# xxxupeng/stereo_toolbox

Hardware: AMD Instinct MI355X
Metric: stereo pairs/sec @ 540x960 D=192 (GwcNet_GC fwd+bwd) (higher is better)
Workload: dtype f32; 1 GPU; GwcNet_GC(maxdisp=192) train step: fwd+bwd+allreduce+Adam, 576x960 pairs (reference pad_to_2x shape), batch 1/GPU, fp32, synthetic randn inputs, deterministic filler weights; global_batch=1, parallelism=dp1, grad_sync=none (single rank: flat fp32 buffer packed, no collective), launch=eager, optimizer=torch.optim.Adam(fused=True)

## Files before the change

include/stx_hip.h:

```cpp
#ifndef STX_HIP_H
#define STX_HIP_H
#ifdef __cplusplus
extern "C" {
#endif

const char* stx_last_error(void);
const char* stx_build_info(void);
int stx_get_tuning(const char* name);
int stx_set_tuning(const char* name, int value);

int stx_cost_volume_fwd(const float* Lg, const float* Rg, int Cg, int G, const float* Lc, const float* Rc, int Cc,
                        const float* scale, float* vol, int B, int H, int W, int D, int mask_left, void* stream);
int stx_group_normalize_fwd(const float* x, float* y, int B, int C, int G, int HW, float out_scale, void* stream);
int stx_group_normalize_bwd(const float* x, const float* gy, float* gx, int B, int C, int G, int HW, float out_scale, void* stream);
int stx_cost_volume_bwd(const float* gvol, const float* Lg, const float* Rg, int Cg, int G, int Cc, float* gLg,
                        float* gRg, float* gLc, float* gRc, int B, int H, int W, int D, int mask_left, void* stream);

int stx_head_fwd(const float* cost, float* disp, float* stats, int B, int Dc, int Hc, int Wc, int D, int H, int W,
                 void* stream);
long long stx_head_bwd_workspace_floats(int B, int Dc, int H, int W);
int stx_head_bwd(const float* gdisp, const float* cost, const float* disp, const float* stats, float* gcost,
                 float* workspace, int B, int Dc, int Hc, int Wc, int D, int H, int W, void* stream);
int stx_head_fwd2(const float* cost, float* disp, float* stats, int B, int Dc, int Hc, int Wc, int D, int H, int W,
                  int align_corners, void* stream);
int stx_head_bwd2(const float* gdisp, const float* cost, const float* disp, const float* stats, float* gcost,
                  float* workspace, int B, int Dc, int Hc, int Wc, int D, int H, int W, int align_corners, void* stream);
int stx_softargmax_fwd(const float* x, float* out, int B, int D, int HW, void* stream);
int stx_argmax_fwd(const float* x, long long* out, int B, int D, int HW, void* stream);
int stx_unimodal_fwd(const float* x, float* out, int B, int D, int HW, void* stream);
int stx_dominant_modal_fwd(const float* x, float* out, int B, int D, int HW, void* stream);
int stx_modal_fwd(const float* x, float* out, float* aux, int B, int D, int HW, int kind, void* stream);
int stx_modal_bwd(const float* g, const float* out, const float* aux, float* gx, int B, int D, int HW, void* stream);
int stx_split_mode(const float* x, float* mode, unsigned char* mask, int B, int D, int HW, void* stream);
int stx_softmax_d_fwd(const float* x, float* y, int B, int D, int HW, void* stream);

long long stx_conv3d_packed_floats(int K, int N, int T);
int stx_conv3d_pack_weight(const float* w, float* wp, int A, int B, int T, int mode, void* stream);
int stx_conv3d_fwd_blocks(int Do, int Ho, int Wo);
long long stx_conv3d_fwd_stat_rows(int B, int Di, int Hi, int Wi, int Cin, int Cout, int ks, int stride);
int stx_conv3d_fwd(const float* x, const float* wp, float* out, const float* scale, const float* bias,
                   const float* residual, float* stats, int B, int Di, int Hi, int Wi, int Cin, int Cout, int ks,
                   int stride, int relu, void* stream);
int stx_deconv3d_fwd_blocks(int Di, int Hi, int Wi);
int stx_deconv3d_fwd(const float* x, const float* wp, float* out, const float* scale, const float* bias,
                     const float* residual, float* stats, int B, int Di, int Hi, int Wi, int Cin, int Cout, int Do,
                     int Ho, int Wo, int relu, void* stream);
long long stx_conv3d_wgrad_workspace_floats(int B, int Dc, int Hc, int Wc, int CF, int CC, int ks, int stride);
int stx_conv3d_wgrad(const float* fine, const float* coarse, float* dw, float* workspace, int B, int Df, int Hf, int Wf,
                     int CF, int Dc, int Hc, int Wc, int CC, int ks, int stride, void* stream);

int stx_conv3d_wgrad_bn_supported(int B, int D, int H, int W, int CF, int CC);
int stx_conv3d_wgrad_bn(const float* x, const float* gy, const float* z, const float* scale, const float* shift, const float* mean,
                        const float* invstd, const float* gamma, const float* sums, float inv_n, int act, float* dz, float* dw,
                        float* workspace, int B, int D, int H, int W, int CF, int CC, void* stream);

int stx_conv3d_axial_supported(int Cin, int Cout, int kd, int kh, int kw);
long long stx_conv3d_axial_packed_floats(int K, int N, int kd, int kh, int kw);
int stx_conv3d_axial_pack_weight(const float* w, float* wp, int A, int B, int kd, int kh, int kw, int mode, void* stream);
long long stx_conv3d_axial_fwd_stat_rows(int B, int D, int H, int W, int Cin, int Cout, int kd, int kh, int kw);
int stx_conv3d_axial_fwd(const float* x, const float* wp, float* out, const float* scale, const float* bias,
                         const float* residual, float* stats, int B, int D, int H, int W, int Cin, int Cout, int kd, int kh,
                         int kw, int act, void* stream);
long long stx_conv3d_axial_wgrad_workspace_floats(int B, int D, int H, int W, int CF, int CC, int kd, int kh, int kw);
int stx_conv3d_axial_wgrad(const float* x, const float* gz, float* dw, float* workspace, int B, int D, int H, int W, int CF,
                           int CC, int kd, int kh, int kw, void* stream);

int stx_convgru_supported(int hidden, int nx, int cx0, int cx1, int cx2, int ksize);
long long stx_convgru_packed_floats(int K, int N);
int stx_convgru_pack_weight(const float* w0, const float* w1, float* wp, int A, int Bd, int mode, void* stream);
int stx_convgru_gemm(const float* s0, int c0, int p0, const float* s1, int c1, int p1, const float* s2, int c2, int p2,
                     const float* s3, int c3, int p3, const float* wp, int N, int epi, int split, const float* bias0,
                     const float* bias1, const float* add0, int add0_pitch, const float* add1, int add1_pitch, const float* h,
                     int h_pitch, const float* z, float* out0, float* out1, float* out2, int out_pitch, int B, int H, int W,
                     void* stream);
int stx_convgru_gate_rows(long long P, int hidden);
int stx_convgru_gate_bwd(const float* g, int g_pitch, const float* z, const float* q, const float* h, int h_pitch, float* gq,
                         float* gz, float* rows, long long P, int hidden, void* stream);
int stx_convgru_reset_bwd(float* buf, int buf_pitch, const float* g, int g_pitch, const float* z, const float* r, const float* h,
                          int h_pitch, float* gr, float* rows, long long P, int hidden, void* stream);
int stx_convgru_row_sum(const float* rows, float* out, int nrows, int n, void* stream);
long long stx_convgru_wgrad_workspace_floats(int B, int H, int W, int K, int CC);
int stx_convgru_wgrad(const float* s0, int c0, int p0, const float* s1, int c1, int p1, const float* s2, int c2, int p2,
                      const float* s3, int c3, int p3, const float* g0, const float* g1, int CG, float* dw, float* workspace,
                      int B, int H, int W, void* stream);

int stx_conv2d_supported(int Cin, int Cout);
long long stx_conv2d_stat_rows(int groups);
int stx_conv2d_fwd(const float* x, const float* w, float* out, float* stats, int B, int H, int W, int Cin, int Cout, int dgrad,
                   int groups, void* stream);

int stx_conv3d_c1_fwd(const float* x, const float* w, const float* residual, float* out, int B, int D, int H, int W,
                      int Cin, void* stream);
long long stx_conv3d_c1_wgrad_workspace_floats(int Cin);
int stx_conv3d_c1_wgrad(const float* x, const float* gy, float* dw, float* workspace, int B, int D, int H, int W,
                        int Cin, void* stream);
int stx_conv3d_c1_dgrad(const float* gy, const float* w, float* gx, int B, int D, int H, int W, int Cin, void* stream);

int stx_mish_fwd(const float* x, float* y, long long n, void* stream);
int stx_mish_bwd(const float* gy, const float* x, float* gx, long long n, void* stream);
int stx_depth_to_space(const float* y, float* out, int B, int D, int H, int W, int C, int inverse, void* stream);
int stx_gate_fwd(const float* cv, const float* att, float* out, int B, int D, long long HW, int C, void* stream);
int stx_gate_bwd(const float* g, const float* cv, const float* att, float* gcv, float* gatt, int B, int D, long long HW,
                 int C, void* stream);

int stx_concat_channels(const float* in0, const float* in1, const float* in2, const float* in3, int C0, int C1, int C2, int C3,
                        float* out, long long nvox, void* stream);
int stx_split_channels(const float* in, float* out0, float* out1, float* out2, float* out3, int C0, int C1, int C2, int C3,
                       long long nvox, void* stream);
int stx_transpose(const float* in, float* out, int N, int rows, int cols, void* stream);

int stx_dwconv_hw_fwd(const float* x, const float* w, const int* dil, float* out, int B, int D, int H, int W, int C,
                      int flip, void* stream);
long long stx_dwconv_hw_wgrad_workspace_floats(int C);
int stx_dwconv_hw_wgrad(const float* x, const float* gy, const int* dil, float* dw, float* workspace, int B, int D,
                        int H, int W, int C, void* stream);
int stx_cost_volume_scale_bwd(const float* gvol, const float* Lc, const float* Rc, float* gscale, int B, int Cc, int H,
                              int W, int D, int mask_left, void* stream);
int stx_scale_channels(const float* x, const float* s, float* out, long long nvox, int C, void* stream);
int stx_ac_volume_bwd(const float* gvol, const float* Lc, const float* Rc, const float* prob, float* gL, float* gR,
                      float* gprob, int B, int Cc, int H, int W, int D, int mask_left, void* stream);

int stx_bn_reduce_blocks(void);
int stx_bn_stats_rows(long long nvox, int C);
int stx_bn_stats(const float* z, float* partials, long long nvox, int C, int groups, void* stream);
int stx_bn_finalize(const float* partials, int nrows, int C, double count, const float* gamma, const float* beta,
                    float* running_mean, float* running_var, float momentum, float eps, float* scale, float* shift,
                    float* mean, float* invstd, void* stream);
int stx_bn_finalize_groups(const float* partials, int nrows, int C, double count, const float* gamma, const float* beta,
                           float* running_mean, float* running_var, float momentum, float eps, float* out, int groups,
                           void* stream);
int stx_bn_apply(const float* z1, const float* scale1, const float* shift1, const float* z2, const float* scale2,
                 const float* shift2, float* out, long long nvox, int C, int relu, int groups, void* stream);
int stx_bn_bwd_reduce(const float* gy, const float* y, const float* z1, const float* mean1, const float* invstd1,
                      const float* z2, const float* mean2, const float* invstd2, float* partials, float* sums,
                      long long nvox, int C, int relu, void* stream);
int stx_bn_bwd_apply(const float* gy, const float* y, const float* z1, const float* mean1, const float* invstd1,
                     const float* gamma1, const float* z2, const float* mean2, const float* invstd2,
                     const float* gamma2, const float* sums, float* dz1, float* dz2, float* gout, long long nvox, int C,
                     int relu, void* stream);
int stx_bn_bwd_reduce2(const float* gy, const float* y, const float* z1, const float* mean1, const float* invstd1,
                       const float* z2, const float* mean2, const float* invstd2, const float* scale1,
                       const float* shift1, const float* scale2, const float* shift2, float* partials, float* sums,
                       long long nvox, int C, int relu, int groups, void* stream);
int stx_bn_bwd_apply2(const float* gy, const float* y, const float* z1, const float* mean1, const float* invstd1,
                      const float* gamma1, const float* z2, const float* mean2, const float* invstd2,
                      const float* gamma2, const float* scale1, const float* shift1, const float* scale2,
                      const float* shift2, const float* sums, float* dz1, float* dz2, float* gout, long long nvox,
                      int C, int relu, int groups, void* stream);

int stx_pad_normalize_u8(const unsigned char* img, float* out, int B, int H, int W, int Hp, int Wp, int top,
                         const float* mean3, const float* std3, void* stream);

int stx_sampled_volume_fwd(const float* Lg, const float* Rg, int Cg, int G, const float* Lc, const float* Rc, int Cc,
                           const float* samples, float* vol, int B, int H, int W, int S, int CTp, void* stream);
int stx_sampled_volume_bwd(const float* gvol, const float* Lg, const float* Rg, int Cg, int G, int Cc,
                           const float* samples, float* gLg, float* gRg, float* gLc, float* gRc, int B, int H, int W,
                           int S, int CTp, void* stream);

int stx_warp_fwd(const float* x, const float* disp, float* out, int B, int C, int H, int W, void* stream);
int stx_warp_bwd(const float* gout, const float* x, const float* disp, float* gx, float* gdisp, int B, int C, int H, int W,
                 void* stream);
int stx_corr_volume_fwd(const float* ref, const float* tgt, float* vol, int B, int C, int H, int W, int maxdisp, int groups,
                        void* stream);
int stx_corr_volume_bwd(const float* gvol, const float* ref, const float* tgt, float* gref, float* gtgt, int B, int C, int H,
                        int W, int maxdisp, int groups, void* stream);
int stx_disparity_variance_fwd(const float* x, const float* disp, const float* samples, float* out, int B, int D, int HW,
                               void* stream);
int stx_disparity_variance_bwd(const float* g, const float* x, const float* disp, const float* samples, float* gx, float* gdisp,
                               float* gsamples, int B, int D, int HW, void* stream);

long long stx_geo_pyramid_floats(long long rows, int len, int C, int levels);
int stx_geo_corr_fwd(const float* fmap1, const float* fmap2, float* cpyr, int B, int C, int H, int W1, int W2, int levels,
                     void* stream);
int stx_geo_corr_bwd(const float* gcpyr, const float* fmap1, const float* fmap2, float* gfmap1, float* gfmap2, int B, int C, int H,
                     int W1, int W2, int levels, void* stream);
int stx_geo_pyramid_fwd(const float* vol, float* gpyr, int B, int D, int H, int W, int C, int levels, void* stream);
int stx_geo_pyramid_bwd(const float* ggpyr, float* gvol, int B, int D, int H, int W, int C, int levels, void* stream);
int stx_geo_lookup_fwd(const float* gpyr, const float* cpyr, const float* disp, const float* coords, float* out, int B, int H,
                       int W, int D, int C, int W2, int levels, int radius, void* stream);
// ... 117 lines not shown
```

stereo_toolbox_amd/_capi.py:

```python
import ctypes
import os
import threading

import torch

_P = ctypes.c_void_p
_I = ctypes.c_int
_F = ctypes.c_float
_L = ctypes.c_longlong

SIGNATURES = {
    "stx_get_tuning": [ctypes.c_char_p],
    "stx_set_tuning": [ctypes.c_char_p, _I],
    "stx_cost_volume_fwd": [_P, _P, _I, _I, _P, _P, _I, _P, _P, _I, _I, _I, _I, _I, _P],
    "stx_cost_volume_bwd": [_P, _P, _P, _I, _I, _I, _P, _P, _P, _P, _I, _I, _I, _I, _I, _P],
    "stx_group_normalize_fwd": [_P, _P, _I, _I, _I, _I, _F, _P],
    "stx_group_normalize_bwd": [_P, _P, _P, _I, _I, _I, _I, _F, _P],
    "stx_head_fwd": [_P, _P, _P, _I, _I, _I, _I, _I, _I, _I, _P],
    "stx_head_bwd_workspace_floats": [_I, _I, _I, _I],
    "stx_head_bwd": [_P, _P, _P, _P, _P, _P, _I, _I, _I, _I, _I, _I, _I, _P],
    "stx_head_fwd2": [_P, _P, _P, _I, _I, _I, _I, _I, _I, _I, _I, _P],
    "stx_head_bwd2": [_P, _P, _P, _P, _P, _P, _I, _I, _I, _I, _I, _I, _I, _I, _P],
    "stx_softargmax_fwd": [_P, _P, _I, _I, _I, _P],
    "stx_argmax_fwd": [_P, _P, _I, _I, _I, _P],
    "stx_softmax_d_fwd": [_P, _P, _I, _I, _I, _P],
    "stx_unimodal_fwd": [_P, _P, _I, _I, _I, _P],
    "stx_dominant_modal_fwd": [_P, _P, _I, _I, _I, _P],
    "stx_modal_fwd": [_P, _P, _P, _I, _I, _I, _I, _P],
    "stx_modal_bwd": [_P, _P, _P, _P, _I, _I, _I, _P],
    "stx_split_mode": [_P, _P, _P, _I, _I, _I, _P],
    "stx_conv3d_packed_floats": [_I, _I, _I],
    "stx_conv3d_pack_weight": [_P, _P, _I, _I, _I, _I, _P],
    "stx_conv3d_fwd_blocks": [_I, _I, _I],
    "stx_conv3d_fwd_stat_rows": [_I, _I, _I, _I, _I, _I, _I, _I],
    "stx_deconv3d_fwd_blocks": [_I, _I, _I],
    "stx_conv3d_fwd": [_P, _P, _P, _P, _P, _P, _P, _I, _I, _I, _I, _I, _I, _I, _I, _I, _P],
    "stx_deconv3d_fwd": [_P, _P, _P, _P, _P, _P, _P, _I, _I, _I, _I, _I, _I, _I, _I, _I, _I, _P],
    "stx_conv3d_wgrad_workspace_floats": [_I, _I, _I, _I, _I, _I, _I, _I],
    "stx_conv3d_wgrad": [_P, _P, _P, _P, _I, _I, _I, _I, _I, _I, _I, _I, _I, _I, _I, _P],
    "stx_conv3d_wgrad_bn_supported": [_I, _I, _I, _I, _I, _I],
    "stx_conv3d_wgrad_bn": [_P] * 9 + [_F, _I, _P, _P, _P, _I, _I, _I, _I, _I, _I, _P],
    "stx_conv3d_axial_supported": [_I, _I, _I, _I, _I],
    "stx_conv3d_axial_packed_floats": [_I, _I, _I, _I, _I],
    "stx_conv3d_axial_pack_weight": [_P, _P, _I, _I, _I, _I, _I, _I, _P],
    "stx_conv3d_axial_fwd_stat_rows": [_I] * 9,
    "stx_conv3d_axial_fwd": [_P] * 7 + [_I] * 10 + [_P],
    "stx_conv3d_axial_wgrad_workspace_floats": [_I] * 9,
    "stx_conv3d_axial_wgrad": [_P, _P, _P, _P] + [_I] * 9 + [_P],
    "stx_convgru_supported": [_I] * 6,
    "stx_convgru_packed_floats": [_I, _I],
    "stx_convgru_pack_weight": [_P, _P, _P, _I, _I, _I, _P],
    "stx_convgru_gemm": [_P, _I, _I] * 4 + [_P, _I, _I, _I, _P, _P, _P, _I, _P, _I, _P, _I, _P, _P, _P, _P, _I, _I, _I, _I, _P],
    "stx_convgru_gate_rows": [_L, _I],
    "stx_convgru_gate_bwd": [_P, _I, _P, _P, _P, _I, _P, _P, _P, _L, _I, _P],
    "stx_convgru_reset_bwd": [_P, _I, _P, _I, _P, _P, _P, _I, _P, _P, _L, _I, _P],
    "stx_convgru_row_sum": [_P, _P, _I, _I, _P],
    "stx_convgru_wgrad_workspace_floats": [_I] * 5,
    "stx_convgru_wgrad": [_P, _I, _I] * 4 + [_P, _P, _I, _P, _P, _I, _I, _I, _P],
    "stx_conv2d_supported": [_I, _I],
    "stx_conv2d_stat_rows": [_I],
    "stx_conv2d_fwd": [_P, _P, _P, _P, _I, _I, _I, _I, _I, _I, _I, _P],
    "stx_conv3d_c1_fwd": [_P, _P, _P, _P, _I, _I, _I, _I, _I, _P],
    "stx_conv3d_c1_wgrad_workspace_floats": [_I],
    "stx_conv3d_c1_wgrad": [_P, _P, _P, _P, _I, _I, _I, _I, _I, _P],
    "stx_conv3d_c1_dgrad": [_P, _P, _P, _I, _I, _I, _I, _I, _P],
    "stx_mish_fwd": [_P, _P, _L, _P],
    "stx_mish_bwd": [_P, _P, _P, _L, _P],
    "stx_depth_to_space": [_P, _P, _I, _I, _I, _I, _I, _I, _P],
    "stx_gate_fwd": [_P, _P, _P, _I, _I, _L, _I, _P],
    "stx_gate_bwd": [_P, _P, _P, _P, _P, _I, _I, _L, _I, _P],
    "stx_concat_channels": [_P, _P, _P, _P, _I, _I, _I, _I, _P, _L, _P],
    "stx_split_channels": [_P, _P, _P, _P, _P, _I, _I, _I, _I, _L, _P],
    "stx_transpose": [_P, _P, _I, _I, _I, _P],
    "stx_dwconv_hw_fwd": [_P, _P, _P, _P, _I, _I, _I, _I, _I, _I, _P],
    "stx_dwconv_hw_wgrad_workspace_floats": [_I],
    "stx_dwconv_hw_wgrad": [_P, _P, _P, _P, _P, _I, _I, _I, _I, _I, _P],
    "stx_cost_volume_scale_bwd": [_P, _P, _P, _P, _I, _I, _I, _I, _I, _I, _P],
    "stx_scale_channels": [_P, _P, _P, _L, _I, _P],
    "stx_ac_volume_bwd": [_P, _P, _P, _P, _P, _P, _P, _I, _I, _I, _I, _I, _I, _P],
    "stx_pad_normalize_u8": [_P, _P, _I, _I, _I, _I, _I, _I, _P, _P, _P],
    "stx_warp_fwd": [_P, _P, _P, _I, _I, _I, _I, _P],
    "stx_warp_bwd": [_P, _P, _P, _P, _P, _I, _I, _I, _I, _P],
    "stx_corr_volume_fwd": [_P, _P, _P, _I, _I, _I, _I, _I, _I, _P],
    "stx_corr_volume_bwd": [_P, _P, _P, _P, _P, _I, _I, _I, _I, _I, _I, _P],
    "stx_disparity_variance_fwd": [_P, _P, _P, _P, _I, _I, _I, _P],
    "stx_disparity_variance_bwd": [_P, _P, _P, _P, _P, _P, _P, _I, _I, _I, _P],
    "stx_sampled_volume_fwd": [_P, _P, _I, _I, _P, _P, _I, _P, _P, _I, _I, _I, _I, _I, _P],
    "stx_sampled_volume_bwd": [_P, _P, _P, _I, _I, _I, _P, _P, _P, _P, _P, _I, _I, _I, _I, _I, _P],
    "stx_geo_pyramid_floats": [_L, _I, _I, _I],
    "stx_geo_corr_fwd": [_P, _P, _P, _I, _I, _I, _I, _I, _I, _P],
    "stx_geo_corr_bwd": [_P, _P, _P, _P, _P, _I, _I, _I, _I, _I, _I, _P],
    "stx_geo_pyramid_fwd": [_P, _P, _I, _I, _I, _I, _I, _I, _P],
    "stx_geo_pyramid_bwd": [_P, _P, _I, _I, _I, _I, _I, _I, _P],
    "stx_geo_lookup_fwd": [_P, _P, _P, _P, _P, _I, _I, _I, _I, _I, _I, _I, _I, _P],
    "stx_geo_lookup_bwd": [_P, _P, _P, _P, _P, _I, _I, _I, _I, _I, _I, _I, _I, _P],
    "stx_context_upsample_fwd": [_P, _P, _P, _I, _I, _I, _P],
    "stx_context_upsample_bwd": [_P, _P, _P, _P, _P, _I, _I, _I, _P],
    "stx_corr1d_pyramid_floats": [_L, _I, _I],
    "stx_corr1d_pyramid_fwd": [_P, _P, _P, _I, _I, _I, _I, _I, _I, _F, _P],
    "stx_corr1d_pyramid_bwd": [_P, _P, _P, _P, _P, _I, _I, _I, _I, _I, _I, _F, _P],
    "stx_corr1d_lookup_fwd": [_P, _P, _P, _P, _I, _P, _I, _I, _I, _I, _I, _P],
    "stx_corr1d_lookup_bwd": [_P, _P, _P, _P, _I, _P, _I, _I, _I, _I, _I, _P],
    "stx_allpairs_estimates_fwd": [_P, _I, _P, _P, _P, _P, _P, _I, _I, _I, _I, _P],
    "stx_allpairs_estimates_bwd": [_P, _P, _P, _P, _P, _P, _P, _I, _I, _I, _I, _P],
    "stx_corr1d_volume_pyramid_fwd": [_P, _P, _P, _F, _P, _I, _I, _I, _I, _I, _P],
    "stx_corr1d_volume_pyramid_bwd": [_P, _P, _P, _F, _P, _I, _I, _I, _I, _I, _P],
    "stx_truncate_mask_fwd": [_P, _P, _I, _F, _F, _P, _I, _I, _I, _P],
    "stx_generate_masks_fwd": [_P, _P, _I, _I, _I, _I, _P],
    "stx_masked_volume_fwd": [_P, _P, _P, _P, _I, _I, _I, _I, _I, _P],
    "stx_masked_volume_bwd": [_P, _P, _P, _P, _I, _I, _I, _I, _I, _P],
    "stx_softlrc_fwd": [_P, _P, _F, _P, _P, _I, _I, _I, _P],
    "stx_softlrc_bwd_workspace_floats": [_I, _I, _I],
    "stx_softlrc_bwd": [_P, _P, _P, _P, _F, _P, _P, _P, _I, _I, _I, _P],
    "stx_weighted_lsq_fwd": [_P, _P, _P, _F, _F, _P, _P, _P, _I, _L, _P],
    "stx_weighted_lsq_bwd": [_P, _P, _P, _P, _P, _P, _P, _P, _P, _I, _L, _P],
    "stx_mirror_detector_fwd": [_P, _P, _P, _P, _F, _F, _P, _L, _P],
    "stx_mirror_detector_bwd": [_P, _P, _P, _P, _P, _F, _F, _P, _P, _P, _P, _L, _P],
    "stx_photo_warp_fwd": [_P, _P, _P, _P, _I, _I, _I, _I, _P],
    "stx_photo_warp_bwd": [_P, _P, _P, _P, _I, _I, _I, _I, _P],
    "stx_ssim_fwd": [_P, _P, _P, _I, _I, _I, _I, _I, _P],
    "stx_ssim_bwd_workspace_floats": [_I, _I, _I, _I],
    "stx_ssim_bwd": [_P, _P, _P, _P, _P, _P, _I, _I, _I, _I, _I, _P],
    "stx_photometric_fwd": [_P, _P, _P, ctypes.c_double, _I, _P, _I, _I, _I, _I, _P],
    "stx_photometric_bwd_workspace_floats": [_I, _I, _I, _I],
# ... 105 lines not shown
```

stereo_toolbox_amd/aggregation.py:

```python
import os
import threading

import torch
import torch.nn as nn

from . import ops


def _is_transposed(conv):
    return isinstance(conv, nn.ConvTranspose3d)


def _conv_cfg(conv):
    ks = conv.kernel_size[0]
    stride = conv.stride[0]
    if _is_transposed(conv):
        k3 = ks == 3 and stride == 2 and conv.padding[0] == 1 and conv.output_padding[0] == 1
        k4 = ks == 4 and stride == 2 and conv.padding[0] == 1 and conv.output_padding[0] == 0
        if not (k3 or k4) or len(set(conv.kernel_size)) != 1 or len(set(conv.stride)) != 1:
            raise ops.StxError("only ConvTranspose3d(k=3, s=2, p=1, op=1) and ConvTranspose3d(k=4, s=2, p=1) are on the hot path")
    else:
        if not ((ks == 3 and conv.padding[0] == 1 and stride in (1, 2)) or (ks == 1 and conv.padding[0] == 0 and stride == 1)):
            raise ops.StxError(f"unsupported Conv3d k={ks} s={stride} p={conv.padding}")
    if conv.bias is not None or conv.groups != 1:
# ... 104 lines not shown
        momentum = 1.0 / float(bn.num_batches_tracked.item())
    else:
        momentum = 0.0
    return {"training": training, "partials": partials, "count": count, "running_mean": bn.running_mean,
            "running_var": bn.running_var, "momentum": momentum, "eps": bn.eps, "sync": sync}


def _raw_conv(x, conv, want):
    ks, stride = _conv_cfg(conv)
    if _is_transposed(conv) and ks == 4:
        return ops.deconv4_raw(x, conv.weight, want)
    return ops.ConvRawFn.apply(x, conv.weight, ks, stride, _is_transposed(conv), want)


@ops.fp32_region
def shared_input_convs(x, blocks):
    cfgs, ws = [], []
    for seq in blocks:
        conv, bn = seq[0], seq[1]
        if _is_transposed(conv) or not bn.training or conv.weight.shape[1] != x.shape[-1] or conv.weight.shape[1] % 8 \
                or conv.weight.shape[0] % 8:
            return None
        ks, stride = _conv_cfg(conv)
        cfgs.append((ks, stride, True))
        ws.append(conv.weight)
    if not _needs_grad(x, *[m for seq in blocks for m in (seq[0], seq[1])]):
        return None
    outs = ops.SharedInputConvsFn.apply(x, tuple(cfgs), *ws)
    return [(outs[2 * k], outs[2 * k + 1]) for k in range(len(blocks))]


@ops.fp32_region
def conv_block(x, conv, bn=None, relu=False, second=None, residual=None, mish=False, leaky=False, raw=None, second_raw=None):
    if (mish and relu) or (leaky and (relu or mish)):
        raise ops.StxError("conv_block: relu, mish and leaky are mutually exclusive")
    if second is not None and residual is not None:
        raise ops.StxError("conv_block: `second` and `residual` are mutually exclusive")
    mods = [conv, bn] + ([second[1], second[2]] if second is not None else [])
    grad = (raw is not None or second_raw is not None
            or _needs_grad(x, residual, *(m for m in mods if m is not None), *([second[0]] if second else [])))
    train_bn = (bn is not None and bn.training) or (second is not None and second[2].training)
    if mish and (grad or train_bn) and (bn is None or residual is not None):
        return ops.mish(conv_block(x, conv, bn, relu=False, second=second, residual=residual))
    if mish:
        relu = 2
    if leaky:
        relu = 3

    if not grad and not train_bn:
        if second is not None:
            s2, b2 = _fold(second[2])
            residual = _infer_conv(second[0], second[1], s2, b2, None, False)
        if bn is not None:
            s1, b1 = _fold(bn)
        else:
            s1 = b1 = None
        return _infer_conv(x, conv, s1, b1, residual, relu)

    want = bn is not None and bn.training
    z1, part1 = raw if raw is not None else _raw_conv(x, conv, want)
    if bn is None:
        y = z1
        if residual is not None:
            y = y + residual
        if relu == 3:
            return torch.nn.functional.leaky_relu(y, 0.01)
        return torch.relu(y) if relu else y
    count1 = z1.numel() // z1.shape[-1]
    st1 = _bn_state(bn, part1 if want else None, count1)
    if second is not None:
        x2, conv2, bn2 = second
        want2 = bn2.training
        z2, part2 = second_raw if second_raw is not None else _raw_conv(x2, conv2, want2)
        st2 = _bn_state(bn2, part2 if want2 else None, z2.numel() // z2.shape[-1])
        return ops.BnActFn.apply(z1, bn.weight, bn.bias, z2, bn2.weight, bn2.bias, None, relu, st1, st2)
    defer = (residual is None and want and relu in (0, 1, False, True) and not _is_transposed(conv) and _conv_cfg(conv) == (3, 1)
             and conv.weight.shape[0] % 32 == 0 and conv.weight.shape[1] % 32 == 0 and not st1.get("sync")
             and os.environ.get("STX_BN_BWD_IN_WGRAD", "1") != "0")
    if defer:
        ops.bn_defer_reset_if_stale()
    return ops.BnActFn.apply(z1, bn.weight, bn.bias, None, None, None, residual, relu, st1, None, 1, defer)


def _axial_cfg(conv):
    if not isinstance(conv, nn.Conv3d) or _is_transposed(conv):
        raise ops.StxError("axial_conv_block: expected an nn.Conv3d")
    kernel = ops._axial_kernel(conv.weight, "axial_conv_block")
    if tuple(conv.stride) != (1, 1, 1) or tuple(conv.dilation) != (1, 1, 1) or conv.groups != 1:
        raise ops.StxError(f"axial_conv_block: stride {tuple(conv.stride)} dilation {tuple(conv.dilation)} groups {conv.groups}: "
                           "only dense stride-1 convolutions are served")
    if tuple(conv.padding) != tuple(k // 2 for k in kernel) or conv.padding_mode != "zeros":
        raise ops.StxError(f"axial_conv_block: padding {conv.padding} ({conv.padding_mode}) is not the 'same' zero padding of kernel {kernel}")
    return kernel


def _fold_with_bias(conv, bn):
    scale, shift = _fold(bn)
    if conv.bias is None:
        return scale, shift
    hit = conv.__dict__.get("_stx_fold") if ops._CACHE_ENABLED else None
    key = (conv.bias._version, conv.bias.data_ptr())
    if hit is not None and hit[0] == key and hit[1] is shift:
        return scale, hit[2]
    with torch.no_grad():
        shift_b = torch.addcmul(shift, conv.bias, scale).contiguous()
    if ops._CACHE_ENABLED:
        conv.__dict__["_stx_fold"] = (key, shift, shift_b)
    return scale, shift_b


@ops.fp32_region
def axial_conv_block(x, conv, bn):
    kernel = _axial_cfg(conv)
    if not isinstance(bn, nn.modules.batchnorm._BatchNorm):
        raise ops.StxError(f"axial_conv_block: {type(bn).__name__} is not a BatchNorm")
    if not _needs_grad(x, conv, bn) and not bn.training:
        scale, shift = _fold_with_bias(conv, bn)
        xk, wk, _ = ops._axial_prepare(x, conv.weight.detach(), "axial_conv_block")
        wp = ops.pack_weight_axial(wk, 0, owner=conv.weight if wk.shape == conv.weight.shape else None)
        return ops.conv3d_axial_forward(xk, wp, conv.weight.shape[0], kernel, scale, shift, None, 1)[0]
    want = bn.training
    z, part = ops.AxialConvRawFn.apply(x, conv.weight, want)
    if conv.bias is not None:
        z = ops.ZeroGradBiasFn.apply(z, conv.bias) if want else z + conv.bias
    st = _bn_state(bn, part if want else None, z.numel() // z.shape[-1])
    y = ops.BnActFn.apply(z, bn.weight, bn.bias, None, None, None, None, 1, st, None)
    if want and conv.bias is not None and bn.track_running_stats and bn.running_mean is not None:
        with torch.no_grad():
            bn.running_mean.add_(conv.bias.detach(), alpha=float(st["momentum"]))
    return y


@ops.fp32_region
def convbn_block(x, seq, relu=False, second=None, residual=None, mish=False, raw=None, second_raw=None):
    sec = None
    if second is not None:
        sec = (second[0], second[1][0], second[1][1])
    return conv_block(x, seq[0], seq[1], relu=relu, second=sec, residual=residual, mish=mish, raw=raw, second_raw=second_raw)
```

stereo_toolbox_amd/csrc/conv3d.hip:

```cpp
#include "stx_common.h"
#include <stdlib.h>

namespace {

constexpr int CONV_THREADS = 256;

struct ConvArgs {
    const float* x;
    const float* wp;
    float* out;
    const float* scale;
    const float* bias;
    const float* residual;
    float* stats;
    int Di, Hi, Wi, Cin;
    int Do, Ho, Wo, Cout;
    int relu;
    int nDt, nHt, nWt;
};

__device__ __forceinline__ int xcd_remap(int bid, int nblk) {
    const int q = nblk >> 3, r = nblk & 7;
    const int xcd = bid & 7, k = bid >> 3;
    const int base = (xcd < r) ? xcd * (q + 1) : r * (q + 1) + (xcd - r) * q;
// ... 360 lines not shown
    };
    using HM = HaloMap<ED, EH, EW, NF4>;
    HM hm;
    hm.init(tid, a.Hi, a.Wi, a.Cin);
    auto load_item = [&](int t, int c0) {
        int b, od0, oh0, ow0;
        tile_origin(t, b, od0, oh0, ow0);
        const int id0 = od0 * S - PAD, ih0 = oh0 * S - PAD, iw0 = ow0 * S - PAD;
        unsigned vo[NST];
        hm.offsets(id0, ih0, iw0, a.Di, a.Hi, a.Wi, vo);
        const stx_bufrsrc xrs = HM::rsrc(a.x, b, id0, ih0, iw0, a.Di, a.Hi, a.Wi, a.Cin);
#pragma unroll
        for (int k = 0; k < NST; ++k) stg[k] = stx_buf_ld4(xrs, vo[k], (unsigned)c0 * 4u);
    };
    auto store_item = [&]() {
#pragma unroll
        for (int k = 0; k < NST; ++k) {
            const int e = tid + k * CONV_THREADS;
            const int v = e / NF4, f = e - v * NF4;
            const int wx = v % EW, hy = (v / EW) % EH, dz = v / (EW * EH);
            const int slot = (S == 2) ? (wx & 1) * EWH + (wx >> 1) : wx;
            if (e < NE) stx_st4(tile + ((dz * EH + hy) * EWS + slot) * VS + 4 * f, stg[k]);
        }
    };

    float s1[NTW], s2[NTW];
#pragma unroll
    for (int nt = 0; nt < NTW; ++nt) { s1[nt] = 0.f; s2[nt] = 0.f; }
    f32x16 acc[MT][NTW];
    float4 bring[3][NQC][NTW];
    static_assert(KS == 3, "the pipelined kernel serves 3x3x3 only");
    const float* wbase = a.wp + (size_t)lane * 4 + (size_t)wcol * NTW * 256;
    if (t_lo < t_hi) {
        load_item(t_lo, 0);
        conv_ring_prologue<NTW, NQC, NT>(wbase, NQ, bring);
    }
    for (int t = t_lo; t < t_hi; ++t) {
#pragma unroll
        for (int m = 0; m < MT; ++m)
#pragma unroll
            for (int nt = 0; nt < NTW; ++nt) acc[m][nt] = zero16();
        for (int ch = 0; ch < nchunk; ++ch) {
            __syncthreads();
            store_item();
            __syncthreads();
            {
                const int nch = ch + 1 < nchunk ? ch + 1 : 0;
                const int ntl = ch + 1 < nchunk ? t : t + 1;
                if (ntl < t_hi) load_item(ntl, nch * CK);
            }
            const float* wq = wbase + (size_t)(ch * (CK / 8)) * NT * 256;
            const float* wq_next = ch + 1 < nchunk ? wq + (size_t)NQC * NT * 256 : (t + 1 < t_hi ? wbase : nullptr);
            conv_chunk_taps27<S, MT, NTW, NQC, EH, EWS, EWH, VS, NT>(tile, abase, wq, wq_next, NQ, acc, bring);
        }
        int b, od0, oh0, ow0;
        tile_origin(t, b, od0, oh0, ow0);
#pragma unroll
        for (int m = 0; m < MT; ++m) {
            const int mtile = wrow * MT + m;
            const int od = od0 + mtile / TH, oh = oh0 + mtile % TH;
            int nrows = (od < a.Do && oh < a.Ho) ? (a.Wo - ow0) : 0;
            nrows = nrows > 32 ? 32 : nrows;
            const size_t vox0 = (((size_t)b * a.Do + od) * a.Ho + oh) * a.Wo + ow0;
#pragma unroll
            for (int nt = 0; nt < NTW; ++nt) {
                const int n = (wcol * NTW + nt) * 32 + i;
                const float sc = (a.scale && n < a.Cout) ? a.scale[n] : 1.f;
                const float bs = (a.bias && n < a.Cout) ? a.bias[n] : 0.f;
                conv_epilogue_block(a, acc[m][nt], vox0, 1, nrows, n, sc, bs, lane, s1[nt], s2[nt]);
            }
        }
    }
    if (a.stats) conv_write_stats<NT, WN>(a, s1, s2, tile, tid, (size_t)blockIdx.x);
}

struct MarchArgs {
    ConvArgs c;
    int ncols;
    int ablate;
    int xs, xo;
    int os, oo, ncout;
    int wq_total, wq_off, wnt_total, wnt_off;
    const float* acc_in;
};

constexpr int MW2_MW = 16, MW2_R = 2, MW2_TH = 8, MW2_EH = 10, MW2_EW = 18, MW2_VS = 36;
constexpr int MW2_SLOT = MW2_EH * MW2_EW * MW2_VS;
constexpr int MW2_NF4 = (MW2_EH * MW2_EW * 8 + 255) / 256;
constexpr int MW2_WFLOATS = 27 * 4 * 256;

template <int BS, int EPI = 1>
__global__ __launch_bounds__(256) void conv3d_marchw_kernel(MarchArgs ma) {
    const ConvArgs& a = ma.c;
    STX_DYN_SMEM(smem);
    float* wl = reinterpret_cast<float*>(smem);
    float* planes = wl + MW2_WFLOATS;
    const int tid = threadIdx.x, lane = tid & 63, wave = tid >> 6;
    const int i = lane & 31, half = lane >> 5;
    const int th = wave;
    auto n_lane = [&]() { return i; };

    for (int e = tid; e < MW2_WFLOATS / 4; e += 256) {
        const int tq = e >> 6, l4 = e & 63;
        const int tap = tq >> 2, q = tq & 3;
        const size_t src = (((size_t)tap * ma.wq_total + ma.wq_off + q) * ma.wnt_total + ma.wnt_off) * 256 + 4 * l4;
        stx_st4(wl + 4 * e, stx_ld4(a.wp + src));
    }

    int b = 0, oh0 = 0, ow0 = 0;
    const long long units = (long long)ma.ncols * a.Do;
    const long long wg = xcd_remap(blockIdx.x, gridDim.x);
    int u = __builtin_amdgcn_readfirstlane((int)(units * wg / gridDim.x));
    const int u_end = __builtin_amdgcn_readfirstlane((int)(units * (wg + 1) / gridDim.x));

    float4 stg[MW2_NF4];
    unsigned svoff[MW2_NF4], ovoff = 0, ovalid = 0;
    const unsigned xplane_bytes = (unsigned)a.Hi * (unsigned)a.Wi * (unsigned)ma.xs * 4u;
    const unsigned oplane_bytes = (unsigned)a.Ho * (unsigned)a.Wo * (unsigned)ma.os * 4u;
    auto column_offsets = [&]() {
#pragma unroll
        for (int k = 0; k < MW2_NF4; ++k) {
            const int idx = tid + k * 256;
            const int v = idx >> 3, f = idx & 7;
            const int wx = v % MW2_EW, hy = v / MW2_EW;
            const int gh = oh0 - 1 + hy, gw = ow0 - 1 + wx;
            const bool ok = v < MW2_EH * MW2_EW && gh >= 0 && gh < a.Hi && gw >= 0 && gw < a.Wi;
            svoff[k] = ok ? (unsigned)(((gh * a.Wi + gw) * ma.xs + ma.xo + 4 * f) * 4) : STX_BUF_OOB;
        }
        const int ohb = oh0 + th * MW2_R, owb = ow0 + 4 * half;
        ovoff = (unsigned)((((ohb * a.Wo + owb) * ma.os) + ma.oo + n_lane()) * 4);
        ovalid = 0;
#pragma unroll
        for (int r = 0; r < 16; ++r) {
            const int c = (r & 3) + 8 * ((r >> 2) & 1), dh = r >> 3;
            if (ohb + dh < a.Ho && owb + c < a.Wo && n_lane() < ma.ncout) ovalid |= 1u << r;
        }
    };
    auto load_plane = [&](int pd, bool on) {
        const bool in = on && pd >= 0 && pd < a.Di;
        const stx_bufrsrc rs = stx_make_rsrc(a.x + ((size_t)b * a.Di + (in ? pd : 0)) * a.Hi * a.Wi * ma.xs, in ? xplane_bytes : 0u);
#pragma unroll
        for (int k = 0; k < MW2_NF4; ++k) stg[k] = stx_buf_ld4(rs, svoff[k], 0u);
    };
    auto store_plane = [&](float* buf) {
#pragma unroll
        for (int k = 0; k < MW2_NF4; ++k) {
            const int idx = tid + k * 256;
            const int v = idx >> 3, f = idx & 7;
            if (v < MW2_EH * MW2_EW) stx_st4(buf + v * MW2_VS + 4 * f, stg[k]);
        }
    };

    float s1 = 0.f, s2 = 0.f;
    const int abase = ((th * MW2_R + i / MW2_MW) * MW2_EW + i % MW2_MW) * MW2_VS + 4 * half;
    const float* wlane = wl + lane * 4;
    const int n = i;
    const float sc = (a.scale && n < ma.ncout) ? a.scale[ma.oo + n] : 1.f;
    const float bs = (a.bias && n < ma.ncout) ? a.bias[ma.oo + n] : 0.f;

    auto emit_row = [&](const f32x16& done0, const f32x16& done1, const f32x16& done, int r, int dprev) {
        const int row = (r & 3) + 8 * (r >> 2) + 4 * half;
        const int oh = oh0 + th * MW2_R + row / MW2_MW, ow = ow0 + row % MW2_MW;
        if (oh < a.Ho && ow < a.Wo && n < ma.ncout && ma.ablate != 2) {
            const size_t idx = ((((size_t)b * a.Do + dprev) * a.Ho + oh) * a.Wo + ow) * ma.os + ma.oo + n;
            float v = BS ? (done0[r] + done1[r]) + done[r] : done[r];
            if (ma.acc_in) v += ma.acc_in[idx];
            s1 += v;
            s2 = fmaf(v, v, s2);
            v = fmaf(v, sc, bs);
            if (a.residual) v += a.residual[idx];
            v = stx_act(v, a.relu);
            a.out[idx] = v;
        }
    };
    const bool relu_on = a.relu == 1;
    float accp[16];
    auto load_partials = [&](unsigned vmask, const stx_bufrsrc& rs) {
#pragma unroll
        for (int r = 0; r < 16; ++r) {
            const int c = (r & 3) + 8 * ((r >> 2) & 1), dh = r >> 3;
            accp[r] = stx_buf_ld1(rs, ((vmask >> r) & 1u) ? ovoff : STX_BUF_OOB, (unsigned)((dh * a.Wo + c) * ma.os * 4));
        }
    };
    auto emit_row_plain = [&](const f32x16& done0, const f32x16& done1, const f32x16& done, int r, unsigned vmask,
                              const stx_bufrsrc& ors) {
        const int c = (r & 3) + 8 * ((r >> 2) & 1), dh = r >> 3;
        const bool ok = EPI == 5 ? vmask != 0u : (bool)((vmask >> r) & 1u);
        float v = BS ? (done0[r] + done1[r]) + done[r] : done[r];
        if (EPI == 2) v += accp[r];
        v = ok ? v : 0.f;
        s1 += v;
        s2 = fmaf(v, v, s2);
        if (EPI != 4 && EPI != 5) {
            v = fmaf(v, sc, bs);
            if (EPI == 3) v += accp[r];
            const float vr = fmaxf(v, 0.f);
            v = relu_on ? vr : v;
        }
        stx_buf_st1(ors, (EPI == 5 || ok) ? ovoff : STX_BUF_OOB, (unsigned)((dh * a.Wo + c) * ma.os * 4), v);
    };

    auto tap_plane = [&](const float* pbuf, int kd, f32x16& acc, bool fresh, bool with_epi, const f32x16& done0, const f32x16& done1,
                         const f32x16& done, int dprev, int epi0, unsigned vmask, const stx_bufrsrc& ors) {
        float4 av[2][4], bv[2][4];
        auto load_tap = [&](int t9, int buf) {
            const int kh = t9 / 3, kw = t9 % 3;
            const float* sl = pbuf + abase + (kh * MW2_EW + kw) * MW2_VS;
            const float* wt = wlane + (kd * 9 + t9) * 1024;
#pragma unroll
            for (int q = 0; q < 4; ++q) {
                av[buf][q] = stx_ld4(sl + 8 * q);
                bv[buf][q] = stx_ld4(wt + q * 256);
            }
        };
        load_tap(0, 0);
#pragma unroll
        for (int t9 = 0; t9 < 9; ++t9) {
            if (t9 + 1 < 9) load_tap(t9 + 1, (t9 + 1) & 1);
            const int cb = t9 & 1;
#pragma unroll
            for (int q = 0; q < 4; ++q) {
                acc = __builtin_amdgcn_mfma_f32_32x32x2f32(av[cb][q].x, bv[cb][q].x, (fresh && t9 == 0 && q == 0) ? zero16() : acc, 0, 0, 0);
                acc = __builtin_amdgcn_mfma_f32_32x32x2f32(av[cb][q].y, bv[cb][q].y, acc, 0, 0, 0);
                acc = __builtin_amdgcn_mfma_f32_32x32x2f32(av[cb][q].z, bv[cb][q].z, acc, 0, 0, 0);
                acc = __builtin_amdgcn_mfma_f32_32x32x2f32(av[cb][q].w, bv[cb][q].w, acc, 0, 0, 0);
            }
            const int r = epi0 + t9;
            if (EPI != 1) {
                if (epi0 >= 0 && r < 16) emit_row_plain(done0, done1, done, r, vmask, ors);
            }
            if (t9 + 1 < 9) {
// ... 442 lines not shown
    constexpr int ROWS = (KS == 1) ? NW : T;
    float* dst = a.slab + ((size_t)blockIdx.y * gridDim.x + blockIdx.x) * ROWS * 1024;
#pragma unroll
    for (int t = 0; t < NTAP; ++t) {
        const int row = (KS == 1) ? wave : t * NW + wave;
        if (KS == 1 ? (t == 0) : (row < T)) {
#pragma unroll
            for (int r = 0; r < 16; ++r) {
                const int cf = (r & 3) + 8 * (r >> 2) + 4 * half;
                dst[(size_t)row * 1024 + cf * 32 + i] = acc[t][r];
            }
        }
    }
}

__global__ __launch_bounds__(CONV_THREADS) void conv3d_wgrad_reduce4_kernel(const float* __restrict__ slab,
                                                                            float* __restrict__ dw, int CF, int CC,
                                                                            int T, int nchunks, int rows_per_chunk) {
    __shared__ float red[16][64];
    const int lane = threadIdx.x & 63, wave = threadIdx.x >> 6;
    const int part = wave * 4 + (lane >> 4), ql = lane & 15;
    const int idx0 = blockIdx.x * 64 + ql * 4;
    const int cc_l = idx0 & 31, cf_l = (idx0 >> 5) & 31;
    const int tap = (idx0 >> 10) % T, pair = (idx0 >> 10) / T;
    const float* p;
    size_t stride;
    int n;
    if (rows_per_chunk == T) {
        p = slab + ((size_t)pair * nchunks * T + tap) * 1024 + cf_l * 32 + cc_l;
        stride = (size_t)T * 1024; n = nchunks;
    } else {
        p = slab + ((size_t)pair * nchunks * rows_per_chunk) * 1024 + cf_l * 32 + cc_l;
        stride = 1024; n = nchunks * rows_per_chunk;
    }
    float4 s = make_float4(0.f, 0.f, 0.f, 0.f);
#pragma unroll 4
    for (int c = part; c < n; c += 16) {
        const float4 v = stx_ld4(p + (size_t)c * stride);
        s.x += v.x; s.y += v.y; s.z += v.z; s.w += v.w;
    }
    stx_st4(&red[part][ql * 4], s);
    __syncthreads();
    if (wave == 0) {
        float t = 0.f;
#pragma unroll
        for (int k = 0; k < 16; ++k) t += red[k][lane];
        const int idx = blockIdx.x * 64 + lane;
        const int cc = idx & 31, cf = (idx >> 5) & 31;
        const int ncf = CF / 32, cfb = pair % ncf, ccb = pair / ncf;
        dw[((size_t)(ccb * 32 + cc) * CF + cfb * 32 + cf) * T + tap] = t;
    }
}

template <typename K, typename... Args>
int launch_with_lds(K kernel, dim3 grid, size_t lds, hipStream_t st, Args... args) {
    if (int rc = stx_lds_require((const void*)kernel, lds, "conv3d")) return rc;
    static const bool report = getenv("STX_REPORT_OCCUPANCY") != nullptr;
    if (report) {
        int nb = -1;
        hipOccupancyMaxActiveBlocksPerMultiprocessor(&nb, (const void*)kernel, CONV_THREADS, lds);
        fprintf(stderr, "[stx] conv3d launch: grid %u x %u, %zu B LDS, %d workgroups per CU\n", grid.x, grid.y, lds, nb);
    }
    hipLaunchKernelGGL(kernel, grid, dim3(CONV_THREADS), lds, st, args...);
    return 0;
}

constexpr int CONV_TD = 2, CONV_TH = 2;

template <int KS, int S>
size_t conv_lds_bytes(int CK, int NT) {
    const int ED = (CONV_TD - 1) * S + KS, EH = (CONV_TH - 1) * S + KS, EW = 31 * S + KS;
    const int EWS = (S == 2) ? 2 * ((EW + 1) / 2) : EW;
    size_t t = (size_t)ED * EH * EWS * (CK + 4) * 4;
    size_t red = (size_t)4 * NT * 32 * 2 * 4;
    return t > red ? t : red;
}

template <int S>
void (*pgemm_kernel(int wn))(ConvArgs, int) {
    return wn == 4 ? conv3d_pgemm_kernel<3, S, CONV_TD, CONV_TH, 4, 8, 4>
         : wn == 2 ? conv3d_pgemm_kernel<3, S, CONV_TD, CONV_TH, 4, 8, 2> : conv3d_pgemm_kernel<3, S, CONV_TD, CONV_TH, 4, 8>;
}

void (*march_kernel(int bs, int epi))(MarchArgs) {
    switch (epi) {
    case 0: return bs ? conv3d_marchw_kernel<1, 0> : conv3d_marchw_kernel<0, 0>;
    case 2: return bs ? conv3d_marchw_kernel<1, 2> : conv3d_marchw_kernel<0, 2>;
    case 3: return bs ? conv3d_marchw_kernel<1, 3> : conv3d_marchw_kernel<0, 3>;
    case 4: return bs ? conv3d_marchw_kernel<1, 4> : conv3d_marchw_kernel<0, 4>;
    case 5: return bs ? conv3d_marchw_kernel<1, 5> : conv3d_marchw_kernel<0, 5>;
    default: return bs ? conv3d_marchw_kernel<1, 1> : conv3d_marchw_kernel<0, 1>;
    }
}

template <int KS, int S>
int conv_dispatch(const ConvArgs& a, int NT, int CK, dim3 grid, hipStream_t st) {
    const size_t lds = conv_lds_bytes<KS, S>(CK, NT);
#define CONV_CASE(NT_, CK_)                                                                                        \
    if (NT == NT_ && CK == CK_)                                                                                    \
        return launch_with_lds(conv3d_igemm_kernel<KS, S, CONV_TD, CONV_TH, NT_, CK_>, grid, lds, st, a);
    if constexpr (KS == 1) { CONV_CASE(1, 32) CONV_CASE(2, 32) CONV_CASE(4, 32) }
    if constexpr (KS == 3) {
        if (NT == 2 && CK == 8 && stx_tune(STX_TUNE_CONV_WN) >= 2)
            return launch_with_lds(conv3d_igemm_kernel<KS, S, CONV_TD, CONV_TH, 2, 8, 4, 2>, grid, lds, st, a);
    }
    CONV_CASE(1, 8) CONV_CASE(2, 8) CONV_CASE(4, 8)
#undef CONV_CASE
    return stx_set_error(STX_ERR_ARG, "conv3d: unsupported NT=%d CK=%d", NT, CK);
}

}

static int conv_pick_ck(int Cin, int ks) { return (ks == 1 && Cin % 32 == 0) ? 32 : 8; }
static int conv_nt(int N) { return N <= 32 ? 1 : (N <= 64 ? 2 : 4); }

extern "C" long long stx_conv3d_packed_floats(int K, int N, int T) {
    return (long long)T * (K / 8) * conv_nt(N) * 256;
}

extern "C" int stx_conv3d_pack_weight(const float* w, float* wp, int A, int Bd, int T, int mode, void* stream) {
    stx_begin();
    STX_REQUIRE(w && wp && A > 0 && Bd > 0 && (T == 1 || T == 27), "conv3d_pack_weight: bad args");
    STX_REQUIRE(mode >= 0 && mode <= 2, "conv3d_pack_weight: mode %d", mode);
    const int K = (mode == 0) ? Bd : A, N = (mode == 0) ? A : Bd;
    STX_REQUIRE(K % 8 == 0 && N <= 128, "conv3d_pack_weight: GEMM-K channels (%d) must be a multiple of 8, N (%d) <= 128", K, N);
    const int NT = conv_nt(N);
    const size_t total = (size_t)T * (K / 8) * NT * 256;
    hipLaunchKernelGGL(conv3d_pack_kernel, dim3((unsigned)((total + CONV_THREADS - 1) / CONV_THREADS)),
                       dim3(CONV_THREADS), 0, (hipStream_t)stream, w, wp, A, Bd, T, mode, K, N, NT, total);
    return stx_check_launch("conv3d_pack_weight");
}

static int march_wgs(long long units) {
    long long g = 256;
    if (g > units / 3) g = units / 3;
    return g < 1 ? 1 : (int)g;
}

extern "C" int stx_conv3d_fwd_blocks(int Do, int Ho, int Wo) {
    stx_begin();
    const int a = stx_cdiv(Do, CONV_TD) * stx_cdiv(Ho, CONV_TH) * stx_cdiv(Wo, 32);
    const int m = Do * stx_cdiv(Ho, 4) * stx_cdiv(Wo, 32);
    const int m16 = Do * stx_cdiv(Ho, 8) * stx_cdiv(Wo, 16);
    return a > m ? (a > m16 ? a : m16) : (m > m16 ? m : m16);
}
extern "C" int stx_deconv3d_fwd_blocks(int Di, int Hi, int Wi) {
    stx_begin(); return Di * stx_cdiv(Hi, 2) * stx_cdiv(Wi, 32); }

struct ConvPlan { int kind; int march_wgs; int pgrid; long long rows; };
static int persistent_grid(size_t lds, long long ntiles) {
    int per_cu = (int)(STX_LDS_MAX / (lds + 512));
    per_cu = per_cu < 1 ? 1 : (per_cu > 2 ? 2 : per_cu);
    const long long g = 256ll * per_cu;
    return (int)(g > ntiles ? ntiles : g);
}
static ConvPlan conv_plan(int B, int Di, int Hi, int Wi, int Cin, int Cout, int ks, int stride) {
    const int pad = ks / 2;
    const int Do = (Di + 2 * pad - ks) / stride + 1, Ho = (Hi + 2 * pad - ks) / stride + 1, Wo = (Wi + 2 * pad - ks) / stride + 1;
    ConvPlan p{2, 0, 0, 0};
    if (ks == 3 && stride == 1 && ((Cin == 32 && Cout <= 64) || (Cin == 64 && Cout <= 32) ||
                                   (Cin == 64 && Cout <= 64 && stx_tune(STX_TUNE_CONV_L1_MARCH)))) {
        const long long ncols = (long long)B * stx_cdiv(Ho, MW2_TH) * stx_cdiv(Wo, MW2_MW);
        if (ncols * Do < (1ll << 31) && (long long)Hi * Wi * Cin * 4 < (1ll << 31) && (long long)Ho * Wo * Cout * 4 < (1ll << 31)) {
            p.kind = 0; p.march_wgs = march_wgs(ncols * Do); p.rows = p.march_wgs;
            return p;
        }
    }
    const long long tiles = (long long)stx_cdiv(Do, CONV_TD) * stx_cdiv(Ho, CONV_TH) * stx_cdiv(Wo, 32);
    if (conv_nt(Cout) == 4 && ks == 3 && tiles * B < (1ll << 31)) {
        const size_t lds = stride == 1 ? conv_lds_bytes<3, 1>(8, 4) : conv_lds_bytes<3, 2>(8, 4);
        p.kind = 1; p.pgrid = persistent_grid(lds, tiles * B); p.rows = p.pgrid;
        return p;
    }
    p.rows = tiles * B;
    return p;
}

extern "C" long long stx_conv3d_fwd_stat_rows(int B, int Di, int Hi, int Wi, int Cin, int Cout, int ks, int stride) {
    stx_begin();
    if (B < 1 || Di < 1 || Hi < 1 || Wi < 1 || Cin < 1 || Cout < 1 || !((ks == 3 && (stride == 1 || stride == 2)) || (ks == 1 && stride == 1)))
        return 0;
    return conv_plan(B, Di, Hi, Wi, Cin, Cout, ks, stride).rows;
}

extern "C" int stx_conv3d_fwd(const float* x, const float* wp, float* out, const float* scale, const float* bias,
                              const float* residual, float* stats, int B, int Di, int Hi, int Wi, int Cin, int Cout,
                              int ks, int stride, int relu, void* stream) {
    stx_begin();
    STX_REQUIRE(x && wp && out && B > 0 && Di > 0 && Hi > 0 && Wi > 0, "conv3d_fwd: bad shape");
    STX_REQUIRE(Cin % 8 == 0 && Cout >= 1 && Cout <= 128, "conv3d_fwd: Cin=%d (need %%8) Cout=%d (need <=128)", Cin, Cout);
    STX_REQUIRE((ks == 3 && (stride == 1 || stride == 2)) || (ks == 1 && stride == 1),
                "conv3d_fwd: kernel %d stride %d unsupported", ks, stride);
    ConvArgs a;
    a.x = x; a.wp = wp; a.out = out; a.scale = scale; a.bias = bias; a.residual = residual; a.stats = stats;
    a.Di = Di; a.Hi = Hi; a.Wi = Wi; a.Cin = Cin; a.Cout = Cout; a.relu = relu;
    const int pad = ks / 2;
    a.Do = (Di + 2 * pad - ks) / stride + 1;
    a.Ho = (Hi + 2 * pad - ks) / stride + 1;
    a.Wo = (Wi + 2 * pad - ks) / stride + 1;
    a.nDt = stx_cdiv(a.Do, CONV_TD); a.nHt = stx_cdiv(a.Ho, CONV_TH); a.nWt = stx_cdiv(a.Wo, 32);
    const int NT = conv_nt(Cout);
    hipStream_t st = (hipStream_t)stream;
    const ConvPlan plan = conv_plan(B, Di, Hi, Wi, Cin, Cout, ks, stride);
    if (plan.kind == 0) {
        MarchArgs m2;
        m2.c = a;
        m2.c.nHt = stx_cdiv(a.Ho, MW2_TH);
        m2.c.nWt = stx_cdiv(a.Wo, MW2_MW);
        m2.ncols = B * m2.c.nHt * m2.c.nWt;
        m2.ablate = stx_tune(STX_TUNE_MARCH_ABLATE);
        {
            const int nb2 = plan.march_wgs;
            const size_t lds2 = ((size_t)MW2_WFLOATS + 2 * (size_t)MW2_SLOT) * 4;
            const int bs = stx_tune(STX_TUNE_MARCH_BS), epi_fast = stx_tune(STX_TUNE_MARCH_EPI);
            const bool whole = a.Ho % MW2_TH == 0 && a.Wo % MW2_MW == 0;
            m2.xs = Cin; m2.os = Cout; m2.wq_total = Cin / 8; m2.wnt_total = conv_nt(Cout);
            const int nk = Cin / 32, nn = stx_cdiv(Cout, 32);
            for (int ns = 0; ns < nn; ++ns)
                for (int kslice = 0; kslice < nk; ++kslice) {
                    MarchArgs m = m2;
                    m.xo = 32 * kslice; m.wq_off = 4 * kslice;
                    m.oo = 32 * ns; m.wnt_off = ns; m.ncout = Cout - 32 * ns < 32 ? Cout - 32 * ns : 32;
                    m.acc_in = kslice > 0 ? out : nullptr;
                    if (kslice + 1 < nk) {
                        m.c.scale = nullptr; m.c.bias = nullptr; m.c.residual = nullptr; m.c.stats = nullptr; m.c.relu = 0;
                    }
                    const bool plain = epi_fast && !(m.c.residual && m.acc_in) && m.c.relu < 2;
                    const bool raw = !m.acc_in && !m.c.residual && !m.c.scale && !m.c.bias && m.c.relu == 0;
                    const int epi = plain ? (raw ? (whole && m.ncout == 32 ? 5 : 4) : m.acc_in ? 2 : (m.c.residual ? 3 : 0)) : 1;
                    if (int rc = launch_with_lds(march_kernel(bs, epi), dim3(nb2), lds2, st, m)) return rc;
                }
            return stx_check_launch("conv3d_fwd(march)");
        }
    }
    STX_REQUIRE(halo_range_ok(Di, Hi, Wi, Cin), "conv3d_fwd: a batch item of %d x %d x %d x %d floats exceeds the 2 GiB "
                "buffer-descriptor range", Di, Hi, Wi, Cin);
    const int CK = (stride == 2) ? 8 : conv_pick_ck(Cin, ks);
    dim3 grid(a.nDt * a.nHt * a.nWt, B);
    int rc;
    if (plan.kind == 1) {
        const long long nt_all = (long long)grid.x * B;
        {
            const size_t lds = stride == 1 ? conv_lds_bytes<3, 1>(8, 4) : conv_lds_bytes<3, 2>(8, 4);
            const int wn = stx_tune(STX_TUNE_CONV_WN) == 4 ? 4 : (stx_tune(STX_TUNE_CONV_WN) == 3 ? 2 : 1);
            rc = launch_with_lds(stride == 1 ? pgemm_kernel<1>(wn) : pgemm_kernel<2>(wn), dim3(plan.pgrid), lds, st, a, (int)nt_all);
            if (rc) return rc;
            return stx_check_launch("conv3d_fwd(pipelined)");
        }
    }
    if (ks == 3 && stride == 1) rc = conv_dispatch<3, 1>(a, NT, CK, grid, st);
    else if (ks == 3 && NT == 2 && stx_tune(STX_TUNE_CONV_S2_DENSE)) {
        if (stx_tune(STX_TUNE_CONV_WN) >= 2)
            rc = launch_with_lds(conv3d_igemm_kernel<3, 2, CONV_TD, CONV_TH, 2, 8, 0, 2>, grid, (size_t)5 * 5 * 66 * 8 * 4, st, a);
        else
        rc = launch_with_lds(conv3d_igemm_kernel<3, 2, CONV_TD, CONV_TH, 2, 8, 0>, grid, (size_t)5 * 5 * 66 * 8 * 4, st, a);
    }
    else if (ks == 3) rc = conv_dispatch<3, 2>(a, NT, CK, grid, st);
    else rc = conv_dispatch<1, 1>(a, NT, CK, grid, st);
    if (rc) return rc;
    return stx_check_launch("conv3d_fwd");
}

extern "C" int stx_deconv3d_fwd(const float* x, const float* wp, float* out, const float* scale, const float* bias,
                                const float* residual, float* stats, int B, int Di, int Hi, int Wi, int Cin, int Cout,
                                int Do, int Ho, int Wo, int relu, void* stream) {
    stx_begin();
    STX_REQUIRE(x && wp && out && B > 0 && Di > 0 && Hi > 0 && Wi > 0, "deconv3d_fwd: bad shape");
    STX_REQUIRE(Cin % 32 == 0 && Cout >= 1 && Cout <= 64, "deconv3d_fwd: Cin=%d (need %%32) Cout=%d (need <=64)", Cin, Cout);
    STX_REQUIRE(Do <= 2 * Di && Do >= 2 * Di - 1 && Ho <= 2 * Hi && Ho >= 2 * Hi - 1 && Wo <= 2 * Wi && Wo >= 2 * Wi - 1,
                "deconv3d_fwd: output dims must be 2*in or 2*in-1");
    ConvArgs a;
    a.x = x; a.wp = wp; a.out = out; a.scale = scale; a.bias = bias; a.residual = residual; a.stats = stats;
    a.Di = Di; a.Hi = Hi; a.Wi = Wi; a.Cin = Cin; a.Cout = Cout; a.relu = relu;
    a.Do = Do; a.Ho = Ho; a.Wo = Wo;
    a.nDt = Di; a.nHt = stx_cdiv(Hi, 2); a.nWt = stx_cdiv(Wi, 32);
    STX_REQUIRE(halo_range_ok(Di, Hi, Wi, Cin), "deconv3d_fwd: a batch item of %d x %d x %d x %d floats exceeds the 2 GiB "
                "buffer-descriptor range", Di, Hi, Wi, Cin);
    dim3 grid(a.nDt * a.nHt * a.nWt, B);
    hipStream_t st = (hipStream_t)stream;
    const size_t lds = (size_t)2 * 3 * 33 * (8 + 4) * 4;
    int rc = conv_nt(Cout) == 1 ? launch_with_lds(deconv3d_igemm_kernel<1, 8>, grid, lds, st, a)
                                : launch_with_lds(deconv3d_igemm_kernel<2, 8>, grid, lds, st, a);
    if (rc) return rc;
    return stx_check_launch("deconv3d_fwd");
}

static bool wgrad_pipe(int ks, int stride, int npairs) { return ks == 3 && (stride == 2 || npairs <= 2); }
static void wgrad_tile(int ks, int stride, int Wc, bool pipe, int* TH, int* TW) {
    *TH = pipe ? 4 : 2; *TW = (stride == 2) ? 16 : 32;
    if (ks == 3 && stride == 1 && stx_cdiv(Wc, 16) * 16 < stx_cdiv(Wc, 32) * 32) { *TH = 4; *TW = 16; }
}
static int wgrad_chunks(int ntiles, int npairs, bool pipe) {
    int c = (pipe ? 256 : 512) / npairs;
    if (c < 1) c = 1;
    if (c > ntiles) c = ntiles;
    const int forced = stx_tune(STX_TUNE_WGRAD_GRID);
    if (forced > 0 && forced < c) c = forced;
    return c;
}

struct StxWgradBn {
    const float* z; float* dz;
    const float *scale, *shift, *mean, *invstd, *gamma, *sum_g, *sum_gx;
    float inv_n; int act;
};
int stx_wgrad_march_launch(const float* x, const float* gy, float* slab, int B, int D, int H, int W, int CF, int CC, int nchunks,
                           void* stream, const StxWgradBn* bn);
int stx_wgrad_march_chunks(int B, int D, int H, int W, int npairs);
int stx_wgrad_march_s2_launch(const float* f, const float* c, float* slab, int B, int Df, int Hf, int Wf, int CF, int Dc, int Hc,
                              int Wc, int CC, int nchunks, void* stream);

extern "C" long long stx_conv3d_wgrad_workspace_floats(int B, int Dc, int Hc, int Wc, int CF, int CC, int ks,
                                                       int stride) {
    const int npairs = (CF / 32) * (CC / 32);
    if (npairs < 1 || B < 1 || Dc < 1 || Hc < 1 || Wc < 1) return 0;
    const int rows = (ks == 1) ? 8 : 27;
    const bool pipe = wgrad_pipe(ks, stride, npairs);
    int TH, TW;
    wgrad_tile(ks, stride, Wc, pipe, &TH, &TW);
    int c = wgrad_chunks(B * Dc * stx_cdiv(Hc, TH) * stx_cdiv(Wc, TW), npairs, pipe);
    if (ks == 3) {
        const int cm = stx_wgrad_march_chunks(B, Dc, Hc, Wc, npairs);
        if (cm > c) c = cm;
    }
    return (long long)npairs * c * rows * 1024;
}

extern "C" int stx_conv3d_wgrad(const float* f, const float* c, float* dw, float* workspace, int B, int Df, int Hf,
                                int Wf, int CF, int Dc, int Hc, int Wc, int CC, int ks, int stride, void* stream) {
    stx_begin();
    STX_REQUIRE(f && c && dw && workspace && B > 0, "conv3d_wgrad: null operand");
    STX_REQUIRE(CF >= 32 && CC >= 32 && CF % 32 == 0 && CC % 32 == 0,
                "conv3d_wgrad: channel counts (%d, %d) must be positive multiples of 32", CF, CC);
    STX_REQUIRE(Dc > 0 && Hc > 0 && Wc > 0, "conv3d_wgrad: empty volume");
    STX_REQUIRE((ks == 3 && (stride == 1 || stride == 2)) || (ks == 1 && stride == 1), "conv3d_wgrad: ks/stride");
    STX_REQUIRE((long long)Hf * Wf * CF * 4 < (1ll << 31) && (long long)Hc * Wc * CC * 4 < (1ll << 31),
                "conv3d_wgrad: a plane of %d x %d voxels exceeds the 2 GiB buffer-descriptor range", Hf, Wf);
    WgradArgs a;
    a.f = f; a.c = c; a.slab = workspace;
    a.B = B; a.Df = Df; a.Hf = Hf; a.Wf = Wf; a.CF = CF; a.Dc = Dc; a.Hc = Hc; a.Wc = Wc; a.CC = CC;
    const int npairs = (CF / 32) * (CC / 32);
    const bool pipe = wgrad_pipe(ks, stride, npairs);
    a.ablate = stx_tune(STX_TUNE_WGRAD_ABLATE);
    int TH, TW;
    wgrad_tile(ks, stride, Wc, pipe, &TH, &TW);
    a.nHt = stx_cdiv(Hc, TH); a.nWt = stx_cdiv(Wc, TW);
    a.ntiles = B * Dc * a.nHt * a.nWt;
    int nchunks = wgrad_chunks(a.ntiles, npairs, pipe);
    hipStream_t st = (hipStream_t)stream;
    const int T = ks == 1 ? 1 : 27;
    if (ks == 3 && (stx_tune(STX_TUNE_WGRAD_MARCH) & (stride == 1 ? 1 : 2))) {
        int mc = stx_wgrad_march_chunks(B, Dc, Hc, Wc, npairs);
        const int forced = stx_tune(STX_TUNE_WGRAD_GRID);
        if (forced > 0 && forced < mc) mc = forced;
        const int rc = stride == 1 ? stx_wgrad_march_launch(f, c, workspace, B, Dc, Hc, Wc, CF, CC, mc, stream, nullptr)
                                   : stx_wgrad_march_s2_launch(f, c, workspace, B, Df, Hf, Wf, CF, Dc, Hc, Wc, CC, mc, stream);
        if (rc > 0) return rc;
        if (rc == 0) {
            const int total = npairs * T * 1024;
            hipLaunchKernelGGL(conv3d_wgrad_reduce4_kernel, dim3(total / 64), dim3(CONV_THREADS), 0, st, workspace, dw, CF, CC, T,
                               mc, 27);
            return stx_check_launch("conv3d_wgrad_reduce");
        }
    }
    dim3 grid(nchunks, npairs);
#define WG_LAUNCH(KS_, S_, TH_, TW_, NW_, PIPE_, LDS_)                                                           \
    {                                                                                                             \
        const size_t lds = (LDS_);                                                                                \
        void (*wk)(WgradArgs) = conv3d_wgrad_kernel<KS_, S_, TH_, TW_, NW_, PIPE_>;                               \
        if (int rc = stx_lds_require((const void*)wk, lds, "conv3d_wgrad")) return rc;                            \
        hipLaunchKernelGGL(wk, grid, dim3(NW_ * 64), lds, st, a);                                                 \
    }
    if (ks == 3 && stride == 1) {
        if (TW == 16 && pipe) WG_LAUNCH(3, 1, 4, 16, 8, true, ((size_t)3 * 6 * 18 + 64) * 32 * 4)
        else if (TW == 16) WG_LAUNCH(3, 1, 4, 16, 8, false, ((size_t)3 * 6 * 18 + 64) * 32 * 4)
        else if (pipe) WG_LAUNCH(3, 1, 4, 32, 8, true, ((size_t)3 * 6 * 34 + 128) * 32 * 4)
        else WG_LAUNCH(3, 1, 2, 32, 8, false, ((size_t)3 * 4 * 34 + 64) * 32 * 4)
    } else if (ks == 3) {
        WG_LAUNCH(3, 2, 4, 16, 8, true, ((size_t)3 * 9 * 34 + 64) * 32 * 4)
    } else {
        WG_LAUNCH(1, 1, 2, 32, 4, false, ((size_t)2 * 32 + 64) * 32 * 4)
    }
#undef WG_LAUNCH
    int rc = stx_check_launch("conv3d_wgrad");
    if (rc) return rc;
    const int total = npairs * T * 1024;
    hipLaunchKernelGGL(conv3d_wgrad_reduce4_kernel, dim3(total / 64), dim3(CONV_THREADS), 0, st, workspace, dw, CF, CC, T,
                       nchunks, ks == 1 ? 4 : 27);
    return stx_check_launch("conv3d_wgrad_reduce");
}

extern "C" int stx_conv3d_wgrad_bn_supported(int B, int D, int H, int W, int CF, int CC) {
    stx_begin();
    return (stx_tune(STX_TUNE_WGRAD_MARCH) & 1) && B > 0 && D > 0 && H > 0 && W > 0 && CF >= 32 && CC >= 32 && CF % 32 == 0 &&
           CC % 32 == 0 && (long long)H * W * CF * 4 < (1ll << 31) && (long long)H * W * CC * 4 < (1ll << 31) &&
           (long long)B * stx_cdiv(H, 4) * stx_cdiv(W, 16) < (1ll << 31);
}

extern "C" int stx_conv3d_wgrad_bn(const float* x, const float* gy, const float* z, const float* scale, const float* shift,
                                   const float* mean, const float* invstd, const float* gamma, const float* sums, float inv_n,
                                   int act, float* dz, float* dw, float* workspace, int B, int D, int H, int W, int CF, int CC,
                                   void* stream) {
    stx_begin();
    STX_REQUIRE(x && gy && z && scale && shift && mean && invstd && sums && dz && dw && workspace, "conv3d_wgrad_bn: null operand");
    STX_REQUIRE(act == 0 || act == 1, "conv3d_wgrad_bn: activation code %d (0 or 1)", act);
    STX_REQUIRE(stx_conv3d_wgrad_bn_supported(B, D, H, W, CF, CC), "conv3d_wgrad_bn: shape (%d x %d x %d x %d, %d -> %d channels) is "
                "not served by the march kernel (ask stx_conv3d_wgrad_bn_supported)", B, D, H, W, CF, CC);
    const int npairs = (CF / 32) * (CC / 32);
    int mc = stx_wgrad_march_chunks(B, D, H, W, npairs);
    const int forced = stx_tune(STX_TUNE_WGRAD_GRID);
    if (forced > 0 && forced < mc) mc = forced;
    StxWgradBn bn;
    bn.z = z; bn.dz = dz; bn.scale = scale; bn.shift = shift; bn.mean = mean; bn.invstd = invstd; bn.gamma = gamma;
    bn.sum_g = sums; bn.sum_gx = sums + CC; bn.inv_n = inv_n; bn.act = act;
    const int rc = stx_wgrad_march_launch(x, gy, workspace, B, D, H, W, CF, CC, mc, stream, &bn);
    if (rc > 0) return rc;
    STX_REQUIRE(rc == 0, "conv3d_wgrad_bn: the march kernel refused the shape");
    const int total = npairs * 27 * 1024;
    hipLaunchKernelGGL(conv3d_wgrad_reduce4_kernel, dim3(total / 64), dim3(CONV_THREADS), 0, (hipStream_t)stream, workspace, dw, CF,
                       CC, 27, mc, 27);
    return stx_check_launch("conv3d_wgrad_reduce");
}
```

stereo_toolbox_amd/csrc/conv_c1.hip:

```cpp
#include "stx_common.h"
#include <stdlib.h>

namespace {

constexpr int C1_THREADS = 256;
constexpr int C1_TD = 2, C1_TH = 4, C1_TW = 32;
constexpr int C1_ED = C1_TD + 2, C1_EH = C1_TH + 2, C1_EW = C1_TW + 2;
constexpr int C1_CK = 16, C1_VS = C1_CK + 4;

struct C1Args {
    const float* x;
    const float* w;
    const float* gy;
    const float* res;
    float* out;
    int B, D, H, W, Cin;
    int nDt, nHt, nWt, ntiles;
};

__device__ __forceinline__ void c1_stage(const C1Args& a, float* tile, int b, int d0, int h0, int w0, int c0, int tid) {
    for (int idx = tid; idx < C1_ED * C1_EH * C1_EW * (C1_CK / 4); idx += C1_THREADS) {
        const int v = idx / (C1_CK / 4), f = idx - v * (C1_CK / 4);
        const int wx = v % C1_EW, hy = (v / C1_EW) % C1_EH, dz = v / (C1_EW * C1_EH);
        const int gd = d0 - 1 + dz, gh = h0 - 1 + hy, gw = w0 - 1 + wx;
// ... 160 lines not shown
#pragma unroll
                for (int j = 0; j < 6; ++j) g6[j] = gp[j];
#pragma unroll
                for (int kw = 0; kw < 3; ++kw) {
                    const float4 wv = stx_ld4(ws + ((kd * 3 + kh) * 3 + kw) * Cin + 4 * q);
#pragma unroll
                    for (int j = 0; j < 4; ++j) {
                        const float g = g6[j + 2 - kw];
                        acc[j].x = fmaf(g, wv.x, acc[j].x);
                        acc[j].y = fmaf(g, wv.y, acc[j].y);
                        acc[j].z = fmaf(g, wv.z, acc[j].z);
                        acc[j].w = fmaf(g, wv.w, acc[j].w);
                    }
                }
            }
        const int oh = h0 + lh;
        if (oh < H) {
            float* o = gx + ((((size_t)b * D + d) * H + oh) * W + w0 + lw) * Cin + 4 * q;
#pragma unroll
            for (int j = 0; j < 4; ++j)
                if (w0 + lw + j < W) stx_st4(o + (size_t)j * Cin, acc[j]);
        }
    }
}


__global__ __launch_bounds__(C1_THREADS) void conv_c1_dgrad_mfma_kernel(const float* __restrict__ gy,
                                                                        const float* __restrict__ w, float* __restrict__ gx,
                                                                        int B, int D, int H, int W, int nHt, int nWt, int ntiles) {
    __shared__ float gys[3 * C1D_EH * C1D_EW];
    const int tid = threadIdx.x, lane = tid & 63, wave = tid >> 6;
    const int i = lane & 31, half = lane >> 5;
    float wreg[14];
    int aoff[14];
#pragma unroll
    for (int j = 0; j < 14; ++j) {
        const int tap = 2 * j + half;
        const int tp = tap < 27 ? tap : 26;
        const int kd = tp / 9, kh = (tp / 3) % 3, kw = tp % 3;
        wreg[j] = tap < 27 ? w[(size_t)i * 27 + tap] : 0.f;
        aoff[j] = ((2 - kd) * C1D_EH + (wave + 2 - kh)) * C1D_EW + i + 2 - kw;
    }
    const unsigned plane_bytes = (unsigned)H * (unsigned)W * 128u;
    for (int tile = blockIdx.x; tile < ntiles; tile += gridDim.x) {
        int r_ = tile;
        const int wt = r_ % nWt; r_ /= nWt;
        const int ht = r_ % nHt; r_ /= nHt;
        const int d = r_ % D;
        const int b = r_ / D;
        const int h0 = ht * C1D_TH, w0 = wt * C1D_TW;
        __syncthreads();
        for (int idx = tid; idx < 3 * C1D_EH * C1D_EW; idx += C1_THREADS) {
            const int wx = idx % C1D_EW, hy = (idx / C1D_EW) % C1D_EH, dz = idx / (C1D_EW * C1D_EH);
            const int gd = d - 1 + dz, gh = h0 - 1 + hy, gw = w0 - 1 + wx;
            gys[idx] = (gd >= 0 && gd < D && gh >= 0 && gh < H && gw >= 0 && gw < W)
                           ? gy[(((size_t)b * D + gd) * H + gh) * W + gw] : 0.f;
        }
        __syncthreads();
        f32x16 acc;
#pragma unroll
        for (int r = 0; r < 16; ++r) acc[r] = 0.f;
        float av[14];
#pragma unroll
        for (int j = 0; j < 14; ++j) av[j] = gys[aoff[j]];
#pragma unroll
        for (int j = 0; j < 14; ++j) acc = __builtin_amdgcn_mfma_f32_32x32x2f32(av[j], wreg[j], acc, 0, 0, 0);
        const int oh = h0 + wave;
        const stx_bufrsrc ors = stx_make_rsrc(gx + ((size_t)b * D + d) * H * W * 32, plane_bytes);
        const unsigned vbase = (unsigned)((((oh < H ? oh : 0) * W + w0 + 4 * half) * 32 + i) * 4);
#pragma unroll
        for (int r = 0; r < 16; ++r) {
            const int m = (r & 3) + 8 * (r >> 2);
            const bool ok = oh < H && w0 + 4 * half + m < W;
            stx_buf_st1(ors, ok ? vbase : STX_BUF_OOB, (unsigned)(m * 128), acc[r]);
        }
    }
}


constexpr int C1M_TD = 2, C1M_TH = 8, C1M_TW = 32;
constexpr int C1M_ED = C1M_TD + 2, C1M_EH = C1M_TH + 2, C1M_EW = C1M_TW + 2;
constexpr int C1M_BLOCKS = 1024;

__global__ __launch_bounds__(C1_THREADS) void conv_c1_wgrad_mfma_kernel(const float* __restrict__ x,
                                                                        const float* __restrict__ gy,
                                                                        float* __restrict__ slab, int B, int D, int H,
                                                                        int W, int Cin, int nDt, int nHt, int nWt,
                                                                        int ntiles) {
    __shared__ float gys[C1M_ED * C1M_EH * C1M_EW];
    __shared__ float red[4][1024];
    const int tid = threadIdx.x, lane = tid & 63, wave = tid >> 6;
    const int i = lane & 31, half = lane >> 5;
    const int cb = blockIdx.y;
    const int kd = i / 9, kh = (i / 3) % 3, kw = i % 3;
    const int toff = (i < 27) ? ((2 - kd) * C1M_EH + (2 - kh)) * C1M_EW + (2 - kw) + half : half;
    f32x16 acc;
#pragma unroll
    for (int r = 0; r < 16; ++r) acc[r] = 0.f;
    for (int t = blockIdx.x; t < ntiles; t += gridDim.x) {
        int r = t;
        const int wt = r % nWt; r /= nWt;
        const int ht = r % nHt; r /= nHt;
        const int dt = r % nDt;
        const int b = r / nDt;
        const int d0 = dt * C1M_TD, h0 = ht * C1M_TH, w0 = wt * C1M_TW;
        __syncthreads();
        for (int idx = tid; idx < C1M_ED * C1M_EH * C1M_EW; idx += C1_THREADS) {
            const int wx = idx % C1M_EW, hy = (idx / C1M_EW) % C1M_EH, dz = idx / (C1M_EW * C1M_EH);
            const int gd = d0 - 1 + dz, gh = h0 - 1 + hy, gw = w0 - 1 + wx;
            gys[idx] = (gd >= 0 && gd < D && gh >= 0 && gh < H && gw >= 0 && gw < W)
                           ? gy[(((size_t)b * D + gd) * H + gh) * W + gw] : 0.f;
        }
        __syncthreads();
#pragma unroll 1
        for (int k = 0; k < 4; ++k) {
            const int row = wave * 4 + k;
            const int ld = row / C1M_TH, lh = row % C1M_TH;
            const int gd = d0 + ld, gh = h0 + lh;
            const bool rowok = gd < D && gh < H;
            const float* xr = x + ((((size_t)b * D + gd) * H + gh) * W + w0 + half) * Cin + cb * 32 + i;
            float av[16];
#pragma unroll
            for (int p = 0; p < 16; ++p)
                av[p] = (rowok && w0 + 2 * p + half < W) ? xr[(size_t)(2 * p) * Cin] : 0.f;
            const float* gp = gys + (ld * C1M_EH + lh) * C1M_EW + toff;
#pragma unroll
            for (int p = 0; p < 16; ++p) {
                float bv = gp[2 * p];
                bv = (i < 27) ? bv : 0.f;
                acc = __builtin_amdgcn_mfma_f32_32x32x2f32(av[p], bv, acc, 0, 0, 0);
            }
        }
    }
#pragma unroll
    for (int r = 0; r < 16; ++r) red[wave][((r & 3) + 8 * (r >> 2) + 4 * half) * 32 + i] = acc[r];
    __syncthreads();
    float* dst = slab + ((size_t)cb * gridDim.x + blockIdx.x) * 1024;
    for (int idx = tid; idx < 1024; idx += C1_THREADS)
        dst[idx] = (red[0][idx] + red[1][idx]) + (red[2][idx] + red[3][idx]);
}

__global__ __launch_bounds__(C1_THREADS) void c1m_reduce_kernel(const float* __restrict__ slab, int nrows,
                                                                float* __restrict__ dw) {
    __shared__ double red[C1_THREADS];
    const int m = blockIdx.x, tid = threadIdx.x;
    const int tap = m % 27, cfull = m / 27, cb = cfull >> 5, c = cfull & 31;
    const float* p = slab + (size_t)cb * nrows * 1024 + c * 32 + tap;
    double s = 0.0;
    for (int r = tid; r < nrows; r += C1_THREADS) s += (double)p[(size_t)r * 1024];
    red[tid] = s;
    __syncthreads();
    for (int k = C1_THREADS / 2; k > 0; k >>= 1) {
        if (tid < k) red[tid] += red[tid + k];
        __syncthreads();
    }
    if (tid == 0) dw[m] = (float)red[0];
}


constexpr int C1F_TH = 8, C1F_TW = 32;
constexpr int C1F_EH = C1F_TH + 2, C1F_EW = C1F_TW + 2, C1F_NV = C1F_EH * C1F_EW;
constexpr int C1F_MT = (C1F_NV + 31) / 32;
constexpr int C1F_WGS = 512;

__global__ __launch_bounds__(C1_THREADS) void conv_c1_fwd_mfma_kernel(const float* __restrict__ x,
                                                                      const float* __restrict__ w,
                                                                      const float* __restrict__ res,
                                                                      float* __restrict__ out, int B, int D, int H, int W,
                                                                      int nHt, int nWt, int ncols) {
    STX_DYN_SMEM(smem);
    float* Ps = reinterpret_cast<float*>(smem);
    const int tid = threadIdx.x, lane = tid & 63, wave = __builtin_amdgcn_readfirstlane(tid >> 6);
    const int i = lane & 31, half = lane >> 5;
    float wreg[16];
#pragma unroll
    for (int s_ = 0; s_ < 16; ++s_) wreg[s_] = (i < 27) ? w[(size_t)(16 * half + s_) * 27 + i] : 0.f;
    const int lh = tid / C1F_TW, lw = tid % C1F_TW;

    constexpr int MTW = (C1F_MT + 3) / 4;
    const long long units = (long long)ncols * D;
    int u = __builtin_amdgcn_readfirstlane((int)(units * blockIdx.x / gridDim.x));
    const int u_end = __builtin_amdgcn_readfirstlane((int)(units * (blockIdx.x + 1) / gridDim.x));
    const unsigned plane_bytes = (unsigned)H * (unsigned)W * 32u * 4u;
    while (u < u_end) {
        const int col = u / D;
        const int d_lo = u - col * D;
        const int left = u_end - u;
        const int d_hi = (D - d_lo < left) ? D : d_lo + left;
        u += d_hi - d_lo;
        const int wt = col % nWt, ht = (col / nWt) % nHt, b = col / (nWt * nHt);
        const int h0 = ht * C1F_TH, w0 = wt * C1F_TW;
        const int oh = h0 + lh, ow = w0 + lw;
        const bool ook = oh < H && ow < W;
        unsigned voff[MTW];
#pragma unroll
        for (int t = 0; t < MTW; ++t) {
            const int hv = (wave + 4 * t) * 32 + i;
            const int hy = hv / C1F_EW, wx = hv - hy * C1F_EW;
            const int gh = h0 - 1 + hy, gw = w0 - 1 + wx;
            const bool ok = wave + 4 * t < C1F_MT && hv < C1F_NV && gh >= 0 && gh < H && gw >= 0 && gw < W;
            voff[t] = ok ? (unsigned)(((gh * W + gw) * 32 + 16 * half) * 4) : STX_BUF_OOB;
        }
        float4 nxt[MTW][4];
        auto load_plane = [&](int p) {
            const bool in = p >= 0 && p < D && p <= d_hi;
            const stx_bufrsrc rs = stx_make_rsrc(x + ((size_t)b * D + (in ? p : 0)) * H * W * 32, in ? plane_bytes : 0u);
#pragma unroll
            for (int t = 0; t < MTW; ++t)
#pragma unroll
                for (int q = 0; q < 4; ++q) nxt[t][q] = stx_buf_ld4(rs, voff[t], 16u * q);
        };
        float accA = 0.f, accB = 0.f;
        load_plane(d_lo - 1);
        __syncthreads();
        for (int p = d_lo - 1; p <= d_hi; ++p) {
            float* Pb = Ps + ((p + 2) & 1) * (C1F_NV * 27);
            const bool pin = p >= 0 && p < D;
            float4 cur[MTW][4];
#pragma unroll
            for (int t = 0; t < MTW; ++t)
#pragma unroll
                for (int q = 0; q < 4; ++q) cur[t][q] = nxt[t][q];
            load_plane(p + 1);
            if (pin) {
#pragma unroll
                for (int t = 0; t < MTW; ++t) {
                    const int m = wave + 4 * t;
                    if (m < C1F_MT) {
                        f32x16 acc;
#pragma unroll
                        for (int r = 0; r < 16; ++r) acc[r] = 0.f;
#pragma unroll
                        for (int q = 0; q < 4; ++q) {
                            acc = __builtin_amdgcn_mfma_f32_32x32x2f32(cur[t][q].x, wreg[4 * q + 0], acc, 0, 0, 0);
                            acc = __builtin_amdgcn_mfma_f32_32x32x2f32(cur[t][q].y, wreg[4 * q + 1], acc, 0, 0, 0);
                            acc = __builtin_amdgcn_mfma_f32_32x32x2f32(cur[t][q].z, wreg[4 * q + 2], acc, 0, 0, 0);
                            acc = __builtin_amdgcn_mfma_f32_32x32x2f32(cur[t][q].w, wreg[4 * q + 3], acc, 0, 0, 0);
                        }
                        if (i < 27) {
#pragma unroll
                            for (int r = 0; r < 16; ++r) {
                                const int v = m * 32 + (r & 3) + 8 * (r >> 2) + 4 * half;
                                if (v < C1F_NV) Pb[v * 27 + i] = acc[r];
                            }
                        }
                    }
                }
            }
            __syncthreads();
            float s0 = 0.f, s1 = 0.f, s2 = 0.f;
            if (pin) {
#pragma unroll
                for (int kh = 0; kh < 3; ++kh)
#pragma unroll
                    for (int kw = 0; kw < 3; ++kw) {
                        const float* pp = Pb + ((lh + kh) * C1F_EW + lw + kw) * 27 + kh * 3 + kw;
                        s0 += pp[0];
                        s1 += pp[9];
                        s2 += pp[18];
                    }
            }
            const float done = accA + s2;
            const int od = p - 1;
            if (od >= d_lo && od < d_hi && ook) {
                const size_t o = (((size_t)b * D + od) * H + oh) * W + ow;
                out[o] = res ? done + res[o] : done;
            }
            accA = accB + s1;
            accB = s0;
        }
    }
}

}

extern "C" int stx_conv3d_c1_fwd(const float* x, const float* w, const float* residual, float* out, int B, int D,
                                 int H, int W, int Cin, void* stream) {
    stx_begin();
    STX_REQUIRE(x && w && out && B > 0 && D > 0 && H > 0 && W > 0, "conv3d_c1_fwd: bad shape");
    STX_REQUIRE(Cin % C1_CK == 0, "conv3d_c1_fwd: Cin=%d must be a multiple of %d", Cin, C1_CK);
    if (Cin == 32 && (long long)H * W * 128 < (1ll << 31)) {
        const int nHt = stx_cdiv(H, C1F_TH), nWt = stx_cdiv(W, C1F_TW);
        const long long ncols = (long long)B * nHt * nWt, units = ncols * D;
        STX_REQUIRE(units < (1ll << 31), "conv3d_c1_fwd: volume too large");
        long long g = C1F_WGS;
        if (g > units / 4) g = units / 4 > 0 ? units / 4 : 1;
        const size_t lds = (size_t)2 * C1F_NV * 27 * 4;
        if (int rc = stx_lds_require((const void*)conv_c1_fwd_mfma_kernel, lds, "conv3d_c1_fwd(mfma)")) return rc;
        hipLaunchKernelGGL(conv_c1_fwd_mfma_kernel, dim3((unsigned)g), dim3(C1_THREADS), lds, (hipStream_t)stream, x, w,
                           residual, out, B, D, H, W, nHt, nWt, (int)ncols);
        return stx_check_launch("conv3d_c1_fwd(mfma)");
    }
    C1Args a;
    a.x = x; a.w = w; a.gy = nullptr; a.res = residual; a.out = out;
    a.B = B; a.D = D; a.H = H; a.W = W; a.Cin = Cin;
    a.nDt = stx_cdiv(D, C1_TD); a.nHt = stx_cdiv(H, C1_TH); a.nWt = stx_cdiv(W, C1_TW);
    a.ntiles = B * a.nDt * a.nHt * a.nWt;
    if (int rc = stx_lds_require((const void*)conv_c1_fwd_kernel, C1_TILE_BYTES, "conv3d_c1_fwd")) return rc;
    hipLaunchKernelGGL(conv_c1_fwd_kernel, dim3(a.ntiles), dim3(C1_THREADS), C1_TILE_BYTES, (hipStream_t)stream, a);
    return stx_check_launch("conv3d_c1_fwd");
}

extern "C" long long stx_conv3d_c1_wgrad_workspace_floats(int Cin) {
    const long long valu = (long long)C1_WGRAD_BLOCKS * Cin * 27;
    const long long mfma = (long long)C1M_BLOCKS * 1024 * ((Cin + 31) / 32);
    return valu > mfma ? valu : mfma;
}

extern "C" int stx_conv3d_c1_wgrad(const float* x, const float* gy, float* dw, float* workspace, int B, int D, int H,
                                   int W, int Cin, void* stream) {
    stx_begin();
    STX_REQUIRE(x && gy && dw && workspace && B > 0, "conv3d_c1_wgrad: null operand");
    STX_REQUIRE(Cin % C1_CK == 0 && Cin <= 4 * C1_CK, "conv3d_c1_wgrad: Cin=%d must be 16..64 in steps of 16", Cin);
    if (Cin % 32 == 0) {
        const int nDt = stx_cdiv(D, C1M_TD), nHt = stx_cdiv(H, C1M_TH), nWt = stx_cdiv(W, C1M_TW);
        const long long nt = (long long)B * nDt * nHt * nWt;
        STX_REQUIRE(nt < (1ll << 31), "conv3d_c1_wgrad: volume too large");
        const int nblk = nt < C1M_BLOCKS ? (int)nt : C1M_BLOCKS;
        hipStream_t st = (hipStream_t)stream;
        hipLaunchKernelGGL(conv_c1_wgrad_mfma_kernel, dim3(nblk, Cin / 32), dim3(C1_THREADS), 0, st, x, gy, workspace, B,
                           D, H, W, Cin, nDt, nHt, nWt, (int)nt);
        int rc = stx_check_launch("conv3d_c1_wgrad(mfma)");
        if (rc) return rc;
        hipLaunchKernelGGL(c1m_reduce_kernel, dim3(Cin * 27), dim3(C1_THREADS), 0, st, workspace, nblk, dw);
        return stx_check_launch("conv3d_c1_wgrad(reduce)");
    }
    C1Args a;
    a.x = x; a.w = nullptr; a.gy = gy; a.res = nullptr; a.out = workspace;
    a.B = B; a.D = D; a.H = H; a.W = W; a.Cin = Cin;
    a.nDt = stx_cdiv(D, C1_TD); a.nHt = stx_cdiv(H, C1_TH); a.nWt = stx_cdiv(W, C1_TW);
    a.ntiles = B * a.nDt * a.nHt * a.nWt;
    const int nblk = a.ntiles < C1_WGRAD_BLOCKS ? a.ntiles : C1_WGRAD_BLOCKS;
    const size_t lds = C1_TILE_BYTES + 256 * 4;
    hipStream_t st = (hipStream_t)stream;
    if (int rc = stx_lds_require((const void*)conv_c1_wgrad_kernel, lds, "conv3d_c1_wgrad")) return rc;
    hipLaunchKernelGGL(conv_c1_wgrad_kernel, dim3(nblk), dim3(C1_THREADS), lds, st, a);
    if (int rc = stx_check_launch("conv3d_c1_wgrad")) return rc;
    hipLaunchKernelGGL(c1_colsum_kernel, dim3(Cin * 27), dim3(C1_THREADS), 0, st, workspace, nblk, Cin * 27, dw);
    return stx_check_launch("conv3d_c1_colsum");
}

extern "C" int stx_conv3d_c1_dgrad(const float* gy, const float* w, float* gx, int B, int D, int H, int W, int Cin,
                                   void* stream) {
    stx_begin();
    STX_REQUIRE(gy && w && gx && B > 0 && D > 0 && H > 0 && W > 0, "conv3d_c1_dgrad: bad shape");
    STX_REQUIRE(Cin % 4 == 0 && Cin <= 64, "conv3d_c1_dgrad: Cin=%d must be a multiple of 4, <= 64", Cin);
    const int nHt = stx_cdiv(H, C1D_TH), nWt = stx_cdiv(W, C1D_TW);
    const long long nt = (long long)B * D * nHt * nWt;
    if (Cin == 32 && (long long)H * W * 128 < (1ll << 31) && nt < (1ll << 31)) {
        const long long g = nt < 256 * 8 ? nt : 256 * 8;
        hipLaunchKernelGGL(conv_c1_dgrad_mfma_kernel, dim3((unsigned)g), dim3(C1_THREADS), 0, (hipStream_t)stream, gy, w, gx, B, D,
                           H, W, nHt, nWt, (int)nt);
        return stx_check_launch("conv3d_c1_dgrad(mfma)");
    }
    hipLaunchKernelGGL(conv_c1_dgrad_kernel, dim3((unsigned)((size_t)B * D * nHt * nWt)), dim3(C1_THREADS), 0,
                       (hipStream_t)stream, gy, w, gx, B, D, H, W, Cin, nHt, nWt);
    return stx_check_launch("conv3d_c1_dgrad");
}
```

stereo_toolbox_amd/csrc/stx_common.h:

```cpp
#pragma once
#ifdef STX_HIPEMU
#include "hipemu.h"
#define STX_DYN_SMEM(name) char* name = hipemu::dyn_smem()
#define stx_exp(x) expf(x)
#define stx_fdiv(a, b) ((a) / (b))
#define STX_SCHED_BARRIER() ((void)0)
#define STX_SCHED_GROUP(mask, n) ((void)0)
#define STX_OPAQUE_VGPR(x) ((void)0)
#define STX_TIE3(a, b, c) ((void)0)
#define STX_BARRIER_LDS() __syncthreads()
#define STX_GLDS4(base, off, ldsptr) ((void)(((float*)(ldsptr))[threadIdx.x & 63u] = (base)[(off)]))
#define STX_GLDS_WAIT() ((void)0)
#else
#include <hip/hip_runtime.h>
#define STX_DYN_SMEM(name) extern __shared__ __attribute__((aligned(16))) char name[]
#ifdef STX_PRECISE_MATH
#define stx_exp(x) expf(x)
#define stx_fdiv(a, b) ((a) / (b))
#else
#define stx_exp(x) __expf(x)
#define stx_fdiv(a, b) __fdividef((a), (b))
#endif
#define STX_SCHED_BARRIER() __builtin_amdgcn_sched_barrier(0)
#define STX_SCHED_GROUP(mask, n) __builtin_amdgcn_sched_group_barrier(mask, n, 0)
// ... 35 lines not shown
}
static inline void stx_buf_st4(stx_bufrsrc r, unsigned voff, unsigned soff, float4 v) {
    if (voff >= STX_BUF_OOB || voff >= r.bytes) return;
    const unsigned long long off = (unsigned long long)voff + soff;
    if (off + 16 > r.bytes) abort();
    *reinterpret_cast<float4*>(const_cast<char*>(r.base) + off) = v;
}
#else
typedef __amdgpu_buffer_rsrc_t stx_bufrsrc;
typedef unsigned int stx_u32x4 __attribute__((ext_vector_type(4)));
__device__ __forceinline__ stx_bufrsrc stx_make_rsrc(const void* p, unsigned bytes) {
    return __builtin_amdgcn_make_buffer_rsrc(const_cast<void*>(p), 0, (int)bytes, 0x00020000);
}
__device__ __forceinline__ float4 stx_buf_ld4(stx_bufrsrc r, unsigned voff, unsigned soff) {
    const stx_u32x4 v = __builtin_amdgcn_raw_buffer_load_b128(r, (int)voff, (int)soff, 0);
    return make_float4(__uint_as_float(v[0]), __uint_as_float(v[1]), __uint_as_float(v[2]), __uint_as_float(v[3]));
}
__device__ __forceinline__ float stx_buf_ld1(stx_bufrsrc r, unsigned voff, unsigned soff) {
    return __uint_as_float(__builtin_amdgcn_raw_buffer_load_b32(r, (int)voff, (int)soff, 0));
}
__device__ __forceinline__ void stx_buf_st1(stx_bufrsrc r, unsigned voff, unsigned soff, float v) {
    __builtin_amdgcn_raw_buffer_store_b32(__float_as_uint(v), r, (int)voff, (int)soff, 0);
}
__device__ __forceinline__ void stx_buf_st4(stx_bufrsrc r, unsigned voff, unsigned soff, float4 v) {
    const stx_u32x4 u = {__float_as_uint(v.x), __float_as_uint(v.y), __float_as_uint(v.z), __float_as_uint(v.w)};
    __builtin_amdgcn_raw_buffer_store_b128(u, r, (int)voff, (int)soff, 0);
}
#endif
template <typename T>
__device__ __forceinline__ T* stx_uniform_ptr(T* p) {
    const unsigned long long v = (unsigned long long)p;
    const unsigned lo = (unsigned)__builtin_amdgcn_readfirstlane((int)(unsigned)v);
    const unsigned hi = (unsigned)__builtin_amdgcn_readfirstlane((int)(unsigned)(v >> 32));
    return (T*)(((unsigned long long)hi << 32) | lo);
}
#include <stdint.h>

typedef float f32x4 __attribute__((ext_vector_type(4)));
typedef float f32x16 __attribute__((ext_vector_type(16)));

#define STX_OK 0
#define STX_ERR_ARG 1
#define STX_ERR_LAUNCH 2

int stx_set_error(int code, const char* fmt, ...);
int stx_check_launch(const char* what);
static inline void stx_begin() { (void)hipGetLastError(); }

#define STX_REQUIRE(cond, ...)                                   \
    do {                                                         \
        if (!(cond)) return stx_set_error(STX_ERR_ARG, __VA_ARGS__); \
    } while (0)

static inline int stx_cdiv(int a, int b) { return (a + b - 1) / b; }

constexpr size_t STX_LDS_DEFAULT = 64 * 1024;
constexpr size_t STX_LDS_MAX = 160 * 1024;
bool stx_lds_try(const void* kern, size_t bytes);
int stx_lds_require(const void* kern, size_t bytes, const char* what);

enum StxTune {
    STX_TUNE_MARCH_BS,
    STX_TUNE_MARCH_EPI,
    STX_TUNE_MARCH_ABLATE,
    STX_TUNE_WGRAD_ABLATE,
    STX_TUNE_WGRAD_MARCH,
    STX_TUNE_WGRAD_GRID,
    STX_TUNE_CONV_L1_MARCH,
    STX_TUNE_CONV_S2_DENSE,
    STX_TUNE_CONV_WN,
    STX_TUNE_CV_OLD,
    STX_TUNE_CV_GRID,
    STX_TUNE_CV_PF,
    STX_TUNE_CV_UNITS,
    STX_TUNE_CV_WIN,
    STX_TUNE_CVB_OLD,
    STX_TUNE_CVB_TEAM,
    STX_TUNE_CVB_GRID,
    STX_TUNE_CVB_NSET,
    STX_TUNE_SV_BWD_V1,
    STX_TUNE_DWCONV_ROLL,
    STX_TUNE_C2_PAD,
    STX_TUNE_C2_ABLATE,
    STX_TUNE_COUNT
};
int stx_tune(StxTune id);

__device__ __forceinline__ float stx_mish_tanh_sp(float x, float& w) {
    w = stx_exp(x < 20.f ? x : 20.f);
    const float n = w * (w + 2.f);
    return x > 20.f ? 1.f : stx_fdiv(n, n + 2.f);
}
__device__ __forceinline__ float stx_mish(float x) {
    float w;
    return x * stx_mish_tanh_sp(x, w);
}
__device__ __forceinline__ float stx_mish_grad(float x) {
    float w;
    const float t = stx_mish_tanh_sp(x, w);
    const float ds = x > 20.f ? 1.f : stx_fdiv(w, 1.f + w);
    return t + x * (1.f - t * t) * ds;
}
#define STX_LEAKY_SLOPE 0.01f
__device__ __forceinline__ float stx_act(float v, int code) {
    return code == 1 ? (v > 0.f ? v : 0.f) : (code == 2 ? stx_mish(v) : (code == 3 ? (v > 0.f ? v : STX_LEAKY_SLOPE * v) : v));
}
__device__ __forceinline__ float stx_act_bwd(float g, float t, int code) {
    return code == 2 ? g * stx_mish_grad(t) : (code == 3 ? (t > 0.f ? g : STX_LEAKY_SLOPE * g) : (t > 0.f ? g : 0.f));
}

__device__ __forceinline__ float4 stx_ld4(const float* p) { return *reinterpret_cast<const float4*>(p); }
__device__ __forceinline__ void stx_st4(float* p, float4 v) { *reinterpret_cast<float4*>(p) = v; }
__device__ __forceinline__ void stx_st4_nt(float* p, float4 v) {
#ifdef STX_HIPEMU
    *reinterpret_cast<float4*>(p) = v;
#else
    f32x4 t;
    t[0] = v.x; t[1] = v.y; t[2] = v.z; t[3] = v.w;
    __builtin_nontemporal_store(t, reinterpret_cast<f32x4*>(p));
#endif
}
```

stereo_toolbox_amd/csrc/stx_runtime.hip:

```cpp
#include "stx_common.h"
#include <stdarg.h>
#include <stdio.h>

static thread_local char g_err[512] = "";

int stx_set_error(int code, const char* fmt, ...) {
    va_list ap;
    va_start(ap, fmt);
    vsnprintf(g_err, sizeof(g_err), fmt, ap);
    va_end(ap);
    return code;
}

int stx_check_launch(const char* what) {
    hipError_t e = hipGetLastError();
    if (e != hipSuccess) return stx_set_error(STX_ERR_LAUNCH, "%s: launch failed: %s", what, hipGetErrorString(e));
    return STX_OK;
}

bool stx_lds_try(const void* kern, size_t bytes) {
    if (bytes <= STX_LDS_DEFAULT) return true;
    if (bytes > STX_LDS_MAX) return false;
    if (hipFuncSetAttribute(kern, hipFuncAttributeMaxDynamicSharedMemorySize, (int)bytes) == hipSuccess) return true;
    (void)hipGetLastError();
    return false;
}

int stx_lds_require(const void* kern, size_t bytes, const char* what) {
    if (bytes > STX_LDS_MAX) return stx_set_error(STX_ERR_ARG, "%s: %zu B of LDS exceed the %zu B of a CU", what, bytes, STX_LDS_MAX);
    if (!stx_lds_try(kern, bytes)) return stx_set_error(STX_ERR_LAUNCH, "%s: %zu B of LDS refused by this device", what, bytes);
    return STX_OK;
}

extern "C" const char* stx_last_error(void) { return g_err; }

extern "C" const char* stx_build_info(void) {
#ifdef STX_HIPEMU
    return "stx-hipemu (host SIMT emulator build: tests only)";
#else
    return "stx-gfx950 (hipcc --offload-arch=gfx950)";
#endif
}

#include <stdlib.h>
#include <string.h>
namespace {
struct TuneEntry { const char* name; int value; };
constexpr int TUNE_N = STX_TUNE_COUNT + 1;
TuneEntry g_tune[TUNE_N] = {
    {"STX_MARCH_BS", 1}, {"STX_MARCH_EPI", 1}, {"STX_MARCH_ABLATE", 0}, {"STX_WGRAD_ABLATE", 0}, {"STX_WGRAD_MARCH", 3}, {"STX_WGRAD_GRID", 0}, {"STX_CONV_L1_MARCH", 0}, {"STX_CONV_S2_DENSE", 1}, {"STX_CONV_WN", 2},
    {"STX_CV_OLD", 0}, {"STX_CV_GRID", 0}, {"STX_CV_PF", 0}, {"STX_CV_UNITS", 1}, {"STX_CV_WIN", 0}, {"STX_CVB_OLD", 0}, {"STX_CVB_TEAM", 0}, {"STX_CVB_GRID", 0}, {"STX_CVB_NSET", 3},
    {"STX_SV_BWD_V1", 0}, {"STX_DWCONV_ROLL", 1}, {"STX_C2_PAD", 8}, {"STX_C2_ABLATE", 0}, {"STX_DA_GRID", 0},
};
struct TuneInit {
    TuneInit() {
        for (int i = 0; i < TUNE_N; ++i)
            if (const char* e = getenv(g_tune[i].name)) g_tune[i].value = atoi(e);
    }
} g_tune_init;
}

int stx_tune(StxTune id) { return g_tune[id].value; }

extern "C" int stx_get_tuning(const char* name) {
    for (int i = 0; i < TUNE_N; ++i)
        if (name && !strcmp(name, g_tune[i].name)) return g_tune[i].value;
    return -1;
}

extern "C" int stx_set_tuning(const char* name, int value) {
    for (int i = 0; i < TUNE_N; ++i)
        if (name && !strcmp(name, g_tune[i].name)) { g_tune[i].value = value; return STX_OK; }
    return stx_set_error(STX_ERR_ARG, "stx_set_tuning: unknown switch %s", name ? name : "(null)");
}
```

stereo_toolbox_amd/csrc/wgrad_march.hip:

```cpp
#include "stx_common.h"

namespace {

constexpr int WM_TH = 4, WM_TW = 16;
constexpr int WM_NW = 8, WM_THR = WM_NW * 64;
constexpr int WM_EH = WM_TH + 2, WM_EW = WM_TW + 2;
constexpr int WM_EWP = 20;
constexpr int WM_CHP = 132;
constexpr int WM_XPLANE = 32 * WM_CHP;
constexpr int WM_GP = 68;
constexpr int WM_GPLANE = 32 * WM_GP;
constexpr int WM_NXB = 4, WM_NGB = 2;
constexpr int WM_NPX = (WM_EH * WM_EW * 8 + WM_THR - 1) / WM_THR;
static_assert(WM_TH * WM_TW * 8 == WM_THR, "one gy float4 per lane");
constexpr size_t WM_LDS_BYTES = (size_t)(WM_NXB * WM_XPLANE + WM_NGB * WM_GPLANE) * 4;

struct WmArgs {
    const float* x;
    const float* gy;
    float* slab;
    int B, D, H, W, CF, CC;
    int nHt, nWt, ncols;
    long long nsteps;
    const float* z;
    float* dz;
    const float *bn_scale, *bn_shift, *bn_mean, *bn_invstd, *bn_gamma, *bn_sum_g, *bn_sum_gx;
    float bn_inv_n;
    int bn_act;
};

__device__ __forceinline__ f32x16 wm_zero16() {
    f32x16 z;
#pragma unroll
    for (int i = 0; i < 16; ++i) z[i] = 0.f;
    return z;
}

template <bool BN>
__global__ __launch_bounds__(WM_THR) void conv3d_wgrad_march_kernel(WmArgs a) {
    STX_DYN_SMEM(smem);
    float* xl = reinterpret_cast<float*>(smem);
    float* gl = xl + WM_NXB * WM_XPLANE;
    const int tid = threadIdx.x, lane = tid & 63;
    const int wave = __builtin_amdgcn_readfirstlane(tid >> 6);
    const int i = lane & 31, half = lane >> 5;
    const int ncf = a.CF / 32;
    const int cfb = blockIdx.y % ncf, ccb = blockIdx.y / ncf;
    const int kdw = wave / 3, khw = wave % 3;

    f32x16 acc[3], acc8[3];
#pragma unroll
    for (int t = 0; t < 3; ++t) { acc[t] = wm_zero16(); acc8[t] = wm_zero16(); }

    unsigned xoff[WM_NPX];
    int xhw[WM_NPX], xpos[WM_NPX];
#pragma unroll
    for (int k = 0; k < WM_NPX; ++k) {
        const int e = tid + k * WM_THR, v = e >> 3, f = e & 7;
        const int hy = v / WM_EW, wx = v % WM_EW;
        xhw[k] = e < WM_EH * WM_EW * 8 ? (hy << 16 | wx) : -1;
        xoff[k] = (unsigned)(((hy * a.W + wx) * a.CF + cfb * 32 + 4 * f) * 4);
        xpos[k] = (4 * f) * WM_CHP + hy * WM_EWP + wx;
    }
    const int gv = tid >> 3, gf = tid & 7;
    const int glh = gv / WM_TW, glw = gv % WM_TW;
    const unsigned goff = (unsigned)(((glh * a.W + glw) * a.CC + ccb * 32 + 4 * gf) * 4);
    const int gpos = (4 * gf) * WM_GP + glh * WM_TW + glw;
    const long long plane = (long long)a.H * a.W;
    float4 bsc, bsh, bmu, bis, bgm, bsg, bsx;
    if constexpr (BN) {
        const int c4 = ccb * 32 + 4 * gf;
        bsc = stx_ld4(a.bn_scale + c4); bsh = stx_ld4(a.bn_shift + c4); bmu = stx_ld4(a.bn_mean + c4);
        bis = stx_ld4(a.bn_invstd + c4); bsg = stx_ld4(a.bn_sum_g + c4); bsx = stx_ld4(a.bn_sum_gx + c4);
        bgm = a.bn_gamma ? stx_ld4(a.bn_gamma + c4) : make_float4(1.f, 1.f, 1.f, 1.f);
    }

    const int grp8 = (wave >> 1) * WM_EWP + 8 * (wave & 1);
    const int grp8g = (wave >> 1) * WM_TW + 8 * (wave & 1);
    const int xlane = i * WM_CHP + 4 * half, glane = i * WM_GP + 4 * half;

    const long long s0 = a.nsteps * blockIdx.x / gridDim.x, s1 = a.nsteps * (blockIdx.x + 1) / gridDim.x;
    long long s = s0;
    while (s < s1) {
        const int col = (int)(s / a.D), ob = (int)(s - (long long)col * a.D);
        const int oe = (int)((long long)a.D - ob < s1 - s ? a.D : ob + (s1 - s));
        int r = col;
        const int wt = r % a.nWt; r /= a.nWt;
        const int ht = r % a.nHt;
        const int b = r / a.nHt;
        const int oh0 = ht * WM_TH, ow0 = wt * WM_TW;
        unsigned xvo[WM_NPX];
#pragma unroll
        for (int k = 0; k < WM_NPX; ++k) {
            const int gh = oh0 - 1 + (xhw[k] >> 16), gw = ow0 - 1 + (xhw[k] & 0xffff);
            xvo[k] = (xhw[k] >= 0 && gh >= 0 && gh < a.H && gw >= 0 && gw < a.W) ? xoff[k] : STX_BUF_OOB;
        }
        const unsigned gvo = (oh0 + glh < a.H && ow0 + glw < a.W) ? goff : STX_BUF_OOB;
        const long long xorg = (long long)(oh0 - 1) * a.W + (ow0 - 1), gorg = (long long)oh0 * a.W + ow0;

        float4 sx[WM_NPX], sg, sz;
        auto load_x = [&](int p) {
            const bool in = p >= 0 && p < a.D;
            const stx_bufrsrc rs = stx_make_rsrc(a.x + (((long long)b * a.D + (in ? p : 0)) * plane + xorg) * a.CF,
                                                 in ? (unsigned)((plane - xorg) * a.CF * 4) : 0u);
#pragma unroll
            for (int k = 0; k < WM_NPX; ++k) sx[k] = stx_buf_ld4(rs, xvo[k], 0u);
        };
        auto load_g = [&](int p) {
            const bool in = p >= 0 && p < a.D;
            const stx_bufrsrc rs = stx_make_rsrc(a.gy + (((long long)b * a.D + (in ? p : 0)) * plane + gorg) * a.CC,
                                                 in ? (unsigned)((plane - gorg) * a.CC * 4) : 0u);
            sg = stx_buf_ld4(rs, gvo, 0u);
            if constexpr (BN) {
                const stx_bufrsrc rz = stx_make_rsrc(a.z + (((long long)b * a.D + (in ? p : 0)) * plane + gorg) * a.CC,
                                                     in ? (unsigned)((plane - gorg) * a.CC * 4) : 0u);
                sz = stx_buf_ld4(rz, gvo, 0u);
            }
        };
        auto bn_apply_staged = [&](int p) {
            float4 g = sg;
            if (a.bn_act) {
                g.x = stx_act_bwd(g.x, fmaf(sz.x, bsc.x, bsh.x), a.bn_act); g.y = stx_act_bwd(g.y, fmaf(sz.y, bsc.y, bsh.y), a.bn_act);
                g.z = stx_act_bwd(g.z, fmaf(sz.z, bsc.z, bsh.z), a.bn_act); g.w = stx_act_bwd(g.w, fmaf(sz.w, bsc.w, bsh.w), a.bn_act);
            }
            const float n1 = a.bn_inv_n;
            float4 d;
            d.x = bgm.x * bis.x * (g.x - bsg.x * n1 - (sz.x - bmu.x) * bis.x * bsx.x * n1);
            d.y = bgm.y * bis.y * (g.y - bsg.y * n1 - (sz.y - bmu.y) * bis.y * bsx.y * n1);
            d.z = bgm.z * bis.z * (g.z - bsg.z * n1 - (sz.z - bmu.z) * bis.z * bsx.z * n1);
            d.w = bgm.w * bis.w * (g.w - bsg.w * n1 - (sz.w - bmu.w) * bis.w * bsx.w * n1);
            if (gvo == STX_BUF_OOB) d = make_float4(0.f, 0.f, 0.f, 0.f);
            else if (cfb == 0) stx_st4(a.dz + (((long long)b * a.D + p) * plane + gorg) * a.CC + (goff >> 2), d);
            sg = d;
        };
        auto store_x = [&](int p) {
            float* dst = xl + (p & 3) * WM_XPLANE;
#pragma unroll
            for (int k = 0; k < WM_NPX; ++k)
                if (xhw[k] >= 0) {
                    float* q = dst + xpos[k];
                    q[0] = sx[k].x; q[WM_CHP] = sx[k].y; q[2 * WM_CHP] = sx[k].z; q[3 * WM_CHP] = sx[k].w;
                }
        };
        auto store_g = [&](int p) {
            if constexpr (BN) bn_apply_staged(p);
            float* q = gl + (p & 1) * WM_GPLANE + gpos;
            q[0] = sg.x; q[WM_GP] = sg.y; q[2 * WM_GP] = sg.z; q[3 * WM_GP] = sg.w;
        };

        for (int p = ob - 1; p <= ob + 1; ++p) { load_x(p); store_x(p); }
        load_g(ob);
        store_g(ob);
        __syncthreads();

        for (int o = ob; o < oe; ++o) {
            const bool more = o + 1 < oe;
            {
                const bool in = more && o + 2 < a.D;
                const stx_bufrsrc rs = stx_make_rsrc(a.x + (((long long)b * a.D + (in ? o + 2 : 0)) * plane + xorg) * a.CF,
                                                     in ? (unsigned)((plane - xorg) * a.CF * 4) : 0u);
#pragma unroll
                for (int k = 0; k < WM_NPX; ++k) sx[k] = stx_buf_ld4(rs, xvo[k], 0u);
                const stx_bufrsrc rg = stx_make_rsrc(a.gy + (((long long)b * a.D + (more ? o + 1 : 0)) * plane + gorg) * a.CC,
                                                     more ? (unsigned)((plane - gorg) * a.CC * 4) : 0u);
                sg = stx_buf_ld4(rg, gvo, 0u);
                if constexpr (BN) {
                    const stx_bufrsrc rz = stx_make_rsrc(a.z + (((long long)b * a.D + (more ? o + 1 : 0)) * plane + gorg) * a.CC,
                                                         more ? (unsigned)((plane - gorg) * a.CC * 4) : 0u);
                    sz = stx_buf_ld4(rz, gvo, 0u);
                }
            }
            const float* xa = xl + ((o + kdw - 1) & 3) * WM_XPLANE + khw * WM_EWP + xlane;
            const float* x8 = xl + ((o + 1) & 3) * WM_XPLANE + 2 * WM_EWP + grp8 + xlane;
            const float* gb = gl + (o & 1) * WM_GPLANE + glane;
            float4 A0[2], A1[2], Bv[2];
            A0[0] = stx_ld4(xa); A1[0] = stx_ld4(xa + 4); Bv[0] = stx_ld4(gb);
#pragma unroll
            for (int q = 0; q < 8; ++q) {
                const int cb = q & 1, nb = cb ^ 1;
                if (q < 7) {
                    const int h = (q + 1) >> 1, w8 = (q + 1) & 1;
                    A0[nb] = stx_ld4(xa + h * WM_EWP + 8 * w8);
                    A1[nb] = stx_ld4(xa + h * WM_EWP + 8 * w8 + 4);
                    Bv[nb] = stx_ld4(gb + h * WM_TW + 8 * w8);
                } else {
                    A0[nb] = stx_ld4(x8);
                    A1[nb] = stx_ld4(x8 + 4);
                    Bv[nb] = stx_ld4(gb + grp8g);
                }
                STX_SCHED_BARRIER();
                const float av[6] = {A0[cb].x, A0[cb].y, A0[cb].z, A0[cb].w, A1[cb].x, A1[cb].y};
                const float bv[4] = {Bv[cb].x, Bv[cb].y, Bv[cb].z, Bv[cb].w};
#pragma unroll
                for (int j = 0; j < 4; ++j)
#pragma unroll
                    for (int kw = 0; kw < 3; ++kw)
                        acc[kw] = __builtin_amdgcn_mfma_f32_32x32x2f32(av[j + kw], bv[j], acc[kw], 0, 0, 0);
                STX_SCHED_BARRIER();
                if (q == 4) {
                    if (more) { store_x(o + 2); store_g(o + 1); }
                    STX_SCHED_BARRIER();
                }
            }
            {
                const float av[6] = {A0[0].x, A0[0].y, A0[0].z, A0[0].w, A1[0].x, A1[0].y};
                const float bv[4] = {Bv[0].x, Bv[0].y, Bv[0].z, Bv[0].w};
#pragma unroll
                for (int j = 0; j < 4; ++j)
#pragma unroll
                    for (int kw = 0; kw < 3; ++kw)
                        acc8[kw] = __builtin_amdgcn_mfma_f32_32x32x2f32(av[j + kw], bv[j], acc8[kw], 0, 0, 0);
            }
            __syncthreads();
        }
        s += oe - ob;
    }

    float* dst = a.slab + ((size_t)blockIdx.y * gridDim.x + blockIdx.x) * 27 * 1024;
#pragma unroll
// ... 170 lines not shown
            float4 E0[2], O0[2], Bv[2];
            float E1[2];
            E0[0] = stx_ld4(xa); E1[0] = xa[4]; O0[0] = stx_ld4(xa + 20); Bv[0] = stx_ld4(gb);
#pragma unroll
            for (int q = 0; q < 8; ++q) {
                const int cb = q & 1, nb = cb ^ 1;
                if (q < 7) {
                    const int h = (q + 1) >> 1, w8 = (q + 1) & 1;
                    const float* p = xa + (2 * h) * W2_RP + 8 * w8;
                    E0[nb] = stx_ld4(p); E1[nb] = p[4]; O0[nb] = stx_ld4(p + 20);
                    Bv[nb] = stx_ld4(gb + h * WM_TW + 8 * w8);
                } else {
                    E0[nb] = stx_ld4(x8); E1[nb] = x8[4]; O0[nb] = stx_ld4(x8 + 20);
                    Bv[nb] = stx_ld4(gb + grp8g);
                }
                if (ablate != 1) { if (q < W2_NPART) load_part(q); else if (q == W2_NPART) load_g(o + 1, more); }
                STX_SCHED_BARRIER();
                const float ev[5] = {E0[cb].x, E0[cb].y, E0[cb].z, E0[cb].w, E1[cb]};
                const float od[4] = {O0[cb].x, O0[cb].y, O0[cb].z, O0[cb].w};
                const float bv[4] = {Bv[cb].x, Bv[cb].y, Bv[cb].z, Bv[cb].w};
                if (ablate != 2) {
#pragma unroll
                for (int j = 0; j < 4; ++j) {
                    acc[0] = __builtin_amdgcn_mfma_f32_32x32x2f32(ev[j], bv[j], acc[0], 0, 0, 0);
                    acc[1] = __builtin_amdgcn_mfma_f32_32x32x2f32(od[j], bv[j], acc[1], 0, 0, 0);
                    acc[2] = __builtin_amdgcn_mfma_f32_32x32x2f32(ev[j + 1], bv[j], acc[2], 0, 0, 0);
                }
                }
                STX_SCHED_BARRIER();
            }
            {
                const float ev[5] = {E0[0].x, E0[0].y, E0[0].z, E0[0].w, E1[0]};
                const float od[4] = {O0[0].x, O0[0].y, O0[0].z, O0[0].w};
                const float bv[4] = {Bv[0].x, Bv[0].y, Bv[0].z, Bv[0].w};
#pragma unroll
                for (int j = 0; j < 4; ++j) {
                    acc8[0] = __builtin_amdgcn_mfma_f32_32x32x2f32(ev[j], bv[j], acc8[0], 0, 0, 0);
                    acc8[1] = __builtin_amdgcn_mfma_f32_32x32x2f32(od[j], bv[j], acc8[1], 0, 0, 0);
                    acc8[2] = __builtin_amdgcn_mfma_f32_32x32x2f32(ev[j + 1], bv[j], acc8[2], 0, 0, 0);
                }
            }
            __syncthreads();
            if (more && ablate != 3) { store_planes(2 * o + 2, 2 * o + 3, true); store_g(o + 1); }
            __syncthreads();
        }
        s += oe - ob;
    }

    float* dst = a.slab + ((size_t)blockIdx.y * gridDim.x + blockIdx.x) * 27 * 1024;
#pragma unroll
    for (int kw = 0; kw < 3; ++kw)
#pragma unroll
        for (int r = 0; r < 16; ++r) {
            const int cf = (r & 3) + 8 * (r >> 2) + 4 * half;
            dst[(size_t)(wave * 3 + kw) * 1024 + cf * 32 + i] = acc[kw][r];
        }
    float* red = reinterpret_cast<float*>(smem);
#pragma unroll
    for (int kw = 0; kw < 3; ++kw) {
        __syncthreads();
#pragma unroll
        for (int r = 0; r < 16; ++r) {
            const int cf = (r & 3) + 8 * (r >> 2) + 4 * half;
            red[wave * 1024 + cf * 32 + i] = acc8[kw][r];
        }
        __syncthreads();
        for (int e = tid; e < 1024; e += WM_THR) {
            float t = red[e];
#pragma unroll
            for (int w = 1; w < WM_NW; ++w) t += red[w * 1024 + e];
            dst[(size_t)(24 + kw) * 1024 + e] = t;
        }
    }
}

}

struct StxWgradBn {
    const float* z; float* dz;
    const float *scale, *shift, *mean, *invstd, *gamma, *sum_g, *sum_gx;
    float inv_n; int act;
};

int stx_wgrad_march_launch(const float* x, const float* gy, float* slab, int B, int D, int H, int W, int CF, int CC,
                           int nchunks, void* stream, const StxWgradBn* bn) {
    if (CF % 32 || CC % 32 || B < 1 || D < 1 || H < 1 || W < 1) return -1;
    if ((long long)H * W * CF * 4 >= (1ll << 31) || (long long)H * W * CC * 4 >= (1ll << 31)) return -1;
    WmArgs a;
    a.x = x; a.gy = gy; a.slab = slab; a.B = B; a.D = D; a.H = H; a.W = W; a.CF = CF; a.CC = CC;
    a.z = nullptr; a.dz = nullptr;
    a.bn_scale = a.bn_shift = a.bn_mean = a.bn_invstd = a.bn_gamma = a.bn_sum_g = a.bn_sum_gx = nullptr;
    a.bn_inv_n = 0.f; a.bn_act = 0;
    if (bn) {
        a.z = bn->z; a.dz = bn->dz; a.bn_scale = bn->scale; a.bn_shift = bn->shift; a.bn_mean = bn->mean; a.bn_invstd = bn->invstd;
        a.bn_gamma = bn->gamma; a.bn_sum_g = bn->sum_g; a.bn_sum_gx = bn->sum_gx; a.bn_inv_n = bn->inv_n; a.bn_act = bn->act;
    }
    a.nHt = stx_cdiv(H, WM_TH); a.nWt = stx_cdiv(W, WM_TW);
    const long long ncols = (long long)B * a.nHt * a.nWt;
    if (ncols >= (1ll << 31)) return -1;
    a.ncols = (int)ncols;
    a.nsteps = ncols * D;
    const int npairs = (CF / 32) * (CC / 32);
    void (*kern)(WmArgs) = bn ? conv3d_wgrad_march_kernel<true> : conv3d_wgrad_march_kernel<false>;
    if (int rc = stx_lds_require((const void*)kern, WM_LDS_BYTES, "conv3d_wgrad(march)")) return rc;
    hipLaunchKernelGGL(kern, dim3(nchunks, npairs), dim3(WM_THR), WM_LDS_BYTES, (hipStream_t)stream, a);
    return stx_check_launch("conv3d_wgrad(march)");
}

int stx_wgrad_march_s2_launch(const float* f, const float* c, float* slab, int B, int Df, int Hf, int Wf, int CF, int Dc, int Hc,
                              int Wc, int CC, int nchunks, void* stream) {
    if (CF % 32 || CC % 32 || B < 1 || Dc < 1 || Hc < 1 || Wc < 1) return -1;
    if ((long long)Df * Hf * Wf * CF * 4 >= (1ll << 32) || (long long)Hc * Wc * CC * 4 >= (1ll << 31)) return -1;
    WmArgs a = {};
    a.x = f; a.gy = c; a.slab = slab; a.B = B; a.D = Dc; a.H = Hc; a.W = Wc; a.CF = CF; a.CC = CC;
    a.nHt = stx_cdiv(Hc, WM_TH); a.nWt = stx_cdiv(Wc, WM_TW);
    const long long ncols = (long long)B * a.nHt * a.nWt;
    if (ncols >= (1ll << 31)) return -1;
    a.ncols = (int)ncols;
    a.nsteps = ncols * Dc;
    const int npairs = (CF / 32) * (CC / 32);
    if (int rc = stx_lds_require((const void*)conv3d_wgrad_march_s2_kernel, W2_LDS_BYTES, "conv3d_wgrad(march s2)")) return rc;
    hipLaunchKernelGGL(conv3d_wgrad_march_s2_kernel, dim3(nchunks, npairs), dim3(WM_THR), W2_LDS_BYTES, (hipStream_t)stream, a,
                       Df, Hf, Wf, stx_tune(STX_TUNE_WGRAD_ABLATE));
    return stx_check_launch("conv3d_wgrad(march s2)");
}

int stx_wgrad_march_chunks(int B, int D, int H, int W, int npairs) {
    const long long nsteps = (long long)B * stx_cdiv(H, WM_TH) * stx_cdiv(W, WM_TW) * D;
    long long c = 256 / npairs;
    if (c < 1) c = 1;
    if (c > nsteps) c = nsteps;
    return (int)c;
}
```

stereo_toolbox_amd/models/GwcNet/gwcnet.py:

```python
import torch
import torch.nn as nn

from ... import ops
from ...aggregation import conv_block, convbn_block, deferred_bn_counters, shared_input_convs
from ..features2d import ResTrunk, cat_features, channels_last_weights_, convbn, init_reference_style, run_head2d, run_pair
from .submodule import convbn_3d


class feature_extraction(ResTrunk):
    fused_everywhere = True

    def __init__(self, concat_feature=False, concat_feature_channel=12):
        super().__init__()
        self.concat_feature = concat_feature
        if concat_feature:
            self.lastconv = nn.Sequential(convbn(320, 128, 3, 1, 1, 1), nn.ReLU(inplace=True),
                                          nn.Conv2d(128, concat_feature_channel, 1, bias=False))

    def forward(self, x):
        gwc = cat_features(self.trunk(x))
        if not self.concat_feature:
            return {"gwc_feature": gwc}
        return {"gwc_feature": gwc, "concat_feature": run_head2d(self.lastconv, gwc)}


class hourglass(nn.Module):

    def __init__(self, c):
        super().__init__()
        self.conv1 = nn.Sequential(convbn_3d(c, c * 2, 3, 2, 1), nn.ReLU(inplace=True))
        self.conv2 = nn.Sequential(convbn_3d(c * 2, c * 2, 3, 1, 1), nn.ReLU(inplace=True))
        self.conv3 = nn.Sequential(convbn_3d(c * 2, c * 4, 3, 2, 1), nn.ReLU(inplace=True))
        self.conv4 = nn.Sequential(convbn_3d(c * 4, c * 4, 3, 1, 1), nn.ReLU(inplace=True))
        self.conv5 = nn.Sequential(nn.ConvTranspose3d(c * 4, c * 2, 3, padding=1, output_padding=1, stride=2, bias=False),
                                   nn.BatchNorm3d(c * 2))
        self.conv6 = nn.Sequential(nn.ConvTranspose3d(c * 2, c, 3, padding=1, output_padding=1, stride=2, bias=False),
                                   nn.BatchNorm3d(c))
        self.redir1 = convbn_3d(c, c, kernel_size=1, stride=1, pad=0)
        self.redir2 = convbn_3d(c * 2, c * 2, kernel_size=1, stride=1, pad=0)

    def forward(self, x, mid=None, also=None):
        rx = shared_input_convs(x, [self.conv1[0], self.redir1] + ([also] if also is not None else []))
        rx = rx or [None, None, None]
        c1 = convbn_block(x, self.conv1[0], relu=True, raw=rx[0])
        c2 = convbn_block(c1, self.conv2[0], relu=True)
        r2 = shared_input_convs(c2, [self.conv3[0], self.redir2]) or [None, None]
        c3 = convbn_block(c2, self.conv3[0], relu=True, raw=r2[0])
        c4 = convbn_block(c3, self.conv4[0], relu=True)
        if mid is not None:
            c4 = mid(c4)
        c5 = convbn_block(c4, self.conv5, relu=True, second=(c2, self.redir2), second_raw=r2[1])
        out = convbn_block(c5, self.conv6, relu=True, second=(x, self.redir1), second_raw=rx[1])
        return (out, rx[2]) if also is not None else out


def classifier(c):
    return nn.Sequential(convbn_3d(c, c, 3, 1, 1), nn.ReLU(inplace=True),
                         nn.Conv3d(c, 1, kernel_size=3, padding=1, stride=1, bias=False))


def run_classifier(seq, x, add=None, raw=None):
    h = convbn_block(x, seq[0], relu=True, raw=raw)
    cost = conv_block(h, seq[2], residual=None if add is None else add.unsqueeze(-1))
    return cost.squeeze(-1)


class GwcNet(nn.Module):
    def __init__(self, maxdisp, use_concat_volume=False):
        super().__init__()
        self.maxdisp = maxdisp
        self.use_concat_volume = use_concat_volume
        self.num_groups = 40
        if use_concat_volume:
            self.concat_channels = 12
            self.feature_extraction = feature_extraction(True, self.concat_channels)
        else:
            self.concat_channels = 0
            self.feature_extraction = feature_extraction(False)
        self.dres0 = nn.Sequential(convbn_3d(self.num_groups + self.concat_channels * 2, 32, 3, 1, 1),
                                   nn.ReLU(inplace=True), convbn_3d(32, 32, 3, 1, 1), nn.ReLU(inplace=True))
        self.dres1 = nn.Sequential(convbn_3d(32, 32, 3, 1, 1), nn.ReLU(inplace=True), convbn_3d(32, 32, 3, 1, 1))
        self.dres2 = hourglass(32)
        self.dres3 = hourglass(32)
        self.dres4 = hourglass(32)
        self.classif0 = classifier(32)
        self.classif1 = classifier(32)
        self.classif2 = classifier(32)
        self.classif3 = classifier(32)
        init_reference_style(self)
        channels_last_weights_(self.feature_extraction)

    def forward(self, left, right):
        with deferred_bn_counters():
            fl, fr = run_pair(self.feature_extraction, left, right, self.training)
            return self.aggregate(fl, fr, left.shape[2], left.shape[3])

    @ops.fp32_region
    def aggregate(self, fl, fr, H, W):
        vol = ops.cost_volume(fl["gwc_feature"], fr["gwc_feature"], fl.get("concat_feature"),
                              fr.get("concat_feature"), self.maxdisp // 4, self.num_groups, mask_left=True)
        cost0 = convbn_block(vol, self.dres0[0], relu=True)
        cost0 = convbn_block(cost0, self.dres0[2], relu=True)
        t = convbn_block(cost0, self.dres1[0], relu=True)
        cost0 = convbn_block(t, self.dres1[2], relu=False, residual=cost0)
        if self.training:
            out1, r0 = self.dres2(cost0, also=self.classif0[0])
            out2, r1 = self.dres3(out1, also=self.classif1[0])
            out3, r2 = self.dres4(out2, also=self.classif2[0])
            return [ops.regression_head(run_classifier(c, o, raw=r), self.maxdisp, H, W)
                    for c, o, r in ((self.classif0, cost0, r0), (self.classif1, out1, r1), (self.classif2, out2, r2),
                                    (self.classif3, out3, None))]
        out1 = self.dres2(cost0)
        out2 = self.dres3(out1)
        out3 = self.dres4(out2)
        return ops.regression_head(run_classifier(self.classif3, out3), self.maxdisp, H, W)


def GwcNet_G(d=192):
    return GwcNet(d, use_concat_volume=False)


def GwcNet_GC(d=192):
    return GwcNet(d, use_concat_volume=True)
```

stereo_toolbox_amd/ops.py:

```python
import ctypes

import torch

from ._capi import StxError, get_lib

_P = ctypes.c_void_p


class _DevPtr(ctypes.c_void_p):
    """A device pointer that remembers the device of the tensor it came from: _call() reads the launch device off its
    own arguments, so nothing survives between launches (an exception between building the arguments and the launch
    cannot leak state into the next one)."""


def _stream(dev=None):
    return _P(torch.cuda.current_stream(dev).cuda_stream)


def _p(t):
    if t is None:
        return None
    p = _DevPtr(t.data_ptr())
    p.dev = t.device
    return p
# ... 210 lines not shown
    n = get_lib().raw("stx_conv3d_wgrad_workspace_floats")(B, D, H, W, CF, CC, 3, 1)
    ws = _WS.get("wgrad", n, x.device)
    dw = torch.empty(CC, CF, 27, dtype=torch.float32, device=x.device)
    dz = torch.empty_like(gy)
    _call("stx_conv3d_wgrad_bn", _p(x), _p(gy), _p(pend.z), _p(pend.scale), _p(pend.shift), _p(pend.mean), _p(pend.invstd),
          _p(pend.gamma), _p(pend.sums), float(pend.inv_n), int(pend.act), _p(dz), _p(dw), _p(ws), B, D, H, W, CF, CC)
    return dw, dz


class _PendingBn:
    __slots__ = ("g", "z", "scale", "shift", "mean", "invstd", "gamma", "sums", "inv_n", "act")

    def materialize(self):
        C = self.z.shape[-1]
        nvox = self.z.numel() // C
        dz = torch.empty_like(self.z)
        _call("stx_bn_bwd_apply2", _p(self.g), None, _p(self.z), _p(self.mean), _p(self.invstd), _p(self.gamma), None, None,
              None, None, _p(self.scale), _p(self.shift), None, None, _p(self.sums), _p(dz), None, None, nvox, C, int(self.act), 1)
        return dz


_BN_DEFER = {"outstanding": 0, "armed": False}


def _bn_defer_check():
    n, _BN_DEFER["outstanding"], _BN_DEFER["armed"] = _BN_DEFER["outstanding"], 0, False
    if n:
        raise StxError(f"{n} deferred BatchNorm-backward record(s) were not consumed by their convolution's backward node: "
                       "the gradients of this backward pass are wrong (set STX_BN_BWD_IN_WGRAD=0 and report)")


def _defer_pending_bn(g, pend):
    g._stx_pending_bn = pend
    _BN_DEFER["outstanding"] += 1
    if not _BN_DEFER["armed"]:
        _BN_DEFER["armed"] = True
        torch.autograd.Variable._execution_engine.queue_callback(_bn_defer_check)


def bn_defer_reset_if_stale():
    if not _BN_DEFER["armed"]:
        return
    task_id = getattr(torch._C, "_current_graph_task_id", None)
    if task_id is None or task_id() == -1:
        _BN_DEFER["outstanding"], _BN_DEFER["armed"] = 0, False


def _take_pending_bn(g):
    pend = getattr(g, "_stx_pending_bn", None) if g is not None else None
    if pend is not None:
        del g._stx_pending_bn
        _BN_DEFER["outstanding"] -= 1
        if pend.g is not g:
            raise StxError("deferred BatchNorm backward: record attached to a different gradient tensor")
    return pend


def _is_c1(w, ks, stride, transposed):
    return (not transposed) and ks == 3 and stride == 1 and w.shape[0] == 1 and w.shape[1] % 16 == 0 and w.shape[1] <= 64


def conv3d_c1_forward(x, w, residual=None):
    _chk(x, "x", 5)
    _chk(w, "weight", 5)
    B, D, H, W, Cin = x.shape
    out = torch.empty(B, D, H, W, 1, dtype=torch.float32, device=x.device)
    _call("stx_conv3d_c1_fwd", _p(x), _p(w), _p(residual), _p(out), B, D, H, W, Cin)
    return out


def conv3d_c1_wgrad(x, gy):
    B, D, H, W, Cin = x.shape
    ws = _WS.get("c1wgrad", get_lib().raw("stx_conv3d_c1_wgrad_workspace_floats")(Cin), x.device)
    dw = torch.empty(1, Cin, 3, 3, 3, dtype=torch.float32, device=x.device)
    _call("stx_conv3d_c1_wgrad", _p(x), _p(gy), _p(dw), _p(ws), B, D, H, W, Cin)
    return dw


def conv3d_c1_dgrad(gy, w, Cin):
    B, D, H, W, _ = gy.shape
    gx = torch.empty(B, D, H, W, Cin, dtype=torch.float32, device=gy.device)
    _call("stx_conv3d_c1_dgrad", _p(gy), _p(w), _p(gx), B, D, H, W, Cin)
    return gx


class ConvRawFn(torch.autograd.Function):

    @staticmethod
    def forward(ctx, x, w, ks, stride, transposed, want_stats):
        _chk(x, "x", 5)
        ctx.cin_true = None
        ctx.x_prepadded = False
        if not transposed and x.shape[-1] != w.shape[1]:
            if x.shape[-1] != (w.shape[1] + 7) // 8 * 8:
                raise StxError(f"conv: input has {x.shape[-1]} channels, weight expects {w.shape[1]}")
            ctx.cin_true, ctx.x_prepadded = w.shape[1], True
            w = pad_weight_channels(w, x.shape[-1])
        elif not transposed and x.shape[-1] % 8 != 0:
            ctx.cin_true = x.shape[-1]
            x, w = pad_input_channels(x, w)
        if _is_c1(w, ks, stride, transposed) and not want_stats:
            z, stats = conv3d_c1_forward(x, w.contiguous()), None
        elif transposed:
            Cout = w.shape[1]
            z, stats = deconv3d_forward(x, pack_weight(w, 2), Cout, want_stats=want_stats)
        else:
            Cout = w.shape[0]
            z, stats = conv3d_forward(x, pack_weight(w, 0), Cout, ks, stride, want_stats=want_stats)
        ctx.save_for_backward(x, w)
        ctx.cfg = (ks, stride, transposed)
        if stats is None:
            stats = x.new_empty(0)
        ctx.mark_non_differentiable(stats)
        return z, stats

    @staticmethod
    def backward(ctx, gz, _gstats):
        x, w = ctx.saved_tensors
        ks, stride, transposed = ctx.cfg
        pend = _take_pending_bn(gz)
        gx = gw = None
        B, D, H, W, Cin = x.shape
        if pend is not None:
            if (ctx.needs_input_grad[1] and not transposed and ks == 3 and stride == 1 and ctx.cin_true is None
                    and get_lib().raw("stx_conv3d_wgrad_bn_supported")(B, D, H, W, Cin, w.shape[0])):
                gw_pre, gz = conv3d_wgrad_bn(x, gz, pend)
                gw_pre = gw_pre.reshape(w.shape)
            else:
                gw_pre, gz = None, pend.materialize()
        else:
            gw_pre = None
        gz = gz.contiguous()
        if transposed:
            Ci, Co = w.shape[0], w.shape[1]
            if ctx.needs_input_grad[0]:
                gx, _ = conv3d_forward(gz, pack_weight(w, 0), Ci, 3, 2)
            if ctx.needs_input_grad[1]:
                gz_w = gz if Co % 32 == 0 else _pad_channels(gz, (Co + 31) // 32 * 32)
                x_w = x if Ci % 32 == 0 else _pad_channels(x, (Ci + 31) // 32 * 32)
                gw = conv3d_wgrad(gz_w, x_w, 3, 2)[:Ci, :Co].reshape(w.shape)
        else:
            Co, Ci = w.shape[0], w.shape[1]
            c1 = _is_c1(w, ks, stride, transposed)
            gz_k, w_k = gz, w
            if Co % 8 != 0 and not c1:
                Cp = (Co + 7) // 8 * 8
                gz_k = _pad_channels(gz, Cp)
                w_k = w.new_zeros(Cp, *w.shape[1:])
                w_k[:Co] = w
            if ctx.needs_input_grad[0]:
                if c1:
                    gx = conv3d_c1_dgrad(gz, w.contiguous(), Ci)
                elif stride == 1 and Ci > 128:
                    parts = []
                    for lo in range(0, Ci, 128):
                        hi = min(Ci, lo + 128)
                        g, _ = conv3d_forward(gz_k, pack_weight(w_k[:, lo:hi].contiguous(), 1), hi - lo, ks, 1)
                        parts.append(g)
                    gx = torch.cat(parts, -1)
                elif stride == 1:
                    gx, _ = conv3d_forward(gz_k, pack_weight(w_k, 1), Ci, ks, 1)
                else:
                    if Co % 32:
                        Cp = (Co + 31) // 32 * 32
                        gz_k = _pad_channels(gz, Cp)
                        w_k = w.new_zeros(Cp, *w.shape[1:])
# ... 2762 lines not shown
```

Baseline: 0.1785 pairs/s.

## Fuse BatchNorm+ReLU application into the consuming 3D conv's input load (fwd and wgrad)

Adds 'on-load' variants of the march 3D conv forward, the 1-channel classifier conv, and the weight-gradient kernels. These apply the previous layer's BatchNorm scale/shift and ReLU while loading input tiles, so the normalized activation tensor is never materialized. GwcNet's dres0/dres1 chains and classifiers are routed through a new BnActConvFn autograd function. This is meant to remove a full read-write pass over large 4D cost volumes in both forward and backward. In exchange it recomputes the affine+ReLU in every consumer kernel, adds template variants, and falls back to the old path when a shape is unsupported.

```diff
diff --git a/include/stx_hip.h b/include/stx_hip.h
--- a/include/stx_hip.h
+++ b/include/stx_hip.h
@@ -53,6 +53,18 @@
 int stx_conv3d_wgrad_bn(const float* x, const float* gy, const float* z, const float* scale, const float* shift, const float* mean,
                         const float* invstd, const float* gamma, const float* sums, float inv_n, int act, float* dz, float* dw,
                         float* workspace, int B, int D, int H, int W, int CF, int CC, void* stream);
+
+int stx_conv3d_fwd_onload_supported(int B, int Di, int Hi, int Wi, int Cin, int Cout);
+int stx_conv3d_fwd_onload(const float* x, const float* in_scale, const float* in_shift, int in_act, const float* wp, float* out,
+                          const float* scale, const float* bias, const float* residual, float* stats, int B, int Di, int Hi,
+                          int Wi, int Cin, int Cout, int relu, void* stream);
+int stx_conv3d_wgrad_onload_supported(int B, int D, int H, int W, int CF, int CC);
+int stx_conv3d_wgrad_onload(const float* x, const float* x_scale, const float* x_shift, int x_act, const float* gy, float* dw,
+                            float* workspace, int B, int D, int H, int W, int CF, int CC, void* stream);
+int stx_conv3d_wgrad_bn_onload(const float* x, const float* x_scale, const float* x_shift, int x_act, const float* gy,
+                               const float* z, const float* scale, const float* shift, const float* mean, const float* invstd,
+                               const float* gamma, const float* sums, float inv_n, int act, float* dz, float* dw,
+                               float* workspace, int B, int D, int H, int W, int CF, int CC, void* stream);
 
 int stx_conv3d_axial_supported(int Cin, int Cout, int kd, int kh, int kw);
 long long stx_conv3d_axial_packed_floats(int K, int N, int kd, int kh, int kw);
@@ -95,6 +107,11 @@
 int stx_conv3d_c1_wgrad(const float* x, const float* gy, float* dw, float* workspace, int B, int D, int H, int W,
                         int Cin, void* stream);
 int stx_conv3d_c1_dgrad(const float* gy, const float* w, float* gx, int B, int D, int H, int W, int Cin, void* stream);
+int stx_conv3d_c1_onload_supported(int B, int D, int H, int W, int Cin);
+int stx_conv3d_c1_fwd_onload(const float* x, const float* in_scale, const float* in_shift, int in_act, const float* w,
+                             const float* residual, float* out, int B, int D, int H, int W, int Cin, void* stream);
+int stx_conv3d_c1_wgrad_onload(const float* x, const float* in_scale, const float* in_shift, int in_act, const float* gy,
+                               float* dw, float* workspace, int B, int D, int H, int W, int Cin, void* stream);
 
 int stx_mish_fwd(const float* x, float* y, long long n, void* stream);
 int stx_mish_bwd(const float* gy, const float* x, float* gx, long long n, void* stream);
diff --git a/stereo_toolbox_amd/_capi.py b/stereo_toolbox_amd/_capi.py
--- a/stereo_toolbox_amd/_capi.py
+++ b/stereo_toolbox_amd/_capi.py
@@ -40,6 +40,14 @@
     "stx_conv3d_wgrad": [_P, _P, _P, _P, _I, _I, _I, _I, _I, _I, _I, _I, _I, _I, _I, _P],
     "stx_conv3d_wgrad_bn_supported": [_I, _I, _I, _I, _I, _I],
     "stx_conv3d_wgrad_bn": [_P] * 9 + [_F, _I, _P, _P, _P, _I, _I, _I, _I, _I, _I, _P],
+    "stx_conv3d_fwd_onload_supported": [_I, _I, _I, _I, _I, _I],
+    "stx_conv3d_fwd_onload": [_P, _P, _P, _I, _P, _P, _P, _P, _P, _P, _I, _I, _I, _I, _I, _I, _I, _P],
+    "stx_conv3d_wgrad_onload_supported": [_I, _I, _I, _I, _I, _I],
+    "stx_conv3d_wgrad_onload": [_P, _P, _P, _I, _P, _P, _P, _I, _I, _I, _I, _I, _I, _P],
+    "stx_conv3d_wgrad_bn_onload": [_P, _P, _P, _I] + [_P] * 8 + [_F, _I, _P, _P, _P, _I, _I, _I, _I, _I, _I, _P],
+    "stx_conv3d_c1_onload_supported": [_I, _I, _I, _I, _I],
+    "stx_conv3d_c1_fwd_onload": [_P, _P, _P, _I, _P, _P, _P, _I, _I, _I, _I, _I, _P],
+    "stx_conv3d_c1_wgrad_onload": [_P, _P, _P, _I, _P, _P, _P, _I, _I, _I, _I, _I, _P],
     "stx_conv3d_axial_supported": [_I, _I, _I, _I, _I],
     "stx_conv3d_axial_packed_floats": [_I, _I, _I, _I, _I],
     "stx_conv3d_axial_pack_weight": [_P, _P, _I, _I, _I, _I, _I, _I, _P],
diff --git a/stereo_toolbox_amd/aggregation.py b/stereo_toolbox_amd/aggregation.py
--- a/stereo_toolbox_amd/aggregation.py
+++ b/stereo_toolbox_amd/aggregation.py
@@ -210,6 +210,37 @@
     return ops.BnActFn.apply(z1, bn.weight, bn.bias, None, None, None, residual, relu, st1, None, 1, defer)
 
 
+def _plain_conv3(conv):
+    return (isinstance(conv, nn.Conv3d) and not _is_transposed(conv) and tuple(conv.kernel_size) == (3, 3, 3)
+            and tuple(conv.stride) == (1, 1, 1) and tuple(conv.padding) == (1, 1, 1) and tuple(conv.dilation) == (1, 1, 1)
+            and conv.groups == 1 and conv.bias is None)
+
+
+@ops.fp32_region
+def bn_act_conv(x, seq, consumer, relu=True, raw=None, want_stats=False):
+    conv, bn = seq[0], seq[1]
+    if not torch.is_grad_enabled() or not isinstance(bn, nn.BatchNorm3d) or isinstance(bn, nn.SyncBatchNorm) or not bn.training:
+        return None
+    if not (_plain_conv3(conv) and _plain_conv3(consumer)) or bn.weight is None or bn.bias is None:
+        return None
+    if not all(p.requires_grad for p in (conv.weight, bn.weight, bn.bias, consumer.weight)):
+        return None
+    src = raw[0] if raw is not None else x
+    C = conv.weight.shape[0]
+    if src.dim() != 5 or src.dtype != torch.float32 or C != 32 or consumer.weight.shape[1] != C \
+            or src.shape[-1] != (C if raw is not None else conv.weight.shape[1]) or src.shape[-1] % 8:
+        return None
+    if not ops.bn_on_load_enabled() or not ops.bn_on_load_supported((*src.shape[:4], C), consumer.weight):
+        return None
+    z, part = raw if raw is not None else _raw_conv(x, conv, True)
+    st = _bn_state(bn, part, z.numel() // C)
+    defer = conv.weight.shape[1] % 32 == 0 and os.environ.get("STX_BN_BWD_IN_WGRAD", "1") != "0"
+    if defer:
+        ops.bn_defer_reset_if_stale()
+    out, stats = ops.BnActConvFn.apply(z, bn.weight, bn.bias, consumer.weight, 1 if relu else 0, st, bool(want_stats), defer)
+    return out, (stats if want_stats else None)
+
+
 def _axial_cfg(conv):
     if not isinstance(conv, nn.Conv3d) or _is_transposed(conv):
         raise ops.StxError("axial_conv_block: expected an nn.Conv3d")
diff --git a/stereo_toolbox_amd/csrc/conv3d.hip b/stereo_toolbox_amd/csrc/conv3d.hip
--- a/stereo_toolbox_amd/csrc/conv3d.hip
+++ b/stereo_toolbox_amd/csrc/conv3d.hip
@@ -466,6 +466,8 @@
     int os, oo, ncout;
     int wq_total, wq_off, wnt_total, wnt_off;
     const float* acc_in;
+    const float *in_scale, *in_shift;
+    int in_act;
 };
 
 constexpr int MW2_MW = 16, MW2_R = 2, MW2_TH = 8, MW2_EH = 10, MW2_EW = 18, MW2_VS = 36;
@@ -473,7 +475,7 @@
 constexpr int MW2_NF4 = (MW2_EH * MW2_EW * 8 + 255) / 256;
 constexpr int MW2_WFLOATS = 27 * 4 * 256;
 
-template <int BS, int EPI = 1>
+template <int BS, int EPI = 1, bool XBN = false>
 __global__ __launch_bounds__(256) void conv3d_marchw_kernel(MarchArgs ma) {
     const ConvArgs& a = ma.c;
     STX_DYN_SMEM(smem);
@@ -520,8 +522,12 @@
             if (ohb + dh < a.Ho && owb + c < a.Wo && n_lane() < ma.ncout) ovalid |= 1u << r;
         }
     };
+    float4 xsc = make_float4(1.f, 1.f, 1.f, 1.f), xsh = make_float4(0.f, 0.f, 0.f, 0.f);
+    if constexpr (XBN) { xsc = stx_ld4(ma.in_scale + ma.xo + 4 * (tid & 7)); xsh = stx_ld4(ma.in_shift + ma.xo + 4 * (tid & 7)); }
+    bool stg_in = false;
     auto load_plane = [&](int pd, bool on) {
         const bool in = on && pd >= 0 && pd < a.Di;
+        stg_in = in;
         const stx_bufrsrc rs = stx_make_rsrc(a.x + ((size_t)b * a.Di + (in ? pd : 0)) * a.Hi * a.Wi * ma.xs, in ? xplane_bytes : 0u);
 #pragma unroll
         for (int k = 0; k < MW2_NF4; ++k) stg[k] = stx_buf_ld4(rs, svoff[k], 0u);
@@ -531,6 +537,7 @@
         for (int k = 0; k < MW2_NF4; ++k) {
             const int idx = tid + k * 256;
             const int v = idx >> 3, f = idx & 7;
+            if constexpr (XBN) stg[k] = stx_bn_onload4(stg[k], xsc, xsh, ma.in_act, stg_in && svoff[k] != STX_BUF_OOB);
             if (v < MW2_EH * MW2_EW) stx_st4(buf + v * MW2_VS + 4 * f, stg[k]);
         }
     };
@@ -1139,7 +1146,14 @@
          : wn == 2 ? conv3d_pgemm_kernel<3, S, CONV_TD, CONV_TH, 4, 8, 2> : conv3d_pgemm_kernel<3, S, CONV_TD, CONV_TH, 4, 8>;
 }
 
-void (*march_kernel(int bs, int epi))(MarchArgs) {
+void (*march_kernel(int bs, int epi, bool xbn = false))(MarchArgs) {
+    if (xbn) {
+        switch (epi) {
+        case 4: return bs ? conv3d_marchw_kernel<1, 4, true> : conv3d_marchw_kernel<0, 4, true>;
+        case 5: return bs ? conv3d_marchw_kernel<1, 5, true> : conv3d_marchw_kernel<0, 5, true>;
+        default: return bs ? conv3d_marchw_kernel<1, 1, true> : conv3d_marchw_kernel<0, 1, true>;
+        }
+    }
     switch (epi) {
     case 0: return bs ? conv3d_marchw_kernel<1, 0> : conv3d_marchw_kernel<0, 0>;
     case 2: return bs ? conv3d_marchw_kernel<1, 2> : conv3d_marchw_kernel<0, 2>;
@@ -1240,10 +1254,15 @@
     return conv_plan(B, Di, Hi, Wi, Cin, Cout, ks, stride).rows;
 }
 
-extern "C" int stx_conv3d_fwd(const float* x, const float* wp, float* out, const float* scale, const float* bias,
-                              const float* residual, float* stats, int B, int Di, int Hi, int Wi, int Cin, int Cout,
-                              int ks, int stride, int relu, void* stream) {
+extern "C" int stx_conv3d_fwd_onload_supported(int B, int Di, int Hi, int Wi, int Cin, int Cout) {
     stx_begin();
+    return B > 0 && Di > 0 && Hi > 0 && Wi > 0 && Cin == 32 && Cout >= 1 && Cout <= 64 &&
+           conv_plan(B, Di, Hi, Wi, Cin, Cout, 3, 1).kind == 0;
+}
+
+static int conv3d_fwd_impl(const float* x, const float* in_scale, const float* in_shift, int in_act, const float* wp, float* out,
+                           const float* scale, const float* bias, const float* residual, float* stats, int B, int Di, int Hi,
+                           int Wi, int Cin, int Cout, int ks, int stride, int relu, void* stream) {
     STX_REQUIRE(x && wp && out && B > 0 && Di > 0 && Hi > 0 && Wi > 0, "conv3d_fwd: bad shape");
     STX_REQUIRE(Cin % 8 == 0 && Cout >= 1 && Cout <= 128, "conv3d_fwd: Cin=%d (need %%8) Cout=%d (need <=128)", Cin, Cout);
     STX_REQUIRE((ks == 3 && (stride == 1 || stride == 2)) || (ks == 1 && stride == 1),
@@ -1266,6 +1285,8 @@
         m2.c.nWt = stx_cdiv(a.Wo, MW2_MW);
         m2.ncols = B * m2.c.nHt * m2.c.nWt;
         m2.ablate = stx_tune(STX_TUNE_MARCH_ABLATE);
+        m2.in_scale = in_scale; m2.in_shift = in_shift; m2.in_act = in_act;
+        const bool xbn = in_scale != nullptr;
         {
             const int nb2 = plan.march_wgs;
             const size_t lds2 = ((size_t)MW2_WFLOATS + 2 * (size_t)MW2_SLOT) * 4;
@@ -1284,12 +1305,14 @@
                     }
                     const bool plain = epi_fast && !(m.c.residual && m.acc_in) && m.c.relu < 2;
                     const bool raw = !m.acc_in && !m.c.residual && !m.c.scale && !m.c.bias && m.c.relu == 0;
-                    const int epi = plain ? (raw ? (whole && m.ncout == 32 ? 5 : 4) : m.acc_in ? 2 : (m.c.residual ? 3 : 0)) : 1;
-                    if (int rc = launch_with_lds(march_kernel(bs, epi), dim3(nb2), lds2, st, m)) return rc;
+                    int epi = plain ? (raw ? (whole && m.ncout == 32 ? 5 : 4) : m.acc_in ? 2 : (m.c.residual ? 3 : 0)) : 1;
+                    if (xbn && epi != 4 && epi != 5) epi = 1;
+                    if (int rc = launch_with_lds(march_kernel(bs, epi, xbn), dim3(nb2), lds2, st, m)) return rc;
                 }
             return stx_check_launch("conv3d_fwd(march)");
         }
     }
+    STX_REQUIRE(!in_scale, "conv3d_fwd_onload: shape not served (ask stx_conv3d_fwd_onload_supported)");
     STX_REQUIRE(halo_range_ok(Di, Hi, Wi, Cin), "conv3d_fwd: a batch item of %d x %d x %d x %d floats exceeds the 2 GiB "
                 "buffer-descriptor range", Di, Hi, Wi, Cin);
     const int CK = (stride == 2) ? 8 : conv_pick_ck(Cin, ks);
@@ -1316,6 +1339,25 @@
     else rc = conv_dispatch<1, 1>(a, NT, CK, grid, st);
     if (rc) return rc;
     return stx_check_launch("conv3d_fwd");
+}
+
+extern "C" int stx_conv3d_fwd(const float* x, const float* wp, float* out, const float* scale, const float* bias,
+                              const float* residual, float* stats, int B, int Di, int Hi, int Wi, int Cin, int Cout,
+                              int ks, int stride, int relu, void* stream) {
+    stx_begin();
+    return conv3d_fwd_impl(x, nullptr, nullptr, 0, wp, out, scale, bias, residual, stats, B, Di, Hi, Wi, Cin, Cout, ks, stride, relu,
+                           stream);
+}
+
+extern "C" int stx_conv3d_fwd_onload(const float* x, const float* in_scale, const float* in_shift, int in_act, const float* wp,
+                                     float* out, const float* scale, const float* bias, const float* residual, float* stats, int B,
+                                     int Di, int Hi, int Wi, int Cin, int Cout, int relu, void* stream) {
+    stx_begin();
+    STX_REQUIRE(in_scale && in_shift && (in_act == 0 || in_act == 1), "conv3d_fwd_onload: scale / shift / activation code %d", in_act);
+    STX_REQUIRE(stx_conv3d_fwd_onload_supported(B, Di, Hi, Wi, Cin, Cout), "conv3d_fwd_onload: shape (%d x %d x %d x %d, %d -> %d "
+                "channels) not served", B, Di, Hi, Wi, Cin, Cout);
+    return conv3d_fwd_impl(x, in_scale, in_shift, in_act, wp, out, scale, bias, residual, stats, B, Di, Hi, Wi, Cin, Cout, 3, 1, relu,
+                           stream);
 }
 
 extern "C" int stx_deconv3d_fwd(const float* x, const float* wp, float* out, const float* scale, const float* bias,
@@ -1361,8 +1403,11 @@
     const float *scale, *shift, *mean, *invstd, *gamma, *sum_g, *sum_gx;
     float inv_n; int act;
 };
+struct StxWgradXbn {
+    const float *scale, *shift; int act;
+};
 int stx_wgrad_march_launch(const float* x, const float* gy, float* slab, int B, int D, int H, int W, int CF, int CC, int nchunks,
-                           void* stream, const StxWgradBn* bn);
+                           void* stream, const StxWgradBn* bn, const StxWgradXbn* xbn);
 int stx_wgrad_march_chunks(int B, int D, int H, int W, int npairs);
 int stx_wgrad_march_s2_launch(const float* f, const float* c, float* slab, int B, int Df, int Hf, int Wf, int CF, int Dc, int Hc,
                               int Wc, int CC, int nchunks, void* stream);
@@ -1410,7 +1455,7 @@
         int mc = stx_wgrad_march_chunks(B, Dc, Hc, Wc, npairs);
         const int forced = stx_tune(STX_TUNE_WGRAD_GRID);
         if (forced > 0 && forced < mc) mc = forced;
-        const int rc = stride == 1 ? stx_wgrad_march_launch(f, c, workspace, B, Dc, Hc, Wc, CF, CC, mc, stream, nullptr)
+        const int rc = stride == 1 ? stx_wgrad_march_launch(f, c, workspace, B, Dc, Hc, Wc, CF, CC, mc, stream, nullptr, nullptr)
                                    : stx_wgrad_march_s2_launch(f, c, workspace, B, Df, Hf, Wf, CF, Dc, Hc, Wc, CC, mc, stream);
         if (rc > 0) return rc;
         if (rc == 0) {
@@ -1454,6 +1499,23 @@
            (long long)B * stx_cdiv(H, 4) * stx_cdiv(W, 16) < (1ll << 31);
 }
 
+static int wgrad_march_forms(const char* who, const float* x, const float* gy, float* dw, float* workspace, int B, int D, int H, int W,
+                             int CF, int CC, void* stream, const StxWgradBn* bn, const StxWgradXbn* xbn) {
+    STX_REQUIRE(stx_conv3d_wgrad_bn_supported(B, D, H, W, CF, CC), "%s: shape (%d x %d x %d x %d, %d -> %d channels) is "
+                "not served by the march kernel (ask stx_conv3d_wgrad_bn_supported)", who, B, D, H, W, CF, CC);
+    const int npairs = (CF / 32) * (CC / 32);
+    int mc = stx_wgrad_march_chunks(B, D, H, W, npairs);
+    const int forced = stx_tune(STX_TUNE_WGRAD_GRID);
+    if (forced > 0 && forced < mc) mc = forced;
+    const int rc = stx_wgrad_march_launch(x, gy, workspace, B, D, H, W, CF, CC, mc, stream, bn, xbn);
+    if (rc > 0) return rc;
+    STX_REQUIRE(rc == 0, "%s: the march kernel refused the shape", who);
+    const int total = npairs * 27 * 1024;
+    hipLaunchKernelGGL(conv3d_wgrad_reduce4_kernel, dim3(total / 64), dim3(CONV_THREADS), 0, (hipStream_t)stream, workspace, dw, CF,
+                       CC, 27, mc, 27);
+    return stx_check_launch("conv3d_wgrad_reduce");
+}
+
 extern "C" int stx_conv3d_wgrad_bn(const float* x, const float* gy, const float* z, const float* scale, const float* shift,
                                    const float* mean, const float* invstd, const float* gamma, const float* sums, float inv_n,
                                    int act, float* dz, float* dw, float* workspace, int B, int D, int H, int W, int CF, int CC,
@@ -1461,20 +1523,39 @@
     stx_begin();
     STX_REQUIRE(x && gy && z && scale && shift && mean && invstd && sums && dz && dw && workspace, "conv3d_wgrad_bn: null operand");
     STX_REQUIRE(act == 0 || act == 1, "conv3d_wgrad_bn: activation code %d (0 or 1)", act);
-    STX_REQUIRE(stx_conv3d_wgrad_bn_supported(B, D, H, W, CF, CC), "conv3d_wgrad_bn: shape (%d x %d x %d x %d, %d -> %d channels) is "
-                "not served by the march kernel (ask stx_conv3d_wgrad_bn_supported)", B, D, H, W, CF, CC);
-    const int npairs = (CF / 32) * (CC / 32);
-    int mc = stx_wgrad_march_chunks(B, D, H, W, npairs);
-    const int forced = stx_tune(STX_TUNE_WGRAD_GRID);
-    if (forced > 0 && forced < mc) mc = forced;
     StxWgradBn bn;
     bn.z = z; bn.dz = dz; bn.scale = scale; bn.shift = shift; bn.mean = mean; bn.invstd = invstd; bn.gamma = gamma;
     bn.sum_g = sums; bn.sum_gx = sums + CC; bn.inv_n = inv_n; bn.act = act;
-    const int rc = stx_wgrad_march_launch(x, gy, workspace, B, D, H, W, CF, CC, mc, stream, &bn);
-    if (rc > 0) return rc;
-    STX_REQUIRE(rc == 0, "conv3d_wgrad_bn: the march kernel refused the shape");
-    const int total = npairs * 27 * 1024;
-    hipLaunchKernelGGL(conv3d_wgrad_reduce4_kernel, dim3(total / 64), dim3(CONV_THREADS), 0, (hipStream_t)stream, workspace, dw, CF,
-                       CC, 27, mc, 27);
-    return stx_check_launch("conv3d_wgrad_reduce");
-}
+    return wgrad_march_forms("conv3d_wgrad_bn", x, gy, dw, workspace, B, D, H, W, CF, CC, stream, &bn, nullptr);
+}
+
+extern "C" int stx_conv3d_wgrad_onload_supported(int B, int D, int H, int W, int CF, int CC) {
+    return CF == 32 && stx_conv3d_wgrad_bn_supported(B, D, H, W, CF, CC);
+}
+
+extern "C" int stx_conv3d_wgrad_onload(const float* x, const float* x_scale, const float* x_shift, int x_act, const float* gy,
+                                       float* dw, float* workspace, int B, int D, int H, int W, int CF, int CC, void* stream) {
+    stx_begin();
+    STX_REQUIRE(x && x_scale && x_shift && gy && dw && workspace, "conv3d_wgrad_onload: null operand");
+    STX_REQUIRE(x_act == 0 || x_act == 1, "conv3d_wgrad_onload: activation code %d (0 or 1)", x_act);
+    STX_REQUIRE(CF == 32, "conv3d_wgrad_onload: %d fine channels (32 are served)", CF);
+    const StxWgradXbn xbn = {x_scale, x_shift, x_act};
+    return wgrad_march_forms("conv3d_wgrad_onload", x, gy, dw, workspace, B, D, H, W, CF, CC, stream, nullptr, &xbn);
+}
+
+extern "C" int stx_conv3d_wgrad_bn_onload(const float* x, const float* x_scale, const float* x_shift, int x_act, const float* gy,
+                                          const float* z, const float* scale, const float* shift, const float* mean,
+                                          const float* invstd, const float* gamma, const float* sums, float inv_n, int act, float* dz,
+                                          float* dw, float* workspace, int B, int D, int H, int W, int CF, int CC, void* stream) {
+    stx_begin();
+    STX_REQUIRE(x && x_scale && x_shift && gy && z && scale && shift && mean && invstd && sums && dz && dw && workspace,
+                "conv3d_wgrad_bn_onload: null operand");
+    STX_REQUIRE((act == 0 || act == 1) && (x_act == 0 || x_act == 1), "conv3d_wgrad_bn_onload: activation codes %d, %d (0 or 1)", act,
+                x_act);
+    STX_REQUIRE(CF == 32, "conv3d_wgrad_bn_onload: %d fine channels (32 are served)", CF);
+    StxWgradBn bn;
+    bn.z = z; bn.dz = dz; bn.scale = scale; bn.shift = shift; bn.mean = mean; bn.invstd = invstd; bn.gamma = gamma;
+    bn.sum_g = sums; bn.sum_gx = sums + CC; bn.inv_n = inv_n; bn.act = act;
+    const StxWgradXbn xbn = {x_scale, x_shift, x_act};
+    return wgrad_march_forms("conv3d_wgrad_bn_onload", x, gy, dw, workspace, B, D, H, W, CF, CC, stream, &bn, &xbn);
+}
diff --git a/stereo_toolbox_amd/csrc/conv_c1.hip b/stereo_toolbox_amd/csrc/conv_c1.hip
--- a/stereo_toolbox_amd/csrc/conv_c1.hip
+++ b/stereo_toolbox_amd/csrc/conv_c1.hip
@@ -266,11 +266,13 @@
 constexpr int C1M_ED = C1M_TD + 2, C1M_EH = C1M_TH + 2, C1M_EW = C1M_TW + 2;
 constexpr int C1M_BLOCKS = 1024;
 
+template <bool XBN>
 __global__ __launch_bounds__(C1_THREADS) void conv_c1_wgrad_mfma_kernel(const float* __restrict__ x,
                                                                         const float* __restrict__ gy,
                                                                         float* __restrict__ slab, int B, int D, int H,
                                                                         int W, int Cin, int nDt, int nHt, int nWt,
-                                                                        int ntiles) {
+                                                                        int ntiles, const float* __restrict__ in_scale,
+                                                                        const float* __restrict__ in_shift, int in_act) {
     __shared__ float gys[C1M_ED * C1M_EH * C1M_EW];
     __shared__ float red[4][1024];
     const int tid = threadIdx.x, lane = tid & 63, wave = tid >> 6;
@@ -278,6 +280,8 @@
     const int cb = blockIdx.y;
     const int kd = i / 9, kh = (i / 3) % 3, kw = i % 3;
     const int toff = (i < 27) ? ((2 - kd) * C1M_EH + (2 - kh)) * C1M_EW + (2 - kw) + half : half;
+    float xsc = 1.f, xsh = 0.f;
+    if constexpr (XBN) { xsc = in_scale[cb * 32 + i]; xsh = in_shift[cb * 32 + i]; }
     f32x16 acc;
 #pragma unroll
     for (int r = 0; r < 16; ++r) acc[r] = 0.f;
@@ -305,8 +309,11 @@
             const float* xr = x + ((((size_t)b * D + gd) * H + gh) * W + w0 + half) * Cin + cb * 32 + i;
             float av[16];
 #pragma unroll
-            for (int p = 0; p < 16; ++p)
-                av[p] = (rowok && w0 + 2 * p + half < W) ? xr[(size_t)(2 * p) * Cin] : 0.f;
+            for (int p = 0; p < 16; ++p) {
+                const bool ok = rowok && w0 + 2 * p + half < W;
+                av[p] = ok ? xr[(size_t)(2 * p) * Cin] : 0.f;
+                if constexpr (XBN) av[p] = stx_bn_onload(av[p], xsc, xsh, in_act, ok);
+            }
             const float* gp = gys + (ld * C1M_EH + lh) * C1M_EW + toff;
 #pragma unroll
             for (int p = 0; p < 16; ++p) {
@@ -347,11 +354,14 @@
 constexpr int C1F_MT = (C1F_NV + 31) / 32;
 constexpr int C1F_WGS = 512;
 
+template <bool XBN>
 __global__ __launch_bounds__(C1_THREADS) void conv_c1_fwd_mfma_kernel(const float* __restrict__ x,
                                                                       const float* __restrict__ w,
                                                                       const float* __restrict__ res,
                                                                       float* __restrict__ out, int B, int D, int H, int W,
-                                                                      int nHt, int nWt, int ncols) {
+                                                                      int nHt, int nWt, int ncols,
+                                                                      const float* __restrict__ in_scale,
+                                                                      const float* __restrict__ in_shift, int in_act) {
     STX_DYN_SMEM(smem);
     float* Ps = reinterpret_cast<float*>(smem);
     const int tid = threadIdx.x, lane = tid & 63, wave = __builtin_amdgcn_readfirstlane(tid >> 6);
@@ -360,6 +370,11 @@
 #pragma unroll
     for (int s_ = 0; s_ < 16; ++s_) wreg[s_] = (i < 27) ? w[(size_t)(16 * half + s_) * 27 + i] : 0.f;
     const int lh = tid / C1F_TW, lw = tid % C1F_TW;
+    float4 xsc[4], xsh[4];
+    if constexpr (XBN) {
+#pragma unroll
+        for (int q = 0; q < 4; ++q) { xsc[q] = stx_ld4(in_scale + 16 * half + 4 * q); xsh[q] = stx_ld4(in_shift + 16 * half + 4 * q); }
+    }
 
     constexpr int MTW = (C1F_MT + 3) / 4;
     const long long units = (long long)ncols * D;
@@ -411,6 +426,11 @@
                 for (int t = 0; t < MTW; ++t) {
                     const int m = wave + 4 * t;
                     if (m < C1F_MT) {
+                        if constexpr (XBN) {
+#pragma unroll
+                            for (int q = 0; q < 4; ++q)
+                                cur[t][q] = stx_bn_onload4(cur[t][q], xsc[q], xsh[q], in_act, voff[t] != STX_BUF_OOB);
+                        }
                         f32x16 acc;
 #pragma unroll
                         for (int r = 0; r < 16; ++r) acc[r] = 0.f;
@@ -458,9 +478,15 @@
 
 }
 
-extern "C" int stx_conv3d_c1_fwd(const float* x, const float* w, const float* residual, float* out, int B, int D,
-                                 int H, int W, int Cin, void* stream) {
+extern "C" int stx_conv3d_c1_onload_supported(int B, int D, int H, int W, int Cin) {
     stx_begin();
+    return B > 0 && D > 0 && H > 0 && W > 0 && Cin == 32 && (long long)H * W * 128 < (1ll << 31) &&
+           (long long)B * stx_cdiv(H, C1F_TH) * stx_cdiv(W, C1F_TW) * D < (1ll << 31) &&
+           (long long)B * stx_cdiv(D, C1M_TD) * stx_cdiv(H, C1M_TH) * stx_cdiv(W, C1M_TW) < (1ll << 31);
+}
+
+static int c1_fwd(const float* x, const float* in_scale, const float* in_shift, int in_act, const float* w,
+                  const float* residual, float* out, int B, int D, int H, int W, int Cin, void* stream) {
     STX_REQUIRE(x && w && out && B > 0 && D > 0 && H > 0 && W > 0, "conv3d_c1_fwd: bad shape");
     STX_REQUIRE(Cin % C1_CK == 0, "conv3d_c1_fwd: Cin=%d must be a multiple of %d", Cin, C1_CK);
     if (Cin == 32 && (long long)H * W * 128 < (1ll << 31)) {
@@ -470,11 +496,14 @@
         long long g = C1F_WGS;
         if (g > units / 4) g = units / 4 > 0 ? units / 4 : 1;
         const size_t lds = (size_t)2 * C1F_NV * 27 * 4;
-        if (int rc = stx_lds_require((const void*)conv_c1_fwd_mfma_kernel, lds, "conv3d_c1_fwd(mfma)")) return rc;
-        hipLaunchKernelGGL(conv_c1_fwd_mfma_kernel, dim3((unsigned)g), dim3(C1_THREADS), lds, (hipStream_t)stream, x, w,
-                           residual, out, B, D, H, W, nHt, nWt, (int)ncols);
+        void (*kern)(const float*, const float*, const float*, float*, int, int, int, int, int, int, int, const float*,
+                     const float*, int) = in_scale ? conv_c1_fwd_mfma_kernel<true> : conv_c1_fwd_mfma_kernel<false>;
+        if (int rc = stx_lds_require((const void*)kern, lds, "conv3d_c1_fwd(mfma)")) return rc;
+        hipLaunchKernelGGL(kern, dim3((unsigned)g), dim3(C1_THREADS), lds, (hipStream_t)stream, x, w, residual, out, B, D, H, W,
+                           nHt, nWt, (int)ncols, in_scale, in_shift, in_act);
         return stx_check_launch("conv3d_c1_fwd(mfma)");
     }
+    STX_REQUIRE(!in_scale, "conv3d_c1_fwd_onload: shape not served (ask stx_conv3d_c1_onload_supported)");
     C1Args a;
     a.x = x; a.w = w; a.gy = nullptr; a.res = residual; a.out = out;
     a.B = B; a.D = D; a.H = H; a.W = W; a.Cin = Cin;
@@ -485,15 +514,30 @@
     return stx_check_launch("conv3d_c1_fwd");
 }
 
+extern "C" int stx_conv3d_c1_fwd(const float* x, const float* w, const float* residual, float* out, int B, int D,
+                                 int H, int W, int Cin, void* stream) {
+    stx_begin();
+    return c1_fwd(x, nullptr, nullptr, 0, w, residual, out, B, D, H, W, Cin, stream);
+}
+
+extern "C" int stx_conv3d_c1_fwd_onload(const float* x, const float* in_scale, const float* in_shift, int in_act,
+                                        const float* w, const float* residual, float* out, int B, int D, int H, int W,
+                                        int Cin, void* stream) {
+    stx_begin();
+    STX_REQUIRE(in_scale && in_shift && (in_act == 0 || in_act == 1), "conv3d_c1_fwd_onload: scale / shift / activation code %d",
+                in_act);
+    STX_REQUIRE(stx_conv3d_c1_onload_supported(B, D, H, W, Cin), "conv3d_c1_fwd_onload: shape not served");
+    return c1_fwd(x, in_scale, in_shift, in_act, w, residual, out, B, D, H, W, Cin, stream);
+}
+
 extern "C" long long stx_conv3d_c1_wgrad_workspace_floats(int Cin) {
     const long long valu = (long long)C1_WGRAD_BLOCKS * Cin * 27;
     const long long mfma = (long long)C1M_BLOCKS * 1024 * ((Cin + 31) / 32);
     return valu > mfma ? valu : mfma;
 }
 
-extern "C" int stx_conv3d_c1_wgrad(const float* x, const float* gy, float* dw, float* workspace, int B, int D, int H,
-                                   int W, int Cin, void* stream) {
-    stx_begin();
+static int c1_wgrad(const float* x, const float* in_scale, const float* in_shift, int in_act, const float* gy, float* dw,
+                    float* workspace, int B, int D, int H, int W, int Cin, void* stream) {
     STX_REQUIRE(x && gy && dw && workspace && B > 0, "conv3d_c1_wgrad: null operand");
     STX_REQUIRE(Cin % C1_CK == 0 && Cin <= 4 * C1_CK, "conv3d_c1_wgrad: Cin=%d must be 16..64 in steps of 16", Cin);
     if (Cin % 32 == 0) {
@@ -502,13 +546,18 @@
         STX_REQUIRE(nt < (1ll << 31), "conv3d_c1_wgrad: volume too large");
         const int nblk = nt < C1M_BLOCKS ? (int)nt : C1M_BLOCKS;
         hipStream_t st = (hipStream_t)stream;
-        hipLaunchKernelGGL(conv_c1_wgrad_mfma_kernel, dim3(nblk, Cin / 32), dim3(C1_THREADS), 0, st, x, gy, workspace, B,
-                           D, H, W, Cin, nDt, nHt, nWt, (int)nt);
+        if (in_scale)
+            hipLaunchKernelGGL(conv_c1_wgrad_mfma_kernel<true>, dim3(nblk, Cin / 32), dim3(C1_THREADS), 0, st, x, gy, workspace,
+                               B, D, H, W, Cin, nDt, nHt, nWt, (int)nt, in_scale, in_shift, in_act);
+        else
+            hipLaunchKernelGGL(conv_c1_wgrad_mfma_kernel<false>, dim3(nblk, Cin / 32), dim3(C1_THREADS), 0, st, x, gy, workspace,
+                               B, D, H, W, Cin, nDt, nHt, nWt, (int)nt, in_scale, in_shift, in_act);
         int rc = stx_check_launch("conv3d_c1_wgrad(mfma)");
         if (rc) return rc;
         hipLaunchKernelGGL(c1m_reduce_kernel, dim3(Cin * 27), dim3(C1_THREADS), 0, st, workspace, nblk, dw);
         return stx_check_launch("conv3d_c1_wgrad(reduce)");
     }
+    STX_REQUIRE(!in_scale, "conv3d_c1_wgrad_onload: shape not served (ask stx_conv3d_c1_onload_supported)");
     C1Args a;
     a.x = x; a.w = nullptr; a.gy = gy; a.res = nullptr; a.out = workspace;
     a.B = B; a.D = D; a.H = H; a.W = W; a.Cin = Cin;
@@ -524,6 +573,22 @@
     return stx_check_launch("conv3d_c1_colsum");
 }
 
+extern "C" int stx_conv3d_c1_wgrad(const float* x, const float* gy, float* dw, float* workspace, int B, int D, int H,
+                                   int W, int Cin, void* stream) {
+    stx_begin();
+    return c1_wgrad(x, nullptr, nullptr, 0, gy, dw, workspace, B, D, H, W, Cin, stream);
+}
+
+extern "C" int stx_conv3d_c1_wgrad_onload(const float* x, const float* in_scale, const float* in_shift, int in_act,
+                                          const float* gy, float* dw, float* workspace, int B, int D, int H, int W, int Cin,
+                                          void* stream) {
+    stx_begin();
+    STX_REQUIRE(in_scale && in_shift && (in_act == 0 || in_act == 1), "conv3d_c1_wgrad_onload: scale / shift / activation code %d",
+                in_act);
+    STX_REQUIRE(stx_conv3d_c1_onload_supported(B, D, H, W, Cin), "conv3d_c1_wgrad_onload: shape not served");
+    return c1_wgrad(x, in_scale, in_shift, in_act, gy, dw, workspace, B, D, H, W, Cin, stream);
+}
+
 extern "C" int stx_conv3d_c1_dgrad(const float* gy, const float* w, float* gx, int B, int D, int H, int W, int Cin,
                                    void* stream) {
     stx_begin();
diff --git a/stereo_toolbox_amd/csrc/stx_common.h b/stereo_toolbox_amd/csrc/stx_common.h
--- a/stereo_toolbox_amd/csrc/stx_common.h
+++ b/stereo_toolbox_amd/csrc/stx_common.h
@@ -141,6 +141,7 @@
     STX_TUNE_DWCONV_ROLL,
     STX_TUNE_C2_PAD,
     STX_TUNE_C2_ABLATE,
+    STX_TUNE_BN_ON_LOAD,
     STX_TUNE_COUNT
 };
 int stx_tune(StxTune id);
@@ -164,6 +165,15 @@
 __device__ __forceinline__ float stx_act(float v, int code) {
     return code == 1 ? (v > 0.f ? v : 0.f) : (code == 2 ? stx_mish(v) : (code == 3 ? (v > 0.f ? v : STX_LEAKY_SLOPE * v) : v));
 }
+__device__ __forceinline__ float stx_bn_onload(float z, float sc, float sh, int act, bool ok) {
+    const float v = fmaf(z, sc, sh);
+    const float y = act == 1 ? (v > 0.f ? v : 0.f) : v;
+    return ok ? y : 0.f;
+}
+__device__ __forceinline__ float4 stx_bn_onload4(float4 z, float4 sc, float4 sh, int act, bool ok) {
+    return make_float4(stx_bn_onload(z.x, sc.x, sh.x, act, ok), stx_bn_onload(z.y, sc.y, sh.y, act, ok),
+                       stx_bn_onload(z.z, sc.z, sh.z, act, ok), stx_bn_onload(z.w, sc.w, sh.w, act, ok));
+}
 __device__ __forceinline__ float stx_act_bwd(float g, float t, int code) {
     return code == 2 ? g * stx_mish_grad(t) : (code == 3 ? (t > 0.f ? g : STX_LEAKY_SLOPE * g) : (t > 0.f ? g : 0.f));
 }
diff --git a/stereo_toolbox_amd/csrc/stx_runtime.hip b/stereo_toolbox_amd/csrc/stx_runtime.hip
--- a/stereo_toolbox_amd/csrc/stx_runtime.hip
+++ b/stereo_toolbox_amd/csrc/stx_runtime.hip
@@ -50,7 +50,7 @@
 TuneEntry g_tune[TUNE_N] = {
     {"STX_MARCH_BS", 1}, {"STX_MARCH_EPI", 1}, {"STX_MARCH_ABLATE", 0}, {"STX_WGRAD_ABLATE", 0}, {"STX_WGRAD_MARCH", 3}, {"STX_WGRAD_GRID", 0}, {"STX_CONV_L1_MARCH", 0}, {"STX_CONV_S2_DENSE", 1}, {"STX_CONV_WN", 2},
     {"STX_CV_OLD", 0}, {"STX_CV_GRID", 0}, {"STX_CV_PF", 0}, {"STX_CV_UNITS", 1}, {"STX_CV_WIN", 0}, {"STX_CVB_OLD", 0}, {"STX_CVB_TEAM", 0}, {"STX_CVB_GRID", 0}, {"STX_CVB_NSET", 3},
-    {"STX_SV_BWD_V1", 0}, {"STX_DWCONV_ROLL", 1}, {"STX_C2_PAD", 8}, {"STX_C2_ABLATE", 0}, {"STX_DA_GRID", 0},
+    {"STX_SV_BWD_V1", 0}, {"STX_DWCONV_ROLL", 1}, {"STX_C2_PAD", 8}, {"STX_C2_ABLATE", 0}, {"STX_BN_ON_LOAD", 1}, {"STX_DA_GRID", 0},
 };
 struct TuneInit {
     TuneInit() {
diff --git a/stereo_toolbox_amd/csrc/wgrad_march.hip b/stereo_toolbox_amd/csrc/wgrad_march.hip
--- a/stereo_toolbox_amd/csrc/wgrad_march.hip
+++ b/stereo_toolbox_amd/csrc/wgrad_march.hip
@@ -27,6 +27,8 @@
     const float *bn_scale, *bn_shift, *bn_mean, *bn_invstd, *bn_gamma, *bn_sum_g, *bn_sum_gx;
     float bn_inv_n;
     int bn_act;
+    const float *x_scale, *x_shift;
+    int x_act;
 };
 
 __device__ __forceinline__ f32x16 wm_zero16() {
@@ -36,7 +38,7 @@
     return z;
 }
 
-template <bool BN>
+template <bool BN, bool XBN = false>
 __global__ __launch_bounds__(WM_THR) void conv3d_wgrad_march_kernel(WmArgs a) {
     STX_DYN_SMEM(smem);
     float* xl = reinterpret_cast<float*>(smem);
@@ -74,6 +76,8 @@
         bis = stx_ld4(a.bn_invstd + c4); bsg = stx_ld4(a.bn_sum_g + c4); bsx = stx_ld4(a.bn_sum_gx + c4);
         bgm = a.bn_gamma ? stx_ld4(a.bn_gamma + c4) : make_float4(1.f, 1.f, 1.f, 1.f);
     }
+    float4 xsc, xsh;
+    if constexpr (XBN) { xsc = stx_ld4(a.x_scale + cfb * 32 + 4 * (tid & 7)); xsh = stx_ld4(a.x_shift + cfb * 32 + 4 * (tid & 7)); }
 
     const int grp8 = (wave >> 1) * WM_EWP + 8 * (wave & 1);
     const int grp8g = (wave >> 1) * WM_TW + 8 * (wave & 1);
@@ -135,6 +139,11 @@
         };
         auto store_x = [&](int p) {
             float* dst = xl + (p & 3) * WM_XPLANE;
+            if constexpr (XBN) {
+                const bool pin = p >= 0 && p < a.D;
+#pragma unroll
+                for (int k = 0; k < WM_NPX; ++k) sx[k] = stx_bn_onload4(sx[k], xsc, xsh, a.x_act, pin && xvo[k] != STX_BUF_OOB);
+            }
 #pragma unroll
             for (int k = 0; k < WM_NPX; ++k)
                 if (xhw[k] >= 0) {
@@ -471,8 +480,12 @@
     float inv_n; int act;
 };
 
+struct StxWgradXbn {
+    const float *scale, *shift; int act;
+};
+
 int stx_wgrad_march_launch(const float* x, const float* gy, float* slab, int B, int D, int H, int W, int CF, int CC,
-                           int nchunks, void* stream, const StxWgradBn* bn) {
+                           int nchunks, void* stream, const StxWgradBn* bn, const StxWgradXbn* xbn) {
     if (CF % 32 || CC % 32 || B < 1 || D < 1 || H < 1 || W < 1) return -1;
     if ((long long)H * W * CF * 4 >= (1ll << 31) || (long long)H * W * CC * 4 >= (1ll << 31)) return -1;
     WmArgs a;
@@ -490,7 +503,10 @@
     a.ncols = (int)ncols;
     a.nsteps = ncols * D;
     const int npairs = (CF / 32) * (CC / 32);
-    void (*kern)(WmArgs) = bn ? conv3d_wgrad_march_kernel<true> : conv3d_wgrad_march_kernel<false>;
+    a.x_scale = a.x_shift = nullptr; a.x_act = 0;
+    if (xbn) { a.x_scale = xbn->scale; a.x_shift = xbn->shift; a.x_act = xbn->act; }
+    void (*kern)(WmArgs) = xbn ? (bn ? conv3d_wgrad_march_kernel<true, true> : conv3d_wgrad_march_kernel<false, true>)
+                               : (bn ? conv3d_wgrad_march_kernel<true> : conv3d_wgrad_march_kernel<false>);
     if (int rc = stx_lds_require((const void*)kern, WM_LDS_BYTES, "conv3d_wgrad(march)")) return rc;
     hipLaunchKernelGGL(kern, dim3(nchunks, npairs), dim3(WM_THR), WM_LDS_BYTES, (hipStream_t)stream, a);
     return stx_check_launch("conv3d_wgrad(march)");
diff --git a/stereo_toolbox_amd/models/GwcNet/gwcnet.py b/stereo_toolbox_amd/models/GwcNet/gwcnet.py
--- a/stereo_toolbox_amd/models/GwcNet/gwcnet.py
+++ b/stereo_toolbox_amd/models/GwcNet/gwcnet.py
@@ -2,7 +2,7 @@
 import torch.nn as nn
 
 from ... import ops
-from ...aggregation import conv_block, convbn_block, deferred_bn_counters, shared_input_convs
+from ...aggregation import bn_act_conv, conv_block, convbn_block, deferred_bn_counters, shared_input_convs
 from ..features2d import ResTrunk, cat_features, channels_last_weights_, convbn, init_reference_style, run_head2d, run_pair
 from .submodule import convbn_3d
 
@@ -60,9 +60,20 @@
 
 
 def run_classifier(seq, x, add=None, raw=None):
+    fused = bn_act_conv(x, seq[0], seq[2], relu=True, raw=raw)
+    if fused is not None:
+        cost = fused[0] if add is None else fused[0] + add.unsqueeze(-1)
+        return cost.squeeze(-1)
     h = convbn_block(x, seq[0], relu=True, raw=raw)
     cost = conv_block(h, seq[2], residual=None if add is None else add.unsqueeze(-1))
     return cost.squeeze(-1)
+
+
+def run_chain(x, first, second, relu=True, residual=None):
+    fused = bn_act_conv(x, first, second[0], relu=True, want_stats=second[1].training)
+    if fused is not None:
+        return convbn_block(None, second, relu=relu, residual=residual, raw=fused)
+    return convbn_block(convbn_block(x, first, relu=True), second, relu=relu, residual=residual)
 
 
 class GwcNet(nn.Module):
@@ -99,10 +110,8 @@
     def aggregate(self, fl, fr, H, W):
         vol = ops.cost_volume(fl["gwc_feature"], fr["gwc_feature"], fl.get("concat_feature"),
                               fr.get("concat_feature"), self.maxdisp // 4, self.num_groups, mask_left=True)
-        cost0 = convbn_block(vol, self.dres0[0], relu=True)
-        cost0 = convbn_block(cost0, self.dres0[2], relu=True)
-        t = convbn_block(cost0, self.dres1[0], relu=True)
-        cost0 = convbn_block(t, self.dres1[2], relu=False, residual=cost0)
+        cost0 = run_chain(vol, self.dres0[0], self.dres0[2], relu=True)
+        cost0 = run_chain(cost0, self.dres1[0], self.dres1[2], relu=False, residual=cost0)
         if self.training:
             out1, r0 = self.dres2(cost0, also=self.classif0[0])
             out2, r1 = self.dres3(out1, also=self.classif1[0])
diff --git a/stereo_toolbox_amd/ops.py b/stereo_toolbox_amd/ops.py
--- a/stereo_toolbox_amd/ops.py
+++ b/stereo_toolbox_amd/ops.py
@@ -316,6 +316,135 @@
     gx = torch.empty(B, D, H, W, Cin, dtype=torch.float32, device=gy.device)
     _call("stx_conv3d_c1_dgrad", _p(gy), _p(w), _p(gx), B, D, H, W, Cin)
     return gx
+
+
+def bn_on_load_enabled():
+    return get_lib().get_tuning("STX_BN_ON_LOAD") != 0
+
+
+def bn_on_load_supported(shape, w):
+    B, D, H, W, C = (int(s) for s in shape)
+    if w.dim() != 5 or tuple(w.shape[1:]) != (C, 3, 3, 3):
+        return False
+    raw = get_lib().raw
+    if w.shape[0] == 1:
+        return bool(raw("stx_conv3d_c1_onload_supported")(B, D, H, W, C))
+    Co = w.shape[0]
+    return Co % 32 == 0 and bool(raw("stx_conv3d_fwd_onload_supported")(B, D, H, W, C, Co)) \
+        and bool(raw("stx_conv3d_wgrad_onload_supported")(B, D, H, W, C, Co))
+
+
+def conv3d_forward_onload(z, scale, shift, act, wp, Cout, want_stats=False):
+    _chk(z, "z", 5)
+    B, D, H, W, Cin = z.shape
+    out = torch.empty(B, D, H, W, Cout, dtype=torch.float32, device=z.device)
+    stats = None
+    if want_stats:
+        rows = get_lib().raw("stx_conv3d_fwd_stat_rows")(B, D, H, W, Cin, Cout, 3, 1)
+        stats = torch.empty(rows, 2, Cout, dtype=torch.float32, device=z.device)
+    _call("stx_conv3d_fwd_onload", _p(z), _p(scale), _p(shift), int(act), _p(wp), _p(out), None, None, None, _p(stats), B, D, H, W,
+          Cin, Cout, 0)
+    return out, stats
+
+
+def conv3d_wgrad_onload(z, scale, shift, act, gy):
+    B, D, H, W, CF = z.shape
+    CC = gy.shape[-1]
+    ws = _WS.get("wgrad", get_lib().raw("stx_conv3d_wgrad_workspace_floats")(B, D, H, W, CF, CC, 3, 1), z.device)
+    dw = torch.empty(CC, CF, 27, dtype=torch.float32, device=z.device)
+    _call("stx_conv3d_wgrad_onload", _p(z), _p(scale), _p(shift), int(act), _p(gy), _p(dw), _p(ws), B, D, H, W, CF, CC)
+    return dw
+
+
+def conv3d_wgrad_bn_onload(z, scale, shift, act, gy, pend):
+    B, D, H, W, CF = z.shape
+    CC = gy.shape[-1]
+    ws = _WS.get("wgrad", get_lib().raw("stx_conv3d_wgrad_workspace_floats")(B, D, H, W, CF, CC, 3, 1), z.device)
+    dw = torch.empty(CC, CF, 27, dtype=torch.float32, device=z.device)
+    dz = torch.empty_like(gy)
+    _call("stx_conv3d_wgrad_bn_onload", _p(z), _p(scale), _p(shift), int(act), _p(gy), _p(pend.z), _p(pend.scale), _p(pend.shift),
+          _p(pend.mean), _p(pend.invstd), _p(pend.gamma), _p(pend.sums), float(pend.inv_n), int(pend.act), _p(dz), _p(dw), _p(ws),
+          B, D, H, W, CF, CC)
+    return dw, dz
+
+
+def conv3d_c1_forward_onload(z, scale, shift, act, w, residual=None):
+    _chk(z, "z", 5)
+    _chk(w, "weight", 5)
+    B, D, H, W, Cin = z.shape
+    out = torch.empty(B, D, H, W, 1, dtype=torch.float32, device=z.device)
+    _call("stx_conv3d_c1_fwd_onload", _p(z), _p(scale), _p(shift), int(act), _p(w), _p(residual), _p(out), B, D, H, W, Cin)
+    return out
+
+
+def conv3d_c1_wgrad_onload(z, scale, shift, act, gy):
+    B, D, H, W, Cin = z.shape
+    ws = _WS.get("c1wgrad", get_lib().raw("stx_conv3d_c1_wgrad_workspace_floats")(Cin), z.device)
+    dw = torch.empty(1, Cin, 3, 3, 3, dtype=torch.float32, device=z.device)
+    _call("stx_conv3d_c1_wgrad_onload", _p(z), _p(scale), _p(shift), int(act), _p(gy), _p(dw), _p(ws), B, D, H, W, Cin)
+    return dw
+
+
+class BnActConvFn(torch.autograd.Function):
+
+    @staticmethod
+    def forward(ctx, z, gamma, beta, w, act, bn, want_stats, defer):
+        _chk(z, "z", 5)
+        sc, sh, m, i = bn_finalize(bn["partials"], bn["count"], gamma, beta, bn["running_mean"], bn["running_var"],
+                                   bn["momentum"], bn["eps"])
+        act = int(act)
+        ctx.c1 = w.shape[0] == 1
+        if ctx.c1:
+            out, stats = conv3d_c1_forward_onload(z, sc, sh, act, w.contiguous()), None
+        else:
+            out, stats = conv3d_forward_onload(z, sc, sh, act, pack_weight(w, 0), w.shape[0], want_stats)
+        ctx.save_for_backward(z, gamma, m, i, sc, sh, w)
+        ctx.act, ctx.defer = act, bool(defer)
+        if stats is None:
+            stats = z.new_empty(0)
+        ctx.mark_non_differentiable(stats)
+        return out, stats
+
+    @staticmethod
+    def backward(ctx, gout, _gstats):
+        z, gamma, m, i, sc, sh, w = ctx.saved_tensors
+        B, D, H, W, C = z.shape
+        act = ctx.act
+        pend_out = _take_pending_bn(gout)
+        if ctx.c1:
+            gout = gout.contiguous()
+            gy = conv3d_c1_dgrad(gout, w.contiguous(), C)
+            gw = conv3d_c1_wgrad_onload(z, sc, sh, act, gout)
+        else:
+            gw = None
+            if pend_out is not None:
+                if get_lib().raw("stx_conv3d_wgrad_bn_supported")(B, D, H, W, C, w.shape[0]):
+                    gw, gout = conv3d_wgrad_bn_onload(z, sc, sh, act, gout, pend_out)
+                else:
+                    gout = pend_out.materialize()
+            gout = gout.contiguous()
+            gy, _ = conv3d_forward(gout, pack_weight(w, 1), C, 3, 1)
+            if gw is None:
+                gw = conv3d_wgrad_onload(z, sc, sh, act, gout)
+            gw = gw.reshape(w.shape)
+        nvox = z.numel() // C
+        NB = get_lib().raw("stx_bn_reduce_blocks")()
+        part = _WS.get("bnred", NB * 3 * C, z.device)
+        sums_all = torch.empty(1, 3, C, dtype=torch.float32, device=z.device)
+        _call("stx_bn_bwd_reduce2", _p(gy), None, _p(z), _p(m), _p(i), None, None, None, _p(sc) if act else None,
+              _p(sh) if act else None, None, None, _p(part), _p(sums_all), nvox, C, act, 1)
+        pend = _PendingBn()
+        pend.g, pend.z, pend.scale, pend.shift, pend.mean, pend.invstd = gy, z, sc, sh, m, i
+        pend.gamma, pend.sums, pend.inv_n, pend.act = gamma, sums_all[:1], 1.0 / nvox, act
+        if not act:
+            pend.scale = pend.shift = m
+        tot = sums_all[0]
+        if ctx.defer:
+            _defer_pending_bn(gy, pend)
+            gz = gy
+        else:
+            gz = pend.materialize()
+        return gz, tot[1], tot[0], gw, None, None, None, None
 
 
 class ConvRawFn(torch.autograd.Function):
```

New measurement: 0.1783 pairs/s. About the same (-0.1%).
